# NREL/SSRS

Hardware: AMD Instinct MI355X
Metric: simulated tracks/sec (whole node) (higher is better)
Workload: dtype f64

## Files before the change

include/ssrs_hip.h:

```cpp
#ifndef SSRS_HIP_H_
#define SSRS_HIP_H_

#include <stddef.h>
#include <stdint.h>

#ifdef __cplusplus
extern "C" {
#endif

#define SSRS_VERSION 108

#define SSRS_OK 0
#define SSRS_ERR_INVALID (-1)
#define SSRS_ERR_HIP (-2)
#define SSRS_ERR_START (-3)

#define SSRS_F32 0
#define SSRS_F64 1

int ssrs_version(void);
int ssrs_build_flags(void);
const char *ssrs_last_error(void);
int ssrs_device_info(int device, char *name, size_t name_len, int *compute_units,
                     size_t *hbm_bytes);
// ... 174 lines not shown
                       int64_t ntracks, const int64_t *traj_offsets, int16_t *traj,
                       void *cursor_ws, size_t cursor_bytes, void *stream);

int ssrs_hist_reduce(uint32_t *hist, size_t n, int root, void *nccl_comm, void *stream);


int ssrs_presence_count(const int16_t *traj, int64_t npoints, uint32_t *hist,
                        int rows, int cols, void *scratch8, void *stream);

size_t ssrs_presence_workspace_bytes(int rows, int cols, int krad);

int ssrs_presence_smooth(const uint32_t *count, int krad, float *out, int rows,
                         int cols, void *workspace, size_t workspace_bytes,
                         void *stream);

int ssrs_presence_smooth_u64(const uint64_t *count, int krad, float *out, int rows,
                             int cols, void *workspace, size_t workspace_bytes,
                             void *stream);

int ssrs_presence_normalise_add(const void *src, int src_type, double *acc, size_t n,
                                void *scratch8, void *stream);
int ssrs_presence_normalise_f32(const double *src, float *out, size_t n,
                                void *scratch8, void *stream);


#define SSRS_TURBINE_BIN 32
#define SSRS_TURBINE_MAX 8192
int ssrs_turbine_encounters(const int16_t *traj, const int64_t *traj_offsets, int64_t ntracks,
                            const double *turbines, int nturb, double radius_cells,
                            const int32_t *bin_start, const int32_t *bin_items, int rows, int cols,
                            uint32_t *hits, int32_t *first_step, void *stream);

int ssrs_turbine_encounter_counts(const uint32_t *hits, int64_t ntracks, int nturb,
                                  int64_t *tracks_per_turbine, int32_t *turbines_per_track, void *stream);


#define SSRS_OCCUPANCY_MAX_PLANES 8
size_t ssrs_track_occupancy_workspace_bytes(int rows, int cols, int planes);
int ssrs_track_occupancy(const int16_t *traj, const int64_t *traj_offsets, int64_t ntracks,
                         int rows, int cols, int planes,
                         uint32_t *counts, uint32_t *cells_per_track,
                         void *workspace, size_t workspace_bytes, void *stream);


#define SSRS_RAY_ROW_NORTH 0
#define SSRS_RAY_ROW_EAST 1
#define SSRS_SHELTER_AUTO 0
#define SSRS_SHELTER_LDS 1
#define SSRS_SHELTER_GLOBAL 2
int ssrs_shelter_sx(const void *dem, int dem_type, double res, const double *ray_ur, const double *ray_uc,
                    const double *wdirn, double dmax, int ray_axes, int path, double *tan_sx, double *sx_deg,
                    int rows, int cols, int batch, void *stream);

typedef struct SsrsShelterParams {
    double dmax;
    int32_t ray_axes;
    int32_t path;
    double height;
    double coef[7];
} SsrsShelterParams;

int ssrs_updraft_sheltered(const void *dem, int dem_type, double res, const double *ray_ur, const double *ray_uc,
                           const double *wspeed0, const double *wdirn0, const double *wspeed, const double *wdirn,
                           const void *slope, const void *aspect, int sa_type, const SsrsShelterParams *params,
                           double min_updraft_val, double threshold, float *orograph, double *usable,
                           double *sx_deg, int rows, int cols, int batch, void *stream);

int ssrs_shelter_sx_sector(const void *dem, int dem_type, double res, const double *ray_ur, const double *ray_uc,
                           const double *wdirn, double dmax, int ray_axes, int path, double sector_half_width,
                           double sector_step, double *tan_sx, double *sx_deg, int rows, int cols, int batch,
                           void *stream);
int ssrs_updraft_sheltered_sector(const void *dem, int dem_type, double res, const double *ray_ur, const double *ray_uc,
                                  const double *wspeed0, const double *wdirn0, const double *wspeed,
                                  const double *wdirn, const void *slope, const void *aspect, int sa_type,
                                  const SsrsShelterParams *params, double sector_half_width, double sector_step,
                                  double min_updraft_val, double threshold, float *orograph, double *usable,
                                  double *sx_deg, int rows, int cols, int batch, void *stream);


#define SSRS_SMOOTH_AUTO 0
#define SSRS_SMOOTH_LDS 1
#define SSRS_SMOOTH_GLOBAL 2
size_t ssrs_smooth_workspace_bytes(int rows, int cols, int batch, double sigma);
int ssrs_smooth_reflect(const float *in, double sigma, int path, double min_updraft_val, double threshold,
                        double *smooth, float *orograph, double *usable, int rows, int cols, int batch,
                        void *workspace, size_t workspace_bytes, void *stream);


#define SSRS_ALLEN_MAX_UPDRAFTS (1 << 22)
#define SSRS_ALLEN_TABLE_COLS 6
#define SSRS_ALLEN_AUTO 0
#define SSRS_ALLEN_LDS 1
#define SSRS_ALLEN_GLOBAL 2
size_t ssrs_allen_workspace_bytes(int n_updrafts);
int ssrs_allen_thermal_field(const double *xt, const double *yt, const double *wgain, const double *rgain,
                             int n_updrafts, const int32_t *bin_start, const int32_t *bin_items, double bin_size_m,
                             int nbx, int nby, double rbar, double wtbar, double zzi, int z_below_zi, double we,
                             double res, int rows, int cols, int path, void *out, int out_type, int32_t *nearest,
                             double *table, void *workspace, size_t workspace_bytes, void *stream);


typedef struct SsrsProjection {
    double a;
    double e2;
    double lat_1;
    double lat_2;
    double lat_0;
    double lon_0;
    double x_0;
    double y_0;
    double n;
    double C;
    double rho0;
    double e;
} SsrsProjection;

int ssrs_projection_init_albers(SsrsProjection *proj);

int ssrs_warp_lonlat_raster(const void *src, int src_type, int src_rows, int src_cols, double lon0, double lat0,
                            double dlon, double dlat, double nodata, const SsrsProjection *proj, double west,
                            double south, double res, void *dst, int dst_type, double *lon, double *lat,
                            unsigned long long *uncovered, int rows, int cols, void *stream);


typedef struct SsrsSolveStats {
    int32_t iterations;
    int32_t converged;
    double residual;
    float kernel_ms;
    int32_t amg_levels;
    int32_t amg_coarsest;
    float setup_ms;
    uint64_t workspace_used;
} SsrsSolveStats;

#define SSRS_SOLVE_NO_AMG 1
#define SSRS_SOLVE_K_CYCLE 2
#define SSRS_SOLVE_ONE_SIDED 4

size_t ssrs_potential_workspace_bytes(int rows, int cols);

int ssrs_potential_solve(const double *conductivity, const uint8_t *fixed_mask,
                         const double *fixed_values, const double *initial_guess,
                         float *potential, int rows, int cols, double rel_tol,
                         int max_iterations, int flags, void *workspace,
                         size_t workspace_bytes,
                         void *stats ,
                         void *stream);

int ssrs_uniform_selftest(uint64_t seed, const uint64_t *track,
                          const uint64_t *step, double *out, size_t n,
                          void *stream);

#ifdef __cplusplus
}
#endif
#endif
```

ssrs_amd/_native.py:

```python
import ctypes as C
import os

_HERE = os.path.dirname(os.path.abspath(__file__))
LIB_PATH = os.environ.get('SSRS_HIP_LIB') or os.path.join(_HERE, 'libssrs_hip.so')

SSRS_F32, SSRS_F64 = 0, 1
SSRS_OK, SSRS_ERR_INVALID, SSRS_ERR_HIP, SSRS_ERR_START = 0, -1, -2, -3
SSRS_TRACKS_PROFILE = 1
SSRS_TRACKS_EXACT_ONLY = 2
SSRS_TRACKS_NO_SCHEDULE = 4
SSRS_TRACKS_NO_BINNING = 8
SSRS_TRACKS_RING_TABLE = 16
SSRS_TRACKS_SCATTERED = 32
SSRS_TRACKS_NO_SCATTERED = 64
SSRS_TRACKS_THR_TABLE = 128
SSRS_SOLVE_NO_AMG = 1
SSRS_TURBINE_BIN, SSRS_TURBINE_MAX = 32, 8192
SSRS_OCCUPANCY_MAX_PLANES = 8
SSRS_RAY_AXES = {'row_north': 0, 'row_east': 1}
SSRS_SHELTER_PATH = {'auto': 0, 'lds': 1, 'global': 2}
SSRS_SMOOTH_PATH = {'auto': 0, 'lds': 1, 'global': 2}
SSRS_ALLEN_PATH = {'auto': 0, 'lds': 1, 'global': 2}
SSRS_ALLEN_MAX_UPDRAFTS, SSRS_ALLEN_TABLE_COLS = 1 << 22, 6
SSRS_INTERP = {'nearest': 0, 'linear': 1, 'cubic': 2}

EXPORTS = (
    'ssrs_version', 'ssrs_build_flags', 'ssrs_last_error', 'ssrs_device_info', 'ssrs_slope_aspect',
    'ssrs_orographic_updraft', 'ssrs_threshold_updraft', 'ssrs_updraft_from_dem',
    'ssrs_lattice_workspace_bytes', 'ssrs_updraft_from_dem_lattice',
    'ssrs_wind_from_lattice', 'ssrs_wind_triangles_workspace_bytes', 'ssrs_wind_from_triangles',
    'ssrs_wind_nearest_workspace_bytes', 'ssrs_wind_nearest_index', 'ssrs_wind_from_nearest',
    'ssrs_wind_cubic_workspace_bytes', 'ssrs_wind_from_triangles_cubic', 'ssrs_thermal_seeds', 'ssrs_blur_workspace_bytes',
    'ssrs_gaussian_blur', 'ssrs_thermal_fields', 'ssrs_potential_temperature', 'ssrs_deardorff_velocity',
    'ssrs_thermal_updraft', 'ssrs_scalar_interp_workspace_bytes', 'ssrs_scalar_from_samples', 'ssrs_wtk_thermal_fields',
    'ssrs_track_params_init', 'ssrs_transition_table_build',
    'ssrs_transition_ring_bytes', 'ssrs_transition_ring_build',
    'ssrs_transition_thr_bytes', 'ssrs_transition_thr_build',
    'ssrs_tracks_workspace_bytes', 'ssrs_tracks_workspace_bytes_ex', 'ssrs_tracks_simulate', 'ssrs_uniform_selftest',
    'ssrs_traj_recorder_create', 'ssrs_traj_recorder_destroy', 'ssrs_traj_recorder_complete',
    'ssrs_traj_recorder_used', 'ssrs_tracks_simulate_rec', 'ssrs_tracks_gather', 'ssrs_tracks_simulate_h64',
    'ssrs_hist_reduce', 'ssrs_presence_count', 'ssrs_presence_workspace_bytes', 'ssrs_presence_smooth',
    'ssrs_presence_smooth_u64',
    'ssrs_presence_normalise_add', 'ssrs_presence_normalise_f32',
    'ssrs_potential_workspace_bytes', 'ssrs_potential_solve',
    'ssrs_turbine_encounters', 'ssrs_turbine_encounter_counts',
    'ssrs_shelter_sx', 'ssrs_updraft_sheltered', 'ssrs_shelter_sx_sector', 'ssrs_updraft_sheltered_sector',
    'ssrs_smooth_workspace_bytes', 'ssrs_smooth_reflect',
    'ssrs_projection_init_albers', 'ssrs_warp_lonlat_raster',
    'ssrs_allen_workspace_bytes', 'ssrs_allen_thermal_field',
    'ssrs_track_occupancy_workspace_bytes', 'ssrs_track_occupancy',
)


class SsrsTrackParams(C.Structure):
    _fields_ = [('rows', C.c_int32), ('cols', C.c_int32), ('burnin', C.c_int32),
                ('memory_parameter', C.c_int32), ('max_moves', C.c_int64),
                ('scaling_parameter', C.c_double), ('prior', C.c_double * 9),
                ('steps_per_launch', C.c_int32), ('flags', C.c_int32)]


class SsrsTrackStats(C.Structure):
    _fields_ = [('total_steps', C.c_int64), ('launches', C.c_int32),
                ('kernel_ms', C.c_float), ('wall_ms', C.c_float), ('hist_ms', C.c_float),
                ('window_launches', C.c_int32), ('tile_launches', C.c_int32),
                ('block_window_launches', C.c_int32), ('wander_sorts', C.c_int32),
                ('timed_launches', C.c_int32), ('first_move_ms', C.c_float),
                ('block_window_ms', C.c_float), ('block_window_timed', C.c_int32),
                ('block_window_steps', C.c_int64), ('roam_launches', C.c_int32), ('reserved0', C.c_int32),
                ('roam_wave_pairs', C.c_int64), ('roam_slow_wave_pairs', C.c_int64),
                ('roam_shuffles', C.c_int32), ('roam_wide_launches', C.c_int32)]


class SsrsSolveStats(C.Structure):
    _fields_ = [('iterations', C.c_int32), ('converged', C.c_int32),
                ('residual', C.c_double), ('kernel_ms', C.c_float),
                ('amg_levels', C.c_int32), ('amg_coarsest', C.c_int32),
                ('setup_ms', C.c_float), ('workspace_used', C.c_uint64)]


class SsrsShelterParams(C.Structure):
    _fields_ = [('dmax', C.c_double), ('ray_axes', C.c_int32), ('path', C.c_int32), ('height', C.c_double),
                ('coef', C.c_double * 7)]


class SsrsProjection(C.Structure):
    _fields_ = [(name, C.c_double) for name in ('a', 'e2', 'lat_1', 'lat_2', 'lat_0', 'lon_0', 'x_0', 'y_0',
                                                'n', 'C', 'rho0', 'e')]


OCCUPANCY_ARGTYPES = [C.c_void_p, C.c_void_p, C.c_int64, C.c_int, C.c_int, C.c_int, C.c_void_p, C.c_void_p, C.c_void_p,
                      C.c_size_t, C.c_void_p]

ALLEN_FIELD_ARGTYPES = [C.c_void_p] * 4 + [C.c_int, C.c_void_p, C.c_void_p, C.c_double, C.c_int, C.c_int] + \
    [C.c_double] * 3 + [C.c_int, C.c_double, C.c_double, C.c_int, C.c_int, C.c_int, C.c_void_p, C.c_int, C.c_void_p,
                        C.c_void_p, C.c_void_p, C.c_size_t, C.c_void_p]


class SsrsError(RuntimeError):
    def __init__(self, code, message):
        super().__init__(f'libssrs_hip error {code}: {message}')
        self.code = code


_lib = None


def lib():
    global _lib
    if _lib is None:
        if not os.path.exists(LIB_PATH):
            raise ImportError(
                f'{LIB_PATH} is missing: build it with `python ssrs_amd/csrc/build.py` '
                '(hipcc, gfx950). ssrs_amd has no CPU fallback.')
        L = C.CDLL(LIB_PATH)
        L.ssrs_version.restype = C.c_int
        if L.ssrs_build_flags() & 1 and not os.environ.get('SSRS_ALLOW_PROBE_LIB'):
            raise ImportError(f'{LIB_PATH} is a timing-probe build (results are wrong on purpose); '
                              'set SSRS_ALLOW_PROBE_LIB=1 for timing runs only')
        L.ssrs_last_error.restype = C.c_char_p
        L.ssrs_tracks_workspace_bytes.restype = C.c_size_t
        L.ssrs_tracks_workspace_bytes.argtypes = [C.c_int64]
        L.ssrs_lattice_workspace_bytes.restype = C.c_size_t
        L.ssrs_wind_triangles_workspace_bytes.restype = C.c_size_t
        L.ssrs_wind_triangles_workspace_bytes.argtypes = [C.c_int, C.c_int, C.c_int, C.c_int]
        L.ssrs_lattice_workspace_bytes.argtypes = [C.c_int, C.c_int, C.c_int]
        L.ssrs_wind_nearest_workspace_bytes.restype = C.c_size_t
        L.ssrs_wind_nearest_workspace_bytes.argtypes = [C.c_int, C.c_int, C.c_int]
        L.ssrs_wind_nearest_index.argtypes = [C.c_void_p, C.c_int, C.c_double, C.c_void_p, C.c_int, C.c_int,
                                              C.c_void_p, C.c_size_t, C.c_void_p]
        L.ssrs_wind_cubic_workspace_bytes.restype = C.c_size_t
        L.ssrs_wind_cubic_workspace_bytes.argtypes = [C.c_int, C.c_int, C.c_int, C.c_int, C.c_int]
        L.ssrs_wind_from_triangles_cubic.argtypes = [C.c_void_p] * 8 + [C.c_int, C.c_int, C.c_double, C.c_void_p, C.c_void_p,
                                                                        C.c_int, C.c_int, C.c_int, C.c_void_p, C.c_size_t,
                                                                        C.c_void_p]
        L.ssrs_tracks_workspace_bytes_ex.restype = C.c_size_t
        L.ssrs_tracks_workspace_bytes_ex.argtypes = [C.c_int64, C.c_int, C.c_int, C.c_int]
        L.ssrs_traj_recorder_create.restype = C.c_void_p
        L.ssrs_traj_recorder_create.argtypes = [C.c_void_p, C.c_size_t]
        L.ssrs_traj_recorder_destroy.restype = None
        L.ssrs_traj_recorder_destroy.argtypes = [C.c_void_p]
        L.ssrs_traj_recorder_complete.argtypes = [C.c_void_p]
        L.ssrs_traj_recorder_used.restype = C.c_size_t
        L.ssrs_traj_recorder_used.argtypes = [C.c_void_p]
        L.ssrs_transition_thr_bytes.restype = C.c_size_t
        L.ssrs_transition_thr_bytes.argtypes = [C.c_int, C.c_int]
        L.ssrs_transition_ring_bytes.restype = C.c_size_t
        L.ssrs_transition_ring_bytes.argtypes = [C.c_int, C.c_int]
        if hasattr(L, 'ssrs_presence_workspace_bytes'):
            L.ssrs_presence_workspace_bytes.restype = C.c_size_t
            L.ssrs_presence_workspace_bytes.argtypes = [C.c_int, C.c_int, C.c_int]
        if hasattr(L, 'ssrs_blur_workspace_bytes'):
            L.ssrs_blur_workspace_bytes.restype = C.c_size_t
            L.ssrs_blur_workspace_bytes.argtypes = [C.c_int, C.c_int, C.c_double]
        L.ssrs_thermal_fields.argtypes = [C.c_void_p, C.c_double, C.c_double, C.POINTER(C.c_uint64), C.c_int,
                                          C.c_void_p, C.c_int, C.c_int, C.c_int, C.c_void_p]
        L.ssrs_potential_temperature.argtypes = [C.c_void_p, C.c_void_p, C.c_void_p, C.c_size_t, C.c_void_p]
        L.ssrs_deardorff_velocity.argtypes = [C.c_void_p, C.c_void_p, C.c_void_p, C.c_double, C.c_void_p, C.c_size_t, C.c_void_p]
        L.ssrs_thermal_updraft.argtypes = [C.c_void_p, C.c_double, C.c_void_p, C.c_void_p, C.c_double, C.c_void_p, C.c_size_t,
                                           C.c_void_p]
        L.ssrs_scalar_interp_workspace_bytes.restype = C.c_size_t
        L.ssrs_scalar_interp_workspace_bytes.argtypes = [C.c_int] * 5
        L.ssrs_scalar_from_samples.argtypes = [C.c_int] + [C.c_void_p] * 7 + [C.c_int, C.c_int, C.c_double, C.c_void_p, C.c_int,
                                                                             C.c_int, C.c_int, C.c_void_p, C.c_size_t, C.c_void_p]
        L.ssrs_wtk_thermal_fields.argtypes = [C.c_int] + [C.c_void_p] * 7 + [C.c_int, C.c_int, C.c_double, C.c_void_p, C.c_double,
                                                                            C.c_double, C.c_void_p, C.c_int, C.c_int, C.c_int,
                                                                            C.c_int, C.c_void_p, C.c_size_t, C.c_void_p]
        if hasattr(L, 'ssrs_potential_workspace_bytes'):
            L.ssrs_potential_workspace_bytes.restype = C.c_size_t
            L.ssrs_potential_workspace_bytes.argtypes = [C.c_int, C.c_int]
        if hasattr(L, 'ssrs_turbine_encounters'):
            L.ssrs_turbine_encounters.argtypes = [C.c_void_p, C.c_void_p, C.c_int64, C.c_void_p, C.c_int, C.c_double,
                                                  C.c_void_p, C.c_void_p, C.c_int, C.c_int, C.c_void_p, C.c_void_p,
                                                  C.c_void_p]
            L.ssrs_turbine_encounter_counts.argtypes = [C.c_void_p, C.c_int64, C.c_int, C.c_void_p, C.c_void_p, C.c_void_p]
        L.ssrs_shelter_sx.argtypes = [C.c_void_p, C.c_int, C.c_double, C.c_void_p, C.c_void_p, C.c_void_p, C.c_double,
                                      C.c_int, C.c_int, C.c_void_p, C.c_void_p, C.c_int, C.c_int, C.c_int, C.c_void_p]
        L.ssrs_updraft_sheltered.argtypes = [C.c_void_p, C.c_int, C.c_double] + [C.c_void_p] * 8 + \
            [C.c_int, C.POINTER(SsrsShelterParams), C.c_double, C.c_double, C.c_void_p, C.c_void_p, C.c_void_p,
             C.c_int, C.c_int, C.c_int, C.c_void_p]
        L.ssrs_shelter_sx_sector.argtypes = [C.c_void_p, C.c_int, C.c_double, C.c_void_p, C.c_void_p, C.c_void_p, C.c_double,
                                             C.c_int, C.c_int, C.c_double, C.c_double, C.c_void_p, C.c_void_p, C.c_int,
                                             C.c_int, C.c_int, C.c_void_p]
        L.ssrs_updraft_sheltered_sector.argtypes = [C.c_void_p, C.c_int, C.c_double] + [C.c_void_p] * 8 + \
            [C.c_int, C.POINTER(SsrsShelterParams), C.c_double, C.c_double, C.c_double, C.c_double, C.c_void_p, C.c_void_p,
             C.c_void_p, C.c_int, C.c_int, C.c_int, C.c_void_p]
        L.ssrs_smooth_workspace_bytes.restype = C.c_size_t
        L.ssrs_smooth_workspace_bytes.argtypes = [C.c_int, C.c_int, C.c_int, C.c_double]
        L.ssrs_smooth_reflect.argtypes = [C.c_void_p, C.c_double, C.c_int, C.c_double, C.c_double, C.c_void_p, C.c_void_p,
                                          C.c_void_p, C.c_int, C.c_int, C.c_int, C.c_void_p, C.c_size_t, C.c_void_p]
        L.ssrs_projection_init_albers.argtypes = [C.POINTER(SsrsProjection)]
        L.ssrs_warp_lonlat_raster.argtypes = [C.c_void_p, C.c_int, C.c_int, C.c_int] + [C.c_double] * 5 + \
            [C.POINTER(SsrsProjection)] + [C.c_double] * 3 + [C.c_void_p, C.c_int, C.c_void_p, C.c_void_p, C.c_void_p,
                                                             C.c_int, C.c_int, C.c_void_p]
        L.ssrs_allen_workspace_bytes.restype = C.c_size_t
        L.ssrs_allen_workspace_bytes.argtypes = [C.c_int]
        L.ssrs_allen_thermal_field.argtypes = ALLEN_FIELD_ARGTYPES
        L.ssrs_track_occupancy_workspace_bytes.restype = C.c_size_t
        L.ssrs_track_occupancy_workspace_bytes.argtypes = [C.c_int, C.c_int, C.c_int]
        L.ssrs_track_occupancy.argtypes = OCCUPANCY_ARGTYPES
        _lib = L
    return _lib


def check(rc):
    if rc != SSRS_OK:
        msg = lib().ssrs_last_error().decode('utf-8', 'replace')
        if rc == SSRS_ERR_INVALID or rc == SSRS_ERR_START:
            raise ValueError(f'libssrs_hip: {msg}')
        raise SsrsError(rc, msg)


def ptr(t):
    return C.c_void_p(0 if t is None else t.data_ptr())
```

ssrs_amd/csrc/tracks.hip:

```cpp
#include <rocrand/rocrand_philox4x32_10.h>
#include <hipcub/hipcub.hpp>

#include <cmath>
#include <cstdlib>
#include <cstring>
#include <new>
#include <vector>

#include "common.h"
#include "track_plan.h"
#include "track_policy.h"

namespace ssrs {

__host__ __device__ constexpr int dr_of(int k) { return k / 3 - 1; }
__host__ __device__ constexpr int dc_of(int k) { return k % 3 - 1; }
#define SSRS_NINV_DIAG 0.70710677f

constexpr uint32_t restriction(int d)
{
    const int dr = dr_of(d), dc = dc_of(d);
    uint32_t m = 0;
    for (int k = 0; k < 9; ++k) {
        bool ok = false;
// ... 31 lines not shown
    int n = 0;
    for (int k = 0; k < 9 && n < 3; ++k)
        if ((restriction(d) >> k) & 1u) v |= static_cast<uint32_t>(k < 4 ? k : k - 1) << (3 * n++);
    return v;
}
constexpr uint64_t pack_candidates(int first, int count)
{
    uint64_t v = 0;
    for (int i = 0; i < count; ++i) v |= static_cast<uint64_t>(candidates(first + i)) << (9 * i);
    return v;
}
constexpr uint64_t kCandLo = pack_candidates(0, 7), kCandHi = pack_candidates(7, 2);
static_assert(candidates(7) == (5u | (6u << 3) | (7u << 6)), "(1,0) -> table slots 5,6,7");
static_assert(candidates(5) == (2u | (4u << 3) | (7u << 6)), "(0,1) -> k = 2,5,8 = slots 2,4,7");

__device__ __forceinline__ uint32_t candidates_of(uint32_t d)
{
    const uint64_t v = d < 7 ? (kCandLo >> (9 * d)) : (kCandHi >> (9 * (d - 7)));
    return static_cast<uint32_t>(v) & 0x1FFu;
}

constexpr int kRingK[8] = {7, 8, 5, 2, 1, 0, 3, 6};
constexpr int ring_of_k(int k)
{
    for (int c = 0; c < 8; ++c)
        if (kRingK[c] == k) return c;
    return 8;
}
constexpr bool ring_matches_restrictions()
{
    for (int c = 0; c < 8; ++c) {
        const uint32_t m = (1u << kRingK[(c + 7) % 8]) | (1u << kRingK[c]) | (1u << kRingK[(c + 1) % 8]);
        if (m != restriction(kRingK[c])) return false;
    }
    return true;
}
static_assert(ring_matches_restrictions(), "restriction(d) = ring neighbours of d");
constexpr uint32_t ring_order(int c)
{
    const int ks[3] = {kRingK[(c + 7) % 8], kRingK[c], kRingK[(c + 1) % 8]};
    uint32_t v = 0;
    int n = 0;
    for (int k = 0; k < 9; ++k)
        for (int j = 0; j < 3; ++j)
            if (ks[j] == k) v |= static_cast<uint32_t>(j) << (2 * n++);
    return v;
}
constexpr uint64_t pack_ring_orders()
{
    uint64_t v = 0;
    for (int c = 0; c < 8; ++c) v |= static_cast<uint64_t>(ring_order(c)) << (6 * c);
    return v;
}
constexpr uint64_t kRingOrder = pack_ring_orders();
constexpr uint32_t kOrdId = 0u | (1u << 2) | (2u << 4), kOrdRot = 2u | (0u << 2) | (1u << 4),
                   kOrdRev = 2u | (1u << 2) | (0u << 4), kOrdSwp = 1u | (0u << 2) | (2u << 4);
static_assert(ring_order(0) == kOrdId && ring_order(6) == kOrdId && ring_order(7) == kOrdId, "x0 x1 x2");
static_assert(ring_order(1) == kOrdRot, "after NE: x2 x0 x1");
static_assert(ring_order(2) == kOrdRev && ring_order(3) == kOrdRev && ring_order(4) == kOrdRev, "x2 x1 x0");
static_assert(ring_order(5) == kOrdSwp, "after SW: x1 x0 x2");
static_assert(ring_order(0) == (0u | (1u << 2) | (2u << 4)), "after N: NW, N, NE are k = 6, 7, 8");
static_assert(ring_order(2) == (2u | (1u << 2) | (0u << 4)), "after E: NE, E, SE are k = 8, 5, 2");
constexpr uint32_t pack_ring_deltas(bool rows)
{
    uint32_t v = 1u << 16;
    for (int c = 0; c < 8; ++c)
        v |= static_cast<uint32_t>((rows ? dr_of(kRingK[c]) : dc_of(kRingK[c])) + 1) << (2 * c);
    return v;
}
constexpr uint32_t kRingDr = pack_ring_deltas(true), kRingDc = pack_ring_deltas(false);
constexpr uint32_t pack_ring_next(int sel)
{
    uint32_t v = 0;
    for (int c = 0; c < 8; ++c) v |= static_cast<uint32_t>((c + 7 + ((ring_order(c) >> (2 * sel)) & 3u)) & 7u) << (4 * c);
    return v;
}
constexpr uint32_t kRingNext0 = pack_ring_next(0), kRingNext1 = pack_ring_next(1), kRingNext2 = pack_ring_next(2);
constexpr uint32_t pack_ring_deltas_signed(bool rows)
{
    uint32_t v = 0;
    for (int c = 0; c < 8; ++c)
        v |= (static_cast<uint32_t>(rows ? dr_of(kRingK[c]) : dc_of(kRingK[c])) & 3u) << (4 * c);
    return v;
}
constexpr uint32_t kRingDrS = pack_ring_deltas_signed(true), kRingDcS = pack_ring_deltas_signed(false);
constexpr uint64_t pack_ring_of_k()
{
    uint64_t v = 0;
    for (int k = 0; k < 9; ++k) v |= static_cast<uint64_t>(ring_of_k(k)) << (4 * k);
    return v;
}
constexpr uint64_t kRingOfK = pack_ring_of_k();
constexpr uint64_t pack_k_of_ring()
{
    uint64_t v = 4ull << 32;
    for (int c = 0; c < 8; ++c) v |= static_cast<uint64_t>(kRingK[c]) << (4 * c);
    return v;
}
constexpr uint64_t kKOfRing = pack_k_of_ring();
constexpr int kRingFloats = 10;
__host__ __device__ constexpr size_t ring_mask_offset(int rows, int cols)
{
    return static_cast<size_t>(rows) * static_cast<size_t>(cols) * kRingFloats * sizeof(float) + 8;
}

__device__ __forceinline__ uint4 philox_block(uint64_t seed, uint64_t track, uint64_t blk)
{
#ifdef SSRS_PROBE_NO_PHILOX
    const uint32_t h = static_cast<uint32_t>(blk) * 0x9E3779B9u ^ static_cast<uint32_t>(track) * 0x85EBCA6Bu ^
                       static_cast<uint32_t>(seed);
    return make_uint4(h * 0xC2B2AE35u, h ^ 0x27D4EB2Fu, (h >> 3) * 0x165667B1u, h + 0x9E3779B9u);
#endif
    rocrand_state_philox4x32_10 st;
    rocrand_init(seed, track, blk * 4ull, &st);
    return rocrand4(&st);
}

__device__ __forceinline__ uint4 philox_block_b3(uint64_t seed, uint64_t track, uint64_t blk)
{
    uint32_t c0 = static_cast<uint32_t>(blk), c1 = static_cast<uint32_t>(blk >> 32);
    uint32_t c2 = static_cast<uint32_t>(track), c3 = static_cast<uint32_t>(track >> 32);
    uint32_t k0 = static_cast<uint32_t>(seed), k1 = static_cast<uint32_t>(seed >> 32);
#pragma unroll
    for (int r = 0; r < 10; ++r) {
        const uint64_t p0 = static_cast<uint64_t>(0xD2511F53u) * c0, p1 = static_cast<uint64_t>(0xCD9E8D57u) * c2;
        const uint32_t n0 = __builtin_amdgcn_bitop3_b32(static_cast<uint32_t>(p1 >> 32), c1, k0, 0x96);
        const uint32_t n2 = __builtin_amdgcn_bitop3_b32(static_cast<uint32_t>(p0 >> 32), c3, k1, 0x96);
        c1 = static_cast<uint32_t>(p1);
        c3 = static_cast<uint32_t>(p0);
        c0 = n0;
        c2 = n2;
        k0 += 0x9E3779B9u;
        k1 += 0xBB67AE85u;
    }
    return make_uint4(c0, c1, c2, c3);
}

__device__ __forceinline__ double words_to_uniform(uint32_t a, uint32_t b)
{
    return (static_cast<double>(a >> 5) * 67108864.0 + static_cast<double>(b >> 6)) *
           (1.0 / 9007199254740992.0);
}

__global__ void k_uniform_selftest(uint64_t seed, const uint64_t *track, const uint64_t *step,
                                   double *out, size_t n)
{
    const size_t i = blockIdx.x * static_cast<size_t>(blockDim.x) + threadIdx.x;
    if (i >= n) return;
    const uint4 w = philox_block(seed, track[i], step[i] >> 1);
    const uint4 v = philox_block_b3(seed, track[i], step[i] >> 1);
    const bool same = w.x == v.x && w.y == v.y && w.z == v.z && w.w == v.w;
    const double u = (step[i] & 1) ? words_to_uniform(w.z, w.w) : words_to_uniform(w.x, w.y);
    out[i] = same ? u : __longlong_as_double(0x7FF8000000000000ll);
}

__host__ __device__ __forceinline__ double sum9(const double *x)
{
    return (((x[0] + x[1]) + (x[2] + x[3])) + ((x[4] + x[5]) + (x[6] + x[7]))) + x[8];
}

__device__ __forceinline__ int choose_move(const double *w, const double *prior, double nu,
                                           uint32_t mask, double u, bool fast)
{
    double q[9];
    bool has_nan = false;
#pragma unroll
    for (int k = 0; k < 9; ++k) has_nan |= (w[k] != w[k]);
#pragma unroll
    for (int k = 0; k < 9; ++k) {
        const double v = has_nan ? prior[k] : w[k];
        q[k] = v > 0.0 ? v : 0.0;
    }
    q[4] = 0.0;
    bool any = false;
#pragma unroll
    for (int k = 0; k < 9; ++k) {
        const double z = q[k] * 0.0;
        q[k] = ((mask >> k) & 1u) ? q[k] : z;
        any |= (q[k] != 0.0);
    }
    if (!any) {
#pragma unroll
        for (int k = 0; k < 9; ++k) {
            q[k] = ((mask >> k) & 1u) && k != 4 ? prior[k] : 0.0;
            any |= (q[k] != 0.0);
        }
        if (!any) {
#pragma unroll
            for (int k = 0; k < 9; ++k) q[k] = prior[k];
        }
    }
    if (fast) {
        double c[8];
        double acc = 0.0;
#pragma unroll
        for (int k = 0; k < 8; ++k) { acc = acc + q[k]; c[k] = acc; }
        const double ut = u * (acc + q[8]);
        const double band = ut * 0x1p-46;
        int idx = 0;
        bool near = false;
#pragma unroll
        for (int k = 0; k < 8; ++k) {
            const double d = c[k] - ut;
            idx += d <= 0.0 ? 1 : 0;
            near |= !(fabs(d) > band);
        }
        if (!near) return idx;
    }
    const double s1 = sum9(q);
#pragma unroll
    for (int k = 0; k < 9; ++k) q[k] = q[k] / s1;
    if (nu != 1.0) {
#pragma unroll
        for (int k = 0; k < 9; ++k) q[k] = pow(q[k], nu);
    }
    const double s2 = sum9(q);
    double acc = 0.0;
    double cdf[9];
#pragma unroll
    for (int k = 0; k < 9; ++k) {
        q[k] = q[k] / s2;
        acc = acc + q[k];
        cdf[k] = acc;
    }
    int idx = 0;
#pragma unroll
    for (int k = 0; k < 9; ++k) idx += (cdf[k] / cdf[8] <= u) ? 1 : 0;
    return idx;
}

__device__ __forceinline__ int choose_table_fast(const double *t, uint32_t mask, double u)
{
    double c[8];
    double acc = 0.0;
#pragma unroll
    for (int j = 0; j < 8; ++j) {
        const int k = j < 4 ? j : j + 1;
        acc = acc + (((mask >> k) & 1u) ? t[j] : 0.0);
        c[j] = acc;
    }
    const double ut = u * acc;
    const double band = ut * 0x1p-46;
    int idx = 0;
    double closest = __builtin_inf();
#pragma unroll
    for (int j = 0; j < 7; ++j) {
        const double d = c[j] - ut;
        const int le = d <= 0.0 ? 1 : 0;
        idx += (j == 3) ? 2 * le : le;
        closest = fmin(closest, fabs(d));
    }
    const bool near = !(acc > 0.0) || !(closest > band);
    return near ? -1 : idx;
}

__device__ __forceinline__ int choose_three_fast(double wa, double wb, double wc, double u)
{
    const double ca = wa + 0.0;
    const double cb = ca + wb;
    const double acc = cb + wc;
    const double ut = u * acc;
    const double band = ut * 0x1p-46;
    const double da = ca - ut, db = cb - ut;
    const int sel = da > 0.0 ? 0 : (db > 0.0 ? 1 : 2);
    const double closest = fmin(fmin(fabs(da), fabs(db)), fmin(ut, fabs(acc - ut)));
    const bool near = !(acc > 0.0) || !(closest > band);
    return near ? -1 : sel;
}

__device__ __forceinline__ int choose_three_ring(float fa, float fb, float fc, double u)
{
    const double ca = static_cast<double>(fa);
    const double cb = ca + static_cast<double>(fb);
    const double acc = cb + static_cast<double>(fc);
    const double ut = u * acc;
    const double band = acc * 0x1p-21;
    const double da = ca - ut, db = cb - ut;
    const int sel = da > 0.0 ? 0 : (db > 0.0 ? 1 : 2);
    const double closest = fmin(fabs(da), fabs(db));
    const bool near = !(acc > 0x1p-90) || !(closest > band);
    return near ? -1 : sel;
}

__device__ __forceinline__ int choose_three_ring_f32(float fa, float fb, float fc, float uf)
{
    const float cb = fa + fb;
    const float acc = cb + fc;
    const float ut = uf * acc;
    const float band = acc * 0x1p-19f;
    const float da = fa - ut, db = cb - ut;
    const int sel = da > 0.f ? 0 : (db > 0.f ? 1 : 2);
    const float closest = fminf(fabsf(da), fabsf(db));
    const bool near = !(acc > 0x1p-90f) || !(closest > band);
    return near ? -1 : sel;
}

template <bool HAS_POT>
__device__ __forceinline__ void window_weights(const double *__restrict__ updraft,
                                               const float *__restrict__ potential,
                                               int cols, int row, int col, double *w)
{
    const size_t centre = static_cast<size_t>(row) * cols + col;
    double win[9];
#pragma unroll
    for (int j = 0; j < 9; ++j) {
        const double v = updraft[centre + dr_of(j) * cols + dc_of(j)];
// ... 28 lines not shown
        v[j] = updraft[centre + dr_of(j) * cols + dc_of(j)];
        fine &= (v[j] <= 1e150) & (v[j] >= -1e150);
        if (HAS_POT) {
            p[j] = potential[centre + dr_of(j) * cols + dc_of(j)];
            fine &= fabsf(p[j]) <= 1e38f;
        }
    }
    if (!fine) return -1;
    const double ic = 1.0 / (v[4] > 1e-06 ? v[4] : 1e-06);
    double w3[3] = {0.0, 0.0, 0.0};
    int k3[3] = {0, 0, 0};
    int n = 0;
#pragma unroll
    for (int j = 0; j < 9; ++j) {
        if (j == 4) continue;
        const bool adm = (mask >> j) & 1u;
        if (adm) {
            double w = 2.0 / (ic + 1.0 / (v[j] > 1e-06 ? v[j] : 1e-06));
            if (HAS_POT) {
                const float d = p[4] - p[j];
                const float ninv = (j & 1) ? 1.f : SSRS_NINV_DIAG;
                const float e = d * ninv;
                w = w * static_cast<double>(e);
            }
            w = w > 0.0 ? w : 0.0;
            if (n == 0) { w3[0] = w; k3[0] = j; } else if (n == 1) { w3[1] = w; k3[1] = j; } else { w3[2] = w; k3[2] = j; }
            ++n;
        }
    }
    if (n != 3) return -1;
    if (w3[0] == 0.0 && w3[1] == 0.0 && w3[2] == 0.0) {
        const double *t = thr + 9u * last_k;
        int idx = 0;
#pragma unroll
        for (int k = 0; k < 9; ++k) idx += t[k] <= u ? 1 : 0;
        return (idx == 4 || idx > 8) ? -1 : idx;
    }
    const int sel = choose_three_fast(w3[0], w3[1], w3[2], u);
    return sel < 0 ? -1 : (sel == 0 ? k3[0] : (sel == 1 ? k3[1] : k3[2]));
}

constexpr int kTabW = 64, kTabH = 16;
__device__ __forceinline__ int xcd_band(int b, int n)
{
    const int q = n / 8, r = n % 8, x = b % 8, j = b / 8;
    return (x < r ? x * (q + 1) : r * (q + 1) + (x - r) * q) + j;
}

template <bool RING>
__global__ __launch_bounds__(kBlock) void k_transition_table(
    const double *__restrict__ updraft, const float *__restrict__ potential,
    void *__restrict__ table_out, int rows, int cols, int tiles_x, int ntiles)
{
    constexpr int LW = kTabW + 2, LH = kTabH + 2;
    __shared__ double s_inv[LW * LH];
    __shared__ float s_pot[LW * LH];
    const int t = xcd_band(blockIdx.x, ntiles);
    const int r0 = (t / tiles_x) * kTabH, c0 = (t % tiles_x) * kTabW;
    for (int i = threadIdx.x; i < LW * LH; i += kBlock) {
        const int lr = i / LW, lc = i - lr * LW;
        int gr = r0 - 1 + lr, gc = c0 - 1 + lc;
        gr = gr < 0 ? 0 : (gr >= rows ? rows - 1 : gr);
        gc = gc < 0 ? 0 : (gc >= cols ? cols - 1 : gc);
        const size_t g = static_cast<size_t>(gr) * cols + gc;
        const double v = updraft[g];
        const double w = v != v ? v : (v > 1e-06 ? v : 1e-06);
        s_inv[i] = 1.0 / w;
        s_pot[i] = potential ? potential[g] : 0.f;
    }
    __syncthreads();
    const int lc = static_cast<int>(threadIdx.x % kTabW) + 1;
    const int col = c0 + lc - 1;
    if (col >= cols) return;
    for (int lr = static_cast<int>(threadIdx.x / kTabW) + 1; lr <= kTabH; lr += kBlock / kTabW) {
        const int row = r0 + lr - 1;
        if (row >= rows) break;
        const size_t i = static_cast<size_t>(row) * cols + col;
        double w[9];
        const bool interior = row > 0 && col > 0 && row < rows - 1 && col < cols - 1;
        if (interior) {
            const double ic = s_inv[lr * LW + lc];
            const float pc = s_pot[lr * LW + lc];
#pragma unroll
            for (int j = 0; j < 9; ++j) {
                const int o = (lr + dr_of(j)) * LW + lc + dc_of(j);
                w[j] = 2.0 / (ic + s_inv[o]);
                if (potential) {
                    const float d = pc - s_pot[o];
                    const float ninv = (j == 4) ? 0.f : ((j & 1) ? 1.f : SSRS_NINV_DIAG);
                    const float e = d * ninv;
                    w[j] = w[j] * static_cast<double>(e);
                }
            }
        } else {
#pragma unroll
            for (int j = 0; j < 9; ++j) w[j] = 0.0;
        }
        bool has_nan = false;
#pragma unroll
        for (int j = 0; j < 9; ++j) has_nan |= (w[j] != w[j]);
        if (RING) {
            bool bad = has_nan;
#pragma unroll
            for (int j = 0; j < 9; ++j) bad |= (w[j] - w[j] != 0.0);
            float f[kRingFloats];
#pragma unroll
            for (int j = 0; j < kRingFloats; ++j) {
                const double v = w[kRingK[(j + 7) % 8]];
                f[j] = bad ? __builtin_nanf("") : (v > 0.0 ? static_cast<float>(v) : -0.0f);
            }
            float2 *dst = reinterpret_cast<float2 *>(static_cast<float *>(table_out) + i * kRingFloats);
#pragma unroll
            for (int k = 0; k < kRingFloats / 2; ++k) dst[k] = make_float2(f[2 * k], f[2 * k + 1]);
            uint32_t zm = 0;
#pragma unroll
            for (int c = 0; c < 8; ++c) zm |= (!bad && !(w[kRingK[c]] > 0.0)) ? (1u << c) : 0u;
            (static_cast<uint8_t *>(table_out) + ring_mask_offset(rows, cols))[i] = static_cast<uint8_t>(zm);
        } else {
            double2 *dst = reinterpret_cast<double2 *>(static_cast<double *>(table_out) + i * 8);
            double o[8];
#pragma unroll
            for (int j = 0, k = 0; j < 9; ++j) {
                if (j == 4) continue;
                o[k++] = has_nan ? __builtin_nan("") : (w[j] > 0.0 ? w[j] : 0.0);
            }
#pragma unroll
            for (int k = 0; k < 4; ++k) dst[k] = make_double2(o[2 * k], o[2 * k + 1]);
        }
    }
}

struct alignas(16) TrackState {
    int32_t pos;
    int32_t k;
    uint32_t dirs;
    uint32_t aux;
};

static_assert(kPlanBlock == kBlock, "track_plan.h counts in stepper blocks");
struct alignas(16) TrackCtl {
    uint32_t count[4][kXcd];
    uint32_t error;
    uint32_t par_min;
    unsigned long long steps;
    unsigned long long strays;
    uint32_t bin_done;
    uint32_t pad;
    double prior[9];
    unsigned long long roam_slow;
    unsigned long long roam_pairs;
    unsigned long long dbg_tsum, dbg_tmax, dbg_waves, dbg_slowmax;
    uint32_t roam_stop;
    uint32_t deal_live;
};

static_assert(sizeof(TrackCtl) <= 128 * sizeof(uint32_t), "final read-back slot of pinned_counts()");

constexpr uint32_t kWanderMix = 256;
constexpr int kBinRows = 36, kBinCols = kWinCols / 4;
constexpr int kWinBinRows = kWinRows / kBinRows;
constexpr int kWanderBins = 16384;
struct WanderWindows {
    int32_t n;
    int32_t r0[kWanderWindows], c0[kWanderWindows];
};



struct PlanGeom {
    double cos_t, sin_t;
    int offset;
};
__device__ __forceinline__ void plan_coords(const PlanGeom &g, int row, int col, int &par, int &perp)
{
    par = static_cast<int>(lrint(row * g.cos_t + col * g.sin_t)) + g.offset;
    perp = static_cast<int>(lrint(col * g.cos_t - row * g.sin_t)) + g.offset;
}

template <typename KeyT>
__global__ __launch_bounds__(kBlock) void k_plan_keys(const int32_t *__restrict__ start_rc,
                                                     long long ntracks, PlanGeom g,
                                                     KeyT *__restrict__ keys,
                                                     int32_t *__restrict__ vals, TrackCtl *ctl, int par_bits)
{
    const long long t = blockIdx.x * static_cast<long long>(kBlock) + threadIdx.x;
    int par = 0x7fffffff;
    if (t < ntracks) {
        int perp;
        plan_coords(g, start_rc[2 * t], start_rc[2 * t + 1], par, perp);
        par = par < 0 ? 0 : par;
        perp = perp < 0 ? 0 : perp;
        const int top = (1 << par_bits) - 1;
        keys[t] = (static_cast<KeyT>(perp > top ? top : perp) << par_bits) | static_cast<KeyT>(par > top ? top : par);
        vals[t] = static_cast<int32_t>(t);
    }
    __shared__ int s_min;
    if (threadIdx.x == 0) s_min = 0x7fffffff;
    __syncthreads();
#pragma unroll
    for (int off = 32; off > 0; off >>= 1) {
        const int o = __shfl_down(par, off);
        par = o < par ? o : par;
    }
    if ((threadIdx.x & 63) == 0 && par != 0x7fffffff) atomicMin(&s_min, par);
    __syncthreads();
    if (threadIdx.x == 0 && s_min != 0x7fffffff) atomicMin(&ctl->par_min, static_cast<uint32_t>(s_min));
}

__device__ __forceinline__ int wander_window_of(const WanderWindows *__restrict__ w, int n, int row, int col)
{
    int id = n;
    for (int q = n - 1; q >= 0; --q)
        if (static_cast<uint32_t>(row - w->r0[q]) < static_cast<uint32_t>(kWinRows) &&
            static_cast<uint32_t>(col - w->c0[q]) < static_cast<uint32_t>(kWinCols)) id = q;
    return id;
}

enum { MODE_PRIOR = 0, MODE_UPDRAFT = 1, MODE_FLUIDFLOW = 2, MODE_TABLE = 3 };

struct RoamEntry;

struct StepArgs {
    int rows, cols, burnin, memory;
    long long max_k;
    double nu;
    const double *prior;
    const double *updraft;
    const float *potential;
    const double *table;
    unsigned long long seed, track_base;
    uint32_t *hist;
    int16_t *end_rc;
    int32_t *lengths;
    int16_t *traj;
    const long long *traj_off;
    TrackState *state;
    const int32_t *list_in;
    int32_t *list_out;
    TrackCtl *ctl;
    int launch;
    int fast;
    int steps;
    int coherent;
    uint32_t *visits;
    long long visit_stride;
    uint32_t cap;
    long long it_base;
    int plane_shift;
    uint32_t guard;
    int v16_offset;
    int pf_dir, pf_rc;
    uint32_t vcap;
    const double *thr;
    const uint8_t *zmask;
    uint32_t *hist_copies;
    int ncopies;
    const WanderWindows *wander;
    const RoamEntry *roam;
    const void *fine;
    int roam_stop;
    int cheap_exact;
    unsigned long long *dbg_buf;
    int debug_roam;
    uint32_t vis_r, vis_c;
};

__global__ __launch_bounds__(kBlock) void k_tracks_init(
    const int32_t *__restrict__ start_rc, long long ntracks, int rows, int cols,
    uint32_t *hist, int16_t *traj, const long long *traj_off, int32_t *lengths,
    int16_t *end_rc, TrackState *state, TrackCtl *ctl, PlanGeom g, int coherent, uint32_t cap)
{
    const long long t = blockIdx.x * static_cast<long long>(kBlock) + threadIdx.x;
    if (t < kXcd) {
        const long long left = ntracks - t * static_cast<long long>(cap);
        ctl->count[0][t] = static_cast<uint32_t>(left < 0 ? 0 : (left > cap ? cap : left));
        ctl->count[1][t] = ctl->count[2][t] = ctl->count[3][t] = 0;
        if (t == 0) ctl->steps = 0;
    }
    if (t >= ntracks) return;
    const int row = start_rc[2 * t], col = start_rc[2 * t + 1];
    TrackState s;
    s.dirs = 0x44444444u;
    uint32_t delay = 0;
    if (coherent) {
        int par, perp;
        plan_coords(g, row, col, par, perp);
        par = par < 0 ? 0 : par;
        const uint32_t pmin = ctl->par_min;
        delay = static_cast<uint32_t>(par) > pmin ? static_cast<uint32_t>(par) - pmin : 0u;
        if (delay > 0x7FFFFFu) delay = 0x7FFFFFu;
        delay &= ~1u;
    }
    s.aux = kAllButCentre | (delay << 9);
    if (row < 0 || col < 0 || row >= rows || col >= cols) {
        atomicOr(&ctl->error, 1u);
        s.pos = 0;
        s.k = -1;
        if (lengths) lengths[t] = 0;
        if (end_rc) { end_rc[2 * t] = -1; end_rc[2 * t + 1] = -1; }
    } else {
        s.pos = row | (col << 16);
        s.k = 0;
        if (hist) atomicAdd(&hist[static_cast<size_t>(row) * cols + col], 1u);
        if (traj)
            reinterpret_cast<uint32_t *>(traj)[traj_off[t]] =
                static_cast<uint32_t>(row & 0xFFFF) | (static_cast<uint32_t>(col) << 16);
    }
    state[t] = s;
}

template <int MODE>
__global__ __launch_bounds__(kBlock) void k_step_tracks(const StepArgs a)
{
    TrackCtl *ctl = a.ctl;
    const int in_slot = a.launch & 3, out_slot = (a.launch + 1) & 3;
    const uint32_t xcd = blockIdx.x % kXcd;
    const uint32_t nlive = ctl->count[in_slot][xcd];
    const uint32_t il = (blockIdx.x / kXcd) * kBlock + threadIdx.x;
    const uint32_t i = xcd * a.cap + il;
    const uint32_t iv = xcd * a.vcap + il;
    if (blockIdx.x == 0 && threadIdx.x < kXcd)
        ctl->count[(a.launch + 2) & 3][threadIdx.x] = 0;
    if ((il & ~63u) >= nlive) return;

    bool active = il < nlive;
    const int32_t t = active ? (a.list_in ? a.list_in[i] : static_cast<int32_t>(i)) : 0;
    TrackState s = {0, -1, 0, 0};
    if (active) s = a.state[t];
    active = active && s.k >= 0;
    int row = s.pos & 0xFFFF, col = (s.pos >> 16) & 0xFFFF;
    int k = s.k;
    const int max_k = static_cast<int>(a.max_k);
    uint32_t dirs = s.dirs, run = s.aux & 0x1FFu;
    const long long rel64 = (a.coherent ? static_cast<long long>(s.aux >> 9) : 0) -
                            static_cast<long long>(a.launch) * a.steps;
    const int release = rel64 > 0x7fffffffLL ? 0x7fffffff : (rel64 < 0 ? 0 : static_cast<int>(rel64));
    const unsigned long long track = a.track_base + static_cast<unsigned long long>(t);
    const long long toff = (a.traj && active) ? a.traj_off[t] : 0;
    const long long troom = (a.traj && active) ? a.traj_off[t + 1] - toff : 0;
    uint32_t pend_a = 0, pend_b = 0;
    bool have_pending = false;
    uint32_t moved = 0;
    int last_it = -1;

    const int lane_id = threadIdx.x & 63;

    bool done = false;
    int er = row, ec = col;
    auto loop_head = [&]() {
        done = !(k < max_k);
        er = row;
        ec = col;
        if (!done) {
            if (k > a.burnin) {
                done = !(0 < row && row < a.rows - 1 && 0 < col && col < a.cols - 1);
            } else {
                if (er <= 1) er += 2; else if (er >= a.rows - 2) er -= 2;
                if (ec <= 0) ec += 2; else if (ec >= a.cols - 2) ec -= 2;
            }
        }
    };
    double2 t0 = {0.0, 0.0}, t1 = t0, t2 = t0, t3 = t0;
    auto fetch_entry = [&]() {
        if (MODE == MODE_TABLE) {
            const double2 *src = reinterpret_cast<const double2 *>(
                a.table + (static_cast<size_t>(er) * a.cols + ec) * 8);
            t0 = src[0]; t1 = src[1]; t2 = src[2]; t3 = src[3];
        }
    };
    if (active) loop_head();
    fetch_entry();

    for (int it = 0; it < a.steps; ++it) {
        if (!__any(active)) break;
        bool stepped = false;
        if (active && it >= release) {
            if (done) {
                if (a.lengths) a.lengths[t] = static_cast<int32_t>(k + 1);
                if (a.end_rc)
                    reinterpret_cast<uint32_t *>(a.end_rc)[t] =
                        static_cast<uint32_t>(row & 0xFFFF) | (static_cast<uint32_t>(col) << 16);
                active = false;
            } else {
                uint32_t wa, wb;
                if ((k & 1) && have_pending) {
                    wa = pend_a; wb = pend_b;
                } else {
                    const uint4 w4 = philox_block(a.seed, track, static_cast<unsigned long long>(k) >> 1);
                    if (k & 1) { wa = w4.z; wb = w4.w; }
                    else { wa = w4.x; wb = w4.y; pend_a = w4.z; pend_b = w4.w; }
                }
                have_pending = !(k & 1);
                const double u = words_to_uniform(wa, wb);
                uint32_t mask = kAllButCentre;
                if (a.memory == 1) {
                    mask = restriction_of(dirs & 0xFu);
                } else if (a.memory == 0) {
                    mask = run;
                } else {
                    uint32_t d = dirs;
                    for (int j = 0; j < a.memory; ++j) {
                        mask &= restriction_of(d & 0xFu);
                        d >>= 4;
                    }
                }
                int idx = -1;
                if (MODE == MODE_TABLE) {
                    const double tt[8] = {t0.x, t0.y, t1.x, t1.y, t2.x, t2.y, t3.x, t3.y};
                    if (a.fast) idx = choose_table_fast(tt, mask, u);
                    if (__builtin_expect(idx < 0, 0)) {
                        double o[8];
#pragma unroll
                        for (int j = 0; j < 8; ++j) { o[j] = tt[j]; asm volatile("" : "+v"(o[j])); }
                        asm volatile("" : "+v"(mask));
                        const double w[9] = {o[0], o[1], o[2], o[3], 0.0, o[4], o[5], o[6], o[7]};
                        double pr[9];
#pragma unroll
                        for (int j = 0; j < 9; ++j) pr[j] = a.prior[j];
                        idx = choose_move(w, pr, a.nu, mask, u, false);
                    }
                } else {
                    double w[9];
                    if (MODE == MODE_FLUIDFLOW) {
                        window_weights<true>(a.updraft, a.potential, a.cols, er, ec, w);
                    } else if (MODE == MODE_UPDRAFT) {
                        window_weights<false>(a.updraft, a.potential, a.cols, er, ec, w);
                    } else {
#pragma unroll
                        for (int j = 0; j < 9; ++j) w[j] = a.prior[j];
                    }
                    double pr[9];
#pragma unroll
                    for (int j = 0; j < 9; ++j) pr[j] = a.prior[j];
                    idx = choose_move(w, pr, a.nu, mask, u, a.fast != 0);
                }
                row = er + idx / 3 - 1;
                col = ec + idx % 3 - 1;
                dirs = (dirs << 4) | static_cast<uint32_t>(idx);
                if (a.memory == 0) run &= restriction_of(static_cast<uint32_t>(idx));
                ++k;
                ++moved;
                stepped = true;
                loop_head();
                if (a.traj && k < troom)
                    reinterpret_cast<uint32_t *>(a.traj)[toff + k] =
                        static_cast<uint32_t>(row & 0xFFFF) | (static_cast<uint32_t>(col) << 16);
            }
        }
        fetch_entry();
        if (a.visits) {
            a.visits[static_cast<long long>(it) * a.visit_stride + iv] =
                stepped ? __umul24(static_cast<uint32_t>(row), a.vis_r) + __umul24(static_cast<uint32_t>(col), a.vis_c)
                        : 0xFFFFFFFFu;
        } else if (a.hist) {
            uint32_t *h = a.hist;
            if (a.hist_copies)
                h = a.hist_copies + static_cast<size_t>((i >> 6) % static_cast<uint32_t>(a.ncopies)) *
                                        (static_cast<size_t>(a.rows) * a.cols);
            atomicAdd(&h[static_cast<size_t>(row) * a.cols + col], stepped ? 1u : 0u);
        }
        last_it = it;
    }
    if (a.visits)
        for (int it = last_it + 1; it < a.steps; ++it)
            a.visits[static_cast<long long>(it) * a.visit_stride + iv] = 0xFFFFFFFFu;

    const unsigned long long live = __ballot(active);
    const int lane = lane_id;
    const int nsurv = __popcll(live);
    uint32_t base = 0;
    if (lane == 0 && nsurv) base = atomicAdd(&ctl->count[out_slot][xcd], static_cast<uint32_t>(nsurv));
    base = __shfl(base, 0);
    if (active) {
        const int rank = __popcll(live & ((1ull << lane) - 1ull));
        a.list_out[xcd * a.cap + base + rank] = t;
        TrackState o;
        o.pos = row | (col << 16);
        o.k = k;
        o.dirs = dirs;
        o.aux = run | (s.aux & ~0x1FFu);
        a.state[t] = o;
    }
    unsigned long long m = moved;
#pragma unroll
    for (int off = 32; off > 0; off >>= 1) m += __shfl_down(m, off);
    if (lane == 0 && m) atomicAdd(&ctl->steps, m);
}

struct PriorArg { double v[9]; };

constexpr unsigned long long kThrMagic = 0x3152485453525353ull;
struct ThrHeader {
    unsigned long long magic;
    int32_t rows, cols;
    double prior[9];
};
static_assert(sizeof(ThrHeader) <= 256, "the header lives in the leading guard band (>= 256 bytes)");

__global__ void k_ctl_init(TrackCtl *ctl, const PriorArg pr, double *__restrict__ thr, WanderWindows *wander,
                           const ThrHeader *__restrict__ header, int rows, int cols)
{
    const int d = threadIdx.x;
    if (d == 33) wander->n = 0;
    if (d < 32) reinterpret_cast<uint32_t *>(ctl->count)[d] = 0;
    if (d == 32) {
        uint32_t bad = 0;
        if (header) {
            bad = (header->magic != kThrMagic || header->rows != rows || header->cols != cols) ? 2u : 0u;
            for (int k = 0; k < 9; ++k) bad |= (header->prior[k] != pr.v[k]) ? 2u : 0u;
        }
        ctl->error = bad; ctl->par_min = 0xFFFFFFFFu; ctl->steps = 0; ctl->strays = 0; ctl->bin_done = 0; ctl->pad = 0; ctl->roam_slow = 0; ctl->roam_pairs = 0;
        ctl->dbg_tsum = ctl->dbg_tmax = ctl->dbg_waves = ctl->dbg_slowmax = 0;
        ctl->roam_stop = ctl->deal_live = 0;
    }
    if (d < 9) ctl->prior[d] = pr.v[d];
    if (d >= 9) return;
    const double *prior = pr.v;
    const uint32_t mask = restriction_of(static_cast<uint32_t>(d));
    double q[9];
    bool any = false;
#pragma unroll
    for (int k = 0; k < 9; ++k) {
        q[k] = ((mask >> k) & 1u) && k != 4 ? prior[k] : 0.0;
        any |= (q[k] != 0.0);
    }
    if (!any) {
#pragma unroll
        for (int k = 0; k < 9; ++k) q[k] = prior[k];
    }
    const double s1 = sum9(q);
#pragma unroll
    for (int k = 0; k < 9; ++k) q[k] = q[k] / s1;
    const double s2 = sum9(q);
    double acc = 0.0, cdf[9];
#pragma unroll
    for (int k = 0; k < 9; ++k) {
        q[k] = q[k] / s2;
        acc = acc + q[k];
        cdf[k] = acc;
    }
#pragma unroll
    for (int k = 0; k < 9; ++k) thr[d * 9 + k] = cdf[k] / cdf[8];
}

constexpr uint32_t pack_slot_deltas(bool rows)
{
    uint32_t v = 0;
    for (int j = 0; j < 8; ++j) {
        const int k = j < 4 ? j : j + 1;
        v |= static_cast<uint32_t>((rows ? dr_of(k) : dc_of(k)) + 1) << (2 * j);
    }
    return v;
}
constexpr uint32_t kSlotDr = pack_slot_deltas(true), kSlotDc = pack_slot_deltas(false);

struct __attribute__((packed, aligned(4))) RingTriple { float x0, x1, x2; };

template <bool RING, bool ZMASK = false, bool VT = false>
__global__ __launch_bounds__(kBlock) void k_step_lean(const StepArgs a)
{
    TrackCtl *ctl = a.ctl;
    const int in_slot = a.launch & 3, out_slot = (a.launch + 1) & 3;
    const uint32_t xcd = blockIdx.x % kXcd;
    const uint32_t nlive = ctl->count[in_slot][xcd];
    const uint32_t il = (blockIdx.x / kXcd) * kBlock + threadIdx.x;
    const uint32_t i = xcd * a.cap + il;
    const uint32_t iv = xcd * a.vcap + il;
    if (blockIdx.x == 0 && threadIdx.x < kXcd) ctl->count[(a.launch + 2) & 3][threadIdx.x] = 0;
    if ((il & ~63u) >= nlive) return;

    bool active = il < nlive;
    const int32_t t = active ? (a.list_in ? a.list_in[i] : static_cast<int32_t>(i)) : 0;
    TrackState s = {0, -1, 0, 0};
    if (active) s = a.state[t];
    active = active && s.k >= 0;
    const bool was_active = active;
    int row = s.pos & 0xFFFF, col = (s.pos >> 16) & 0xFFFF;
    int k = s.k;
    const int max_k = static_cast<int>(a.max_k);
    uint32_t dirs = s.dirs;
    uint32_t rc = static_cast<uint32_t>(kRingOfK >> (4 * (dirs & 0xFu))) & 0xFu;
    (void)rc;
    const long long rel64 = (a.coherent ? static_cast<long long>(s.aux >> 9) : 0) -
                            static_cast<long long>(a.launch) * a.steps;
    const int release = rel64 > 0x7fffffffLL ? 0x7fffffff : (rel64 < 0 ? 0 : static_cast<int>(rel64));
    const unsigned long long track = a.track_base + static_cast<unsigned long long>(t);
    uint32_t pend_a = 0, pend_b = 0, moved = 0;
    const uint32_t ucols = static_cast<uint32_t>(a.cols);
    const uint32_t in_rows = static_cast<uint32_t>(a.rows - 2), in_cols = static_cast<uint32_t>(a.cols - 2);

    bool done;
    int er, ec;
    auto loop_head = [&]() {
        const bool interior = static_cast<uint32_t>(row - 1) < in_rows && static_cast<uint32_t>(col - 1) < in_cols;
        done = !(k < max_k) || (k > a.burnin && !interior);
        er = row;
        ec = col;
        if (__any(k <= a.burnin)) {
            if (k <= a.burnin) {
                if (er <= 1) er += 2; else if (er >= a.rows - 2) er -= 2;
                if (ec <= 0) ec += 2; else if (ec >= a.cols - 2) ec -= 2;
            }
        }
    };
    double ta = 0.0, tb = 0.0, tc = 0.0;
    uint32_t cand = 0;
    RingTriple x = {0.f, 0.f, 0.f};
    (void)ta; (void)tb; (void)tc; (void)cand; (void)x;
    auto fetch_entry = [&]() {
        const uint32_t cell = __umul24(static_cast<uint32_t>(er), ucols) + static_cast<uint32_t>(ec);
        if (RING) {
            const float *src = reinterpret_cast<const float *>(a.table) +
                               static_cast<size_t>(cell) * kRingFloats + (rc & 7u);
            if (ZMASK) {
                const uint32_t m = a.zmask[cell];
                const uint32_t tri = (((m << 8) | m) >> ((rc + 7u) & 7u)) & 7u;
                if (tri == 7u && rc != 8u) x = RingTriple{-0.0f, -0.0f, -0.0f};
                else x = *reinterpret_cast<const RingTriple *>(src);
            } else {
#ifdef SSRS_PROBE_NO_GATHER
                (void)src;
                x = RingTriple{1.0f, 2.0f + static_cast<float>(er & 1), 1.5f};
#else
                x = *reinterpret_cast<const RingTriple *>(src);
#endif
            }
        } else {
            cand = candidates_of(dirs & 0xFu);
            const double *src = a.table + static_cast<size_t>(cell) * 8;
            ta = src[cand & 7u];
            tb = src[(cand >> 3) & 7u];
            tc = src[cand >> 6];
        }
    };
    loop_head();
    fetch_entry();

    int last_it = -1;
    auto one_step = [&](const int it, const bool even) {
        const bool go = active && it >= release;
        const bool st = go && !done;
        active = active && !(go && done);
        uint32_t w0, w1;
        if (even) {
            const uint4 w4 = philox_block(a.seed, track, static_cast<unsigned long long>(static_cast<uint32_t>(k) >> 1));
            w0 = w4.x; w1 = w4.y; pend_a = w4.z; pend_b = w4.w;
        } else {
            w0 = pend_a; w1 = pend_b;
        }
        int nrow, ncol;
        if (RING) {
            const float uf = static_cast<float>(w0 >> 8) * 0x1p-24f;
            const uint32_t ord = static_cast<uint32_t>(kRingOrder >> (6 * (rc & 7u))) & 63u;
            const uint32_t b0 = __float_as_uint(x.x0), b1 = __float_as_uint(x.x1), b2 = __float_as_uint(x.x2);
            const bool rot = ord == ring_order(1), rev = ord == ring_order(2), swp = ord == ring_order(5);
            const uint32_t ba = (rot || rev) ? b2 : (swp ? b1 : b0);
            const uint32_t bb = (rot || swp) ? b0 : b1;
            const uint32_t bc = rev ? b0 : (rot ? b1 : b2);
            int sel = choose_three_ring_f32(__uint_as_float(ba), __uint_as_float(bb), __uint_as_float(bc), uf);
            bool slow = st && (sel < 0 || rc == 8u);
            double u = 0.0;
            uint32_t prior_nc = 8u;
            if (__builtin_expect(__any(slow), 0)) {
                u = words_to_uniform(w0, w1);
                if (slow && rc != 8u) {
                    if ((ba & bb & bc) == 0x80000000u && (ba | bb | bc) == 0x80000000u) {
// ... 680 lines not shown
            s_surv[kBlock / 64] = tot ? atomicAdd(&ctl->count[out_slot][xcd], static_cast<uint32_t>(kBlock)) : 0xFFFFFFFFu;
        }
        __syncthreads();
        basei = s_surv[kBlock / 64];
        if (basei != 0xFFFFFFFFu) {
            a.list_out[xcd * a.cap + basei + threadIdx.x] = active ? t : -1;
            if (active) {
                TrackState o;
                o.pos = static_cast<int32_t>(row | (col << 16));
                o.k = k;
                o.dirs = static_cast<uint32_t>(kKOfRing >> (4 * rc)) & 0xFu;
                o.aux = s.aux;
                a.state[t] = o;
            }
        }
    } else {
        if (lane == 0 && nsurv) basei = atomicAdd(&ctl->count[out_slot][xcd], static_cast<uint32_t>(nsurv));
        basei = __shfl(basei, 0);
    }
    if (HM != 6 && active) {
        const int rank = __popcll(live & ((1ull << lane) - 1ull));
        a.list_out[xcd * a.cap + basei + rank] = t;
        TrackState o;
        o.pos = static_cast<int32_t>(row | (col << 16));
        o.k = k;
        o.dirs = static_cast<uint32_t>(kKOfRing >> (4 * rc)) & 0xFu;
        o.aux = s.aux;
        a.state[t] = o;
    }
    unsigned long long mv = live0 ? static_cast<unsigned long long>(k - s.k) : 0ull;
#pragma unroll
    for (int off = 32; off > 0; off >>= 1) mv += __shfl_down(mv, off);
    if (lane == 0 && mv) atomicAdd(&ctl->steps, mv);
}

struct alignas(16) RoamEntry {
    uint32_t e0, ea, eb, ec;
};
static_assert(sizeof(RoamEntry) == 16, "one dwordx4 per state");
constexpr size_t kPairMaxCells = 1ull << 25;

template <bool REV>
__global__ __launch_bounds__(kBlock) void k_roam_build(const char *__restrict__ tab, uint32_t guard, int plane_shift,
                                                      int rows, int cols, RoamEntry *__restrict__ out, const ThrPrior pr)
{
    const uint32_t nstate = static_cast<uint32_t>(rows) * static_cast<uint32_t>(cols) * 8u;
    for (uint32_t s = blockIdx.x * kBlock + threadIdx.x; s < nstate; s += gridDim.x * kBlock) {
        const uint32_t rc = s & 7u, cell = s >> 3;
        auto entry = [&](uint32_t c, uint32_t q) {
            return *reinterpret_cast<const uint32_t *>(tab + (guard + (q << plane_shift)) + (c << 2));
        };
        uint4 en = make_uint4(entry(cell, rc), kThrPoison, kThrPoison, kThrPoison);
        const bool rev = REV && en.x == kThrReversal;
        const uint32_t eu = rev ? pr.rev_e : en.x, rcd = rev ? pr.rev_rc : rc;
        if ((eu & 0xFFFFu) <= (eu >> 16)) {
            const uint32_t ord = static_cast<uint32_t>(kRingOrder >> (6u * rcd)) & 63u;
            uint32_t es[3];
#pragma unroll
            for (int j = 0; j < 3; ++j) {
                const uint32_t ncj = (rcd + 7u + ((ord >> (2 * j)) & 3u)) & 7u;
                const uint32_t cj = cell + ((kRingDr >> (2u * ncj)) & 3u) * static_cast<uint32_t>(cols) + ((kRingDc >> (2u * ncj)) & 3u) -
                                    static_cast<uint32_t>(cols) - 1u;
                es[j] = entry(cj, ncj);
            }
            en.y = es[0]; en.z = es[1]; en.w = es[2];
        }
        reinterpret_cast<uint4 *>(out)[s] = en;
    }
}

struct FineEntry { uint32_t t1, t2; };
struct FinePrior { uint32_t zero_t1[8], zero_t2[8], reversal; };

__host__ __device__ __forceinline__ uint32_t fine_fixed(double x)
{
    const double v = x * 4294967296.0 + 0.5;
    return v >= 4294967295.0 ? 0xFFFFFFFFu : static_cast<uint32_t>(static_cast<unsigned long long>(v));
}

template <bool HAS_POT>
__global__ __launch_bounds__(kBlock) void k_fine_build(const double *__restrict__ updraft, const float *__restrict__ potential,
                                                      FineEntry *__restrict__ out, int rows, int cols, int tiles_x, int ntiles,
                                                      const FinePrior fp)
{
    constexpr int LW = kTabW + 2, LH = kTabH + 2;
    __shared__ double s_inv[LW * LH];
    __shared__ float s_pot[LW * LH];
    const int t = xcd_band(blockIdx.x, ntiles);
    const int r0 = (t / tiles_x) * kTabH, c0 = (t % tiles_x) * kTabW;
    for (int i = threadIdx.x; i < LW * LH; i += kBlock) {
        const int lr = i / LW, lc = i - lr * LW;
        int gr = r0 - 1 + lr, gc = c0 - 1 + lc;
        gr = gr < 0 ? 0 : (gr >= rows ? rows - 1 : gr);
        gc = gc < 0 ? 0 : (gc >= cols ? cols - 1 : gc);
        const size_t g = static_cast<size_t>(gr) * cols + gc;
        const double v = updraft[g];
        const double w = v != v ? v : (v > 1e-06 ? v : 1e-06);
        s_inv[i] = 1.0 / w;
        s_pot[i] = HAS_POT ? potential[g] : 0.f;
    }
    __syncthreads();
    const int lc = static_cast<int>(threadIdx.x % kTabW) + 1;
    const int col = c0 + lc - 1;
    if (col >= cols) return;
    for (int lr = static_cast<int>(threadIdx.x / kTabW) + 1; lr <= kTabH; lr += kBlock / kTabW) {
        const int row = r0 + lr - 1;
        if (row >= rows) break;
        const size_t cell = static_cast<size_t>(row) * cols + col;
        const bool interior = row > 0 && col > 0 && row < rows - 1 && col < cols - 1;
        double w[9];
        bool bad = !interior;
        if (interior) {
            const double ic = s_inv[lr * LW + lc];
            const float pc = s_pot[lr * LW + lc];
#pragma unroll
            for (int j = 0; j < 9; ++j) {
                const int o = (lr + dr_of(j)) * LW + lc + dc_of(j);
                w[j] = 2.0 / (ic + s_inv[o]);
                if (HAS_POT) {
                    const float d = pc - s_pot[o];
                    const float ninv = (j == 4) ? 0.f : ((j & 1) ? 1.f : SSRS_NINV_DIAG);
                    const float e = d * ninv;
                    w[j] = w[j] * static_cast<double>(e);
                }
                bad |= !(w[j] - w[j] == 0.0);
                w[j] = w[j] > 0.0 ? w[j] : 0.0;
            }
        }
        FineEntry en[8];
#pragma unroll
        for (int rc = 0; rc < 8; ++rc) {
            const uint32_t ord = ring_order(rc);
            const int ring3[3] = {(rc + 7) % 8, rc, (rc + 1) % 8};
            const int ka = kRingK[ring3[ord & 3u]], kb = kRingK[ring3[(ord >> 2) & 3u]], kc = kRingK[ring3[(ord >> 4) & 3u]];
            FineEntry e = {0xFFFFFFFFu, 0u};
            if (!bad) {
                const double ab = w[ka] + w[kb], tot = ab + w[kc];
                if (tot == 0.0) {
                    if (!((fp.reversal >> rc) & 1u)) { e.t1 = fp.zero_t1[rc]; e.t2 = fp.zero_t2[rc]; }
                } else if (tot - tot == 0.0) {
                    e.t1 = fine_fixed(w[ka] / tot);
                    e.t2 = fine_fixed(ab / tot);
                    if (e.t1 > e.t2) e.t1 = e.t2;
                }
            }
            en[rc] = e;
        }
        uint4 *dst = reinterpret_cast<uint4 *>(out + cell * 8);
#pragma unroll
        for (int q = 0; q < 4; ++q) dst[q] = make_uint4(en[2 * q].t1, en[2 * q].t2, en[2 * q + 1].t1, en[2 * q + 1].t2);
    }
}

template <bool REV, int BT = kBlock>
__global__ __launch_bounds__(BT) void k_step_roam(const StepArgs a, const ThrPrior pr)
{
    __shared__ uint32_t s_win[kWinRows * kWinCols];
    __shared__ int s_box[4];
    __shared__ int s_wid[BT / 64];
    for (int q = threadIdx.x; q < kWinRows * kWinCols; q += BT) s_win[q] = 0u;
    if (threadIdx.x == 0) { s_box[0] = s_box[1] = 0x7fffffff; s_box[2] = s_box[3] = -1; }
    __syncthreads();
    TrackCtl *ctl = a.ctl;
    const int in_slot = a.launch & 3, out_slot = (a.launch + 1) & 3;
    const uint32_t xcd = blockIdx.x % kXcd;
    const uint32_t nlive = ctl->count[in_slot][xcd];
    const uint32_t il = (blockIdx.x / kXcd) * BT + threadIdx.x;
    const uint32_t i = xcd * a.cap + il;
    if (blockIdx.x == 0 && threadIdx.x < kXcd) ctl->count[(a.launch + 2) & 3][threadIdx.x] = 0;

    bool live0 = il < nlive;
    int32_t t = live0 ? (a.list_in ? a.list_in[i] : static_cast<int32_t>(i)) : 0;
    if (t < 0) { live0 = false; t = 0; }
    TrackState s = {0, -1, 0, 0};
    if (live0) s = a.state[t];
    uint32_t rc = static_cast<uint32_t>(kRingOfK >> (4 * (s.dirs & 0xFu))) & 0xFu;
    live0 = live0 && s.k >= 0 && rc < 8u;
    rc &= 7u;
    int row = s.pos & 0xFFFF, col = (s.pos >> 16) & 0xFFFF;
    int win_r0 = 0, win_c0 = 0;
    {
        int r_lo = live0 ? row : 0x7fffffff, r_hi = live0 ? row : -1, c_lo = live0 ? col : 0x7fffffff, c_hi = live0 ? col : -1;
#pragma unroll
        for (int off = 32; off > 0; off >>= 1) {
            int o = __shfl_xor(r_lo, off); r_lo = o < r_lo ? o : r_lo;
            o = __shfl_xor(r_hi, off); r_hi = o > r_hi ? o : r_hi;
            o = __shfl_xor(c_lo, off); c_lo = o < c_lo ? o : c_lo;
            o = __shfl_xor(c_hi, off); c_hi = o > c_hi ? o : c_hi;
        }
        if ((threadIdx.x & 63) == 0 && r_hi >= 0) {
            atomicMin(&s_box[0], r_lo); atomicMin(&s_box[1], c_lo);
            atomicMax(&s_box[2], r_hi); atomicMax(&s_box[3], c_hi);
        }
        __syncthreads();
        const bool fits = s_box[2] - s_box[0] < kWinRows && s_box[3] - s_box[1] < kWinCols;
        const int nwin = a.wander->n;
        int wid = live0 && nwin > 0 ? wander_window_of(a.wander, nwin, row, col) : 0x7fffffff;
        wid = wid >= nwin ? 0x7fffffff : wid;
        {
            const unsigned long long lm = __ballot(wid != 0x7fffffff);
            wid = lm ? __shfl(wid, __ffsll(static_cast<long long>(lm)) - 1) : 0x7fffffff;
        }
        if ((threadIdx.x & 63) == 0) s_wid[threadIdx.x >> 6] = wid;
        __syncthreads();
        wid = 0x7fffffff;
        for (int q = BT / 64 - 1; q >= 0; --q) wid = s_wid[q] != 0x7fffffff ? s_wid[q] : wid;
        if (wid != 0x7fffffff && threadIdx.x == 0) {
            s_box[0] = a.wander->r0[wid]; s_box[2] = s_box[0] + kWinRows - 1;
            s_box[1] = a.wander->c0[wid]; s_box[3] = s_box[1] + kWinCols - 1;
        }
        const bool placed = wid != 0x7fffffff;
        __syncthreads();
        if (!placed && !fits && threadIdx.x == 0) { s_box[0] = r_lo; s_box[1] = c_lo; s_box[2] = r_hi; s_box[3] = c_hi; }
        __syncthreads();
        if (s_box[2] >= 0) {
            win_r0 = (s_box[0] + s_box[2] + 1 - kWinRows) / 2;
            win_c0 = (s_box[1] + s_box[3] + 1 - kWinCols) / 2;
        }
    }
    const char *pair = reinterpret_cast<const char *>(a.roam);
    const uint32_t ucols = static_cast<uint32_t>(a.cols);
    const uint32_t last_cell = static_cast<uint32_t>(a.rows) * ucols - 1u;
    int k = s.k;
    const long long rel64 = (a.coherent ? static_cast<long long>(s.aux >> 9) : 0) + 1 - a.it_base;
    const int rel = rel64 > 0x3fffffffLL ? 0x3fffffff : (rel64 < 0 ? 0 : static_cast<int>(rel64));
    const long long left = a.max_k - k;
    uint32_t span = !live0 ? 0u : (left > 0x3fffffffLL ? 0x3fffffffu : (left < 0 ? 0u : static_cast<uint32_t>(left)));
    const int blk0 = (k - rel) >> 1;
    const unsigned long long track = a.track_base + static_cast<unsigned long long>(t);
    const char *tab = reinterpret_cast<const char *>(a.table);
    const uint32_t psh = static_cast<uint32_t>(a.plane_shift);
    const uint32_t rev_e = pr.rev_e;
    uint32_t win_stray = 0, n_fine = 0;
    const void *fine = a.fine;

    int wr = 0, wc = 0, lcell = 0;
    bool fast = false;
    uint4 E = make_uint4(kThrPoison, kThrPoison, kThrPoison, kThrPoison);
    auto enter = [&](bool released) __attribute__((always_inline)) {
        wr = row - win_r0;
        wc = col - win_c0;
        lcell = row * a.cols + col;
        fast = live0 && released && span != 0u && k > a.burnin;
        const uint32_t sidx = fast ? ((static_cast<uint32_t>(lcell) << 3) | rc) : 0u;
        E = *reinterpret_cast<const uint4 *>(pair + (sidx << 4));
    };
    enter(rel == 0);
    const uint32_t rev_rc4 = 4u * pr.rev_rc;

    auto slow_step = [&](const uint32_t w0, const uint32_t w1) __attribute__((always_inline)) {
        const uint32_t ufi = w0 >> 16;
        const uint32_t cell = static_cast<uint32_t>(row) * ucols + static_cast<uint32_t>(col);
        const uint32_t e = *reinterpret_cast<const uint32_t *>(tab + (a.guard + (rc << psh)) + (cell << 2));
        const int32_t d1 = static_cast<int32_t>(ufi) - static_cast<int32_t>(e & 0xFFFFu);
        const int32_t d2 = static_cast<int32_t>(ufi) - static_cast<int32_t>(e >> 16);
        const bool burn = k <= a.burnin;
        bool special = (static_cast<uint32_t>(d1 + 1) < 2u) | (static_cast<uint32_t>(d2 + 1) < 2u) | (d1 < d2);
        if (burn) special |= (row <= 1) | (row >= a.rows - 2) | (col >= a.cols - 2);
        uint32_t nc;
        int br = row, bc = col;
        if (!special) {
            const uint32_t ord = static_cast<uint32_t>(kRingOrder >> (6u * rc)) & 63u;
            const uint32_t neg = (static_cast<uint32_t>(d1) >> 31) + (static_cast<uint32_t>(d2) >> 31);
            nc = (rc + 7u + ((ord >> (4u - 2u * neg)) & 3u)) & 7u;
        } else {
            if (e == kThrBoundary && !burn) { span = 0u; return; }
            bool exact = true;
            nc = 0;
            if (fine && !(d1 < d2) && !(burn && ((row <= 1) | (row >= a.rows - 2) | (col >= a.cols - 2)))) {
                const uint2 f = reinterpret_cast<const uint2 *>(fine)[(cell << 3) | rc];
                const uint32_t u32 = (w0 & ~31u) | (w1 >> 27);
                const long long f1 = static_cast<long long>(u32) - static_cast<long long>(f.x);
                const long long f2 = static_cast<long long>(u32) - static_cast<long long>(f.y);
                const bool unsure = (f.x > f.y) | (static_cast<unsigned long long>(f1 + 1) < 2ull) | (static_cast<unsigned long long>(f2 + 1) < 2ull);
                if (!unsure) {
                    const uint32_t ord = static_cast<uint32_t>(kRingOrder >> (6u * rc)) & 63u;
                    const uint32_t neg = (f1 < 0 ? 1u : 0u) + (f2 < 0 ? 1u : 0u);
                    nc = (rc + 7u + ((ord >> (4u - 2u * neg)) & 3u)) & 7u;
                    exact = false;
                    ++n_fine;
                }
            }
            if (e == kThrReversal && !burn) {
                int idx = 0;
                bool near = false;
#pragma unroll
                for (int q = 0; q < 9; ++q) {
                    const int32_t d = static_cast<int32_t>(ufi) - static_cast<int32_t>(pr.thr9[q]);
                    idx += d >= 0 ? 1 : 0;
                    near |= static_cast<uint32_t>(d + 1) < 2u;
                }
                const uint32_t pnc = static_cast<uint32_t>(kRingOfK >> (4 * (idx > 8 ? 4 : idx))) & 0xFu;
                if (!near && pnc < 8u) { nc = pnc; exact = false; }
            }
            if (exact) {
                int er = row, ec = col;
                if (burn) {
                    if (er <= 1) er += 2; else if (er >= a.rows - 2) er -= 2;
                    if (ec <= 0) ec += 2; else if (ec >= a.cols - 2) ec -= 2;
                }
                double w[9];
                if (a.potential) window_weights<true>(a.updraft, a.potential, a.cols, er, ec, w);
                else window_weights<false>(a.updraft, a.potential, a.cols, er, ec, w);
                double prr[9];
#pragma unroll
                for (int j = 0; j < 9; ++j) prr[j] = a.prior[j];
                const uint32_t last = static_cast<uint32_t>(kKOfRing >> (4 * rc)) & 0xFu;
                const int idx = choose_move(w, prr, 1.0, restriction_of(last), words_to_uniform(w0, w1), true);
                nc = static_cast<uint32_t>(kRingOfK >> (4 * idx)) & 0xFu;
                br = er; bc = ec;
            }
        }
        row = br + static_cast<int>((kRingDr >> (2u * nc)) & 3u) - 1;
        col = bc + static_cast<int>((kRingDc >> (2u * nc)) & 3u) - 1;
        rc = nc;
        ++k;
        const uint32_t hr = static_cast<uint32_t>(row - win_r0), hc = static_cast<uint32_t>(col - win_c0);
        if (hr < static_cast<uint32_t>(kWinRows) && hc < static_cast<uint32_t>(kWinCols)) {
            atomicAdd(&s_win[hr * kWinCols + hc], 1u);
        } else {
            atomicAdd(&a.hist[static_cast<uint32_t>(row) * ucols + static_cast<uint32_t>(col)], 1u);
            ++win_stray;
        }
    };

    int it = 0;
    uint32_t n_pairs = 0, n_slow = 0;
    const unsigned long long t_begin = a.debug_roam ? __builtin_amdgcn_s_memtime() : 0ull;
    auto one_pair = [&]() __attribute__((always_inline)) {
        const uint4 w4 = philox_block_b3(a.seed, track, static_cast<unsigned long long>(static_cast<uint32_t>(blk0 + (it >> 1))));
        const uint32_t ufa = w4.x >> 16, ufb = w4.z >> 16;
        const bool st_a = static_cast<uint32_t>(it - rel) < span, st_b = static_cast<uint32_t>(it + 1 - rel) < span;
        const uint32_t q0 = E.x, qa = E.y, qb = E.z, qc = E.w;
        const uint32_t rc0 = rc;
        const uint32_t rc04 = 4u * rc0;
        const bool rva = REV && q0 == kThrReversal;
        const uint32_t eua = rva ? rev_e : q0;
        const uint32_t t4a = rva ? rev_rc4 : rc04;
        const bool ga1 = ufa >= (eua & 0xFFFFu), ga2 = ufa >= (eua >> 16);
        const uint32_t nxa = ga2 ? kRingNext2 : (ga1 ? kRingNext1 : kRingNext0);
        const uint32_t nca = (nxa >> t4a) & 7u, nca4 = 4u * nca;
        const uint32_t q1 = ga2 ? qc : (ga1 ? qb : qa);
        const int dra = __builtin_amdgcn_sbfe(static_cast<int>(kRingDrS), nca4, 2u), dca = __builtin_amdgcn_sbfe(static_cast<int>(kRingDcS), nca4, 2u);
        const int cell_a = lcell + __mul24(dra, a.cols) + dca;
        const bool rvb = REV && q1 == kThrReversal;
        const uint32_t eub = rvb ? rev_e : q1;
        const uint32_t t4b = rvb ? rev_rc4 : nca4;
        const bool gb1 = ufb >= (eub & 0xFFFFu), gb2 = ufb >= (eub >> 16);
        const uint32_t nxb = gb2 ? kRingNext2 : (gb1 ? kRingNext1 : kRingNext0);
        const uint32_t ncb = (nxb >> t4b) & 7u, ncb4 = 4u * ncb;
        const int drb = __builtin_amdgcn_sbfe(static_cast<int>(kRingDrS), ncb4, 2u), dcb = __builtin_amdgcn_sbfe(static_cast<int>(kRingDcS), ncb4, 2u);
        const int cell_b = cell_a + __mul24(drb, a.cols) + dcb;
        {
            const uint32_t cb = static_cast<uint32_t>(cell_b) < last_cell ? static_cast<uint32_t>(cell_b) : last_cell;
            E = *reinterpret_cast<const uint4 *>(pair + ((cb << 7) | (ncb4 << 2)));
        }
        const int wra = wr + dra, wca = wc + dca, wrb = wra + drb, wcb = wca + dcb;
        const int32_t a1 = static_cast<int32_t>(ufa) - static_cast<int32_t>(eua & 0xFFFFu);
        const int32_t a2 = static_cast<int32_t>(ufa) - static_cast<int32_t>(eua >> 16);
        const int32_t b1 = static_cast<int32_t>(ufb) - static_cast<int32_t>(eub & 0xFFFFu);
        const int32_t b2 = static_cast<int32_t>(ufb) - static_cast<int32_t>(eub >> 16);
        const bool special = (static_cast<uint32_t>(a1 + 1) < 2u) | (static_cast<uint32_t>(a2 + 1) < 2u) | (a1 < a2) |
                             (static_cast<uint32_t>(b1 + 1) < 2u) | (static_cast<uint32_t>(b2 + 1) < 2u) | (b1 < b2);
        const bool go = fast & st_a & st_b & !special;
        const bool in_a = go & (static_cast<uint32_t>(wra) < static_cast<uint32_t>(kWinRows)) & (static_cast<uint32_t>(wca) < static_cast<uint32_t>(kWinCols));
        const bool in_b = go & (static_cast<uint32_t>(wrb) < static_cast<uint32_t>(kWinRows)) & (static_cast<uint32_t>(wcb) < static_cast<uint32_t>(kWinCols));
        const bool out = go & !(in_a & in_b);
        const bool slow = (st_a | st_b) & !go;
        const unsigned long long rare = __ballot(out | slow);
        atomicAdd(&s_win[in_a ? (wra << 8) + wca : 0], in_a ? 1u : 0u);
        atomicAdd(&s_win[in_b ? (wrb << 8) + wcb : 0], in_b ? 1u : 0u);
        k += go ? 2 : 0;
        wr = go ? wrb : wr;
        wc = go ? wcb : wc;
        lcell = go ? cell_b : lcell;
        rc = go ? ncb : rc0;
        ++n_pairs;
        if (__builtin_expect(rare != 0ull, 0)) {
            if (__any(out)) {
#ifdef SSRS_PROBE_NO_STRAY_ATOMICS
                if (go && !in_a) ++win_stray;
                if (go && !in_b) ++win_stray;
#else
                if (go && !in_a) { atomicAdd(&a.hist[cell_a], 1u); ++win_stray; }
                if (go && !in_b) { atomicAdd(&a.hist[cell_b], 1u); ++win_stray; }
#endif
            }
            if (__any(slow)) {
                ++n_slow;
                if (slow) {
                    if (fast) { row = win_r0 + wr; col = win_c0 + wc; }
#pragma unroll 1
                    for (int h = 0; h < 2; ++h)
                        if (static_cast<uint32_t>(it + h - rel) < span) slow_step(h ? w4.z : w4.x, h ? w4.w : w4.y);
                    enter(true);
                }
            }
        }
        it += 2;
    };
    const uint32_t stop_stamp = static_cast<uint32_t>(a.launch) + 1u;
    uint32_t stop_seen = 0u;
    bool stopped = false;
    for (; it + 8 <= a.steps; ) {
        const unsigned long long stepping = __ballot(static_cast<uint32_t>(it - rel) < span), waiting = __ballot(it < rel && span != 0u);
        const bool stop_now = a.roam_stop && waiting == 0ull &&
                              static_cast<uint32_t>(__builtin_amdgcn_readfirstlane(static_cast<int>(stop_seen))) == stop_stamp;
        if (((stepping | waiting) == 0ull) | stop_now) { stopped = stop_now; break; }
        if (a.roam_stop) stop_seen = __hip_atomic_load(&ctl->roam_stop, __ATOMIC_RELAXED, __HIP_MEMORY_SCOPE_AGENT);
#pragma unroll
        for (int u = 0; u < 4; ++u) one_pair();
    }
    for (; it < a.steps && !stopped; ) {
        if (!__any(static_cast<uint32_t>(it - rel) < span || (it < rel && span != 0u))) break;
        one_pair();
    }
    if (a.roam_stop && !stopped && it >= a.steps && (threadIdx.x & 63) == 0) atomicMax(&ctl->roam_stop, stop_stamp);
    if (fast) { row = win_r0 + wr; col = win_c0 + wc; }
    {
        uint32_t nf = n_fine;
#pragma unroll
        for (int off = 32; off > 0; off >>= 1) nf += __shfl_down(nf, off);
        if ((threadIdx.x & 63) == 0 && nf) atomicAdd(&ctl->pad, nf);
    }
    if ((threadIdx.x & 63) == 0 && n_pairs) {
        atomicAdd(&ctl->roam_pairs, static_cast<unsigned long long>(n_pairs));
        if (n_slow) atomicAdd(&ctl->roam_slow, static_cast<unsigned long long>(n_slow));
        if (a.debug_roam) {
            const unsigned long long dt = __builtin_amdgcn_s_memtime() - t_begin;
            atomicAdd(&ctl->dbg_tsum, dt);
            atomicMax(&ctl->dbg_tmax, dt);
            atomicAdd(&ctl->dbg_waves, 1ull);
            atomicMax(&ctl->dbg_slowmax, (static_cast<unsigned long long>(n_slow) << 32) | n_pairs);
        }
    }
#ifdef SSRS_DEBUG_WAVE_DUMP
    if (a.debug_roam && a.launch == SSRS_DEBUG_WAVE_DUMP && a.dbg_buf) {
        const unsigned long long dt = __builtin_amdgcn_s_memtime() - t_begin;
        const int lanes = __popcll(__ballot(live0));
        uint32_t wst = win_stray;
        for (int off = 32; off > 0; off >>= 1) wst += __shfl_down(wst, off);
        if ((threadIdx.x & 63) == 0) {
            unsigned long long *r = a.dbg_buf + 8ull * (blockIdx.x * (BT / 64) + (threadIdx.x >> 6));
            r[0] = dt; r[1] = static_cast<unsigned long long>(lanes); r[2] = n_pairs; r[3] = n_slow; r[4] = wst;
            r[5] = static_cast<unsigned long long>(win_r0); r[6] = static_cast<unsigned long long>(win_c0);
            r[7] = static_cast<uint32_t>(__popcll(__ballot(fast)));
        }
    }
#endif
    __syncthreads();
    for (int q = threadIdx.x; q < kWinRows * kWinCols; q += BT) {
        const uint32_t n = s_win[q];
        if (n) atomicAdd(&a.hist[static_cast<uint32_t>(win_r0 + q / kWinCols) * ucols + static_cast<uint32_t>(win_c0 + q % kWinCols)], n);
    }
    {
        unsigned long long ws = win_stray;
#pragma unroll
        for (int off = 32; off > 0; off >>= 1) ws += __shfl_down(ws, off);
        if ((threadIdx.x & 63) == 0 && ws) atomicAdd(&ctl->strays, ws);
    }
    const bool active = live0 && span != 0u && k < static_cast<int>(a.max_k);
    if (live0 && !active) {
        if (a.lengths) a.lengths[t] = static_cast<int32_t>(k + 1);
        if (a.end_rc) reinterpret_cast<uint32_t *>(a.end_rc)[t] = (static_cast<uint32_t>(row) & 0xFFFFu) | (static_cast<uint32_t>(col) << 16);
    }
    __shared__ uint32_t s_surv[BT / 64 + 1];
    const int lane = threadIdx.x & 63, wv = threadIdx.x >> 6;
    const int nsurv = __popcll(__ballot(active));
    if (lane == 0) s_surv[wv] = static_cast<uint32_t>(nsurv);
    __syncthreads();
    if (threadIdx.x == 0) {
        uint32_t tot = 0;
        for (int q = 0; q < BT / 64; ++q) tot += s_surv[q];
        s_surv[BT / 64] = tot ? atomicAdd(&ctl->count[out_slot][xcd], static_cast<uint32_t>(BT)) : 0xFFFFFFFFu;
    }
    __syncthreads();
    const uint32_t basei = s_surv[BT / 64];
    if (basei != 0xFFFFFFFFu) {
        a.list_out[xcd * a.cap + basei + threadIdx.x] = active ? t : -1;
        if (active) {
            TrackState o;
            o.pos = static_cast<int32_t>((static_cast<uint32_t>(row) & 0xFFFFu) | (static_cast<uint32_t>(col) << 16));
            o.k = k;
            o.dirs = static_cast<uint32_t>(kKOfRing >> (4 * rc)) & 0xFu;
            o.aux = s.aux;
            a.state[t] = o;
        }
    }
    unsigned long long mv = live0 ? static_cast<unsigned long long>(k - s.k) : 0ull;
#pragma unroll
    for (int off = 32; off > 0; off >>= 1) mv += __shfl_down(mv, off);
    if (lane == 0 && mv) atomicAdd(&ctl->steps, mv);
}

constexpr int kBinThreads = 1024;
constexpr int kBinCells = 30720;
__global__ __launch_bounds__(kBinThreads) void k_bin_visits(const uint32_t *__restrict__ visits,
                                                           long long stride,
                                                           TrackCtl *__restrict__ ctl, int slot,
                                                           uint32_t *__restrict__ hist, int rows,
                                                           int cols, uint32_t cap)
{
    __shared__ uint32_t bins[kBinCells];
    __shared__ uint32_t s_first;
    uint32_t nslots[kXcd];
#pragma unroll
    for (int x = 0; x < kXcd; ++x) nslots[x] = (ctl->count[slot][x] + 63u) & ~63u;
    const uint32_t *v = visits + static_cast<long long>(blockIdx.x) * stride;
    const uint32_t ncell = static_cast<uint32_t>(rows) * cols;
    const int wrows = kBinCells / cols < 1 ? 0 : (kBinCells / cols > rows ? rows : kBinCells / cols);
    if (threadIdx.x == 0) s_first = 0xFFFFFFFFu;
    for (int k = threadIdx.x; k < wrows * cols; k += kBinThreads) bins[k] = 0;
    __syncthreads();
    uint32_t mn = 0xFFFFFFFFu;
    {
        const uint32_t x = threadIdx.x % kXcd;
        uint32_t nx = 0;
#pragma unroll
        for (int y = 0; y < kXcd; ++y) nx = (static_cast<uint32_t>(y) == x) ? nslots[y] : nx;
        for (uint32_t q = 0, j = threadIdx.x / kXcd; q < 4 && j < nx; ++q, j += kBinThreads / kXcd) {
            const uint32_t c = v[x * cap + j];
            mn = c < mn ? c : mn;
        }
    }
#pragma unroll
    for (int off = 32; off > 0; off >>= 1) {
        const uint32_t o = __shfl_down(mn, off);
        mn = o < mn ? o : mn;
    }
    if ((threadIdx.x & 63) == 0 && mn != 0xFFFFFFFFu) atomicMin(&s_first, mn);
    __syncthreads();
    if (s_first == 0xFFFFFFFFu) {
        __syncthreads();
        mn = 0xFFFFFFFFu;
#pragma unroll
        for (int x = 0; x < kXcd; ++x)
            for (uint32_t j = threadIdx.x; j < nslots[x]; j += kBinThreads) {
                const uint32_t c = v[x * cap + j];
                mn = c < mn ? c : mn;
            }
#pragma unroll
        for (int off = 32; off > 0; off >>= 1) {
            const uint32_t o = __shfl_down(mn, off);
            mn = o < mn ? o : mn;
        }
        if ((threadIdx.x & 63) == 0 && mn != 0xFFFFFFFFu) atomicMin(&s_first, mn);
        __syncthreads();
    }
    const uint32_t first = s_first;
    if (first == 0xFFFFFFFFu) return;
    uint32_t brow = first / cols;
    if (wrows >= 3 && brow > 0) --brow;
    const uint32_t base = brow * cols;
    const uint32_t wcells = static_cast<uint32_t>(wrows) * cols;
    uint32_t stray = 0;
    constexpr int kU = 16;
#pragma unroll
    for (int x = 0; x < kXcd; ++x)
        for (uint32_t j = threadIdx.x; j < nslots[x]; j += kBinThreads * kU) {
            uint32_t c[kU];
#pragma unroll
            for (int q = 0; q < kU; ++q) {
                const uint32_t jj = j + q * kBinThreads;
                c[q] = jj < nslots[x] ? v[x * cap + jj] : 0xFFFFFFFFu;
            }
#pragma unroll
            for (int q = 0; q < kU; ++q) {
                if (c[q] >= ncell) continue;
                const uint32_t off = c[q] - base;
                if (off < wcells) atomicAdd(&bins[off], 1u);
                else { atomicAdd(&hist[c[q]], 1u); ++stray; }
            }
        }
#pragma unroll
    for (int off = 32; off > 0; off >>= 1) stray += __shfl_down(stray, off);
    if ((threadIdx.x & 63) == 0 && stray) atomicAdd(&ctl->strays, static_cast<unsigned long long>(stray));
    __syncthreads();
    for (uint32_t k = threadIdx.x; k < wcells; k += kBinThreads * 4) {
        uint32_t n[4];
#pragma unroll
        for (int q = 0; q < 4; ++q) {
            const uint32_t kk = k + q * kBinThreads;
            n[q] = (kk < wcells && base + kk < ncell) ? bins[kk] : 0u;
        }
#pragma unroll
        for (int q = 0; q < 4; ++q)
            if (n[q]) atomicAdd(&hist[base + k + q * kBinThreads], n[q]);
    }
}


__global__ __launch_bounds__(kBinThreads) void k_bin_visits16(const uint16_t *__restrict__ visits, long long stride, int steps,
                                                             TrackCtl *__restrict__ ctl, int slot,
                                                             uint32_t *__restrict__ hist, int rows, int cols, uint32_t cap,
                                                             int v16_offset, long long it_base, uint32_t *host_out, int host_words)
{
    __shared__ uint32_t bins[kBinCells];
    uint32_t nslots[kXcd];
#pragma unroll
    for (int x = 0; x < kXcd; ++x) nslots[x] = (ctl->count[slot][x] + 63u) & ~63u;
    const int it0 = 2 * static_cast<int>(blockIdx.x);
    const long long base = (static_cast<long long>(ctl->par_min) - v16_offset + it_base + it0 - 1) * cols;
    const long long ncell = static_cast<long long>(rows) * cols;
    for (int k = threadIdx.x; k < kBinCells; k += kBinThreads) bins[k] = 0;
    __syncthreads();
    uint32_t stray = 0;
    constexpr int kU = 8;
    for (int sub = 0; sub < 2 && it0 + sub < steps; ++sub) {
        const uint16_t *v = visits + static_cast<long long>(it0 + sub) * stride;
        const uint32_t shift = sub ? static_cast<uint32_t>(cols) : 0u;
#pragma unroll
        for (int x = 0; x < kXcd; ++x) {
            const uint32_t *v2 = reinterpret_cast<const uint32_t *>(v + static_cast<size_t>(x) * cap);
            const uint32_t npair = nslots[x] / 2;
            for (uint32_t j = threadIdx.x; j < npair; j += kBinThreads * kU) {
                uint32_t c[kU];
#pragma unroll
                for (int q = 0; q < kU; ++q) {
                    const uint32_t jj = j + q * kBinThreads;
#ifdef SSRS_PROBE_K3_NOREAD
                    c[q] = jj < npair ? (jj * 2654435761u) % 24000u * 65537u : 0xFFFFFFFFu;
#else
                    c[q] = jj < npair ? v2[jj] : 0xFFFFFFFFu;
#endif
                }
#pragma unroll
                for (int q = 0; q < kU; ++q) {
#pragma unroll
                    for (int h = 0; h < 2; ++h) {
                        uint32_t key = h ? c[q] >> 16 : c[q] & 0xFFFFu;
                        if (key == 0xFFFFu) continue;
                        key += shift;
// ... 642 lines not shown
        if (support == 0 || (support & ~restriction(kRingK[rh])) != 0) continue;
        const uint32_t ord = ring_order(rh);
        const int ring3[3] = {(rh + 7) % 8, rh, (rh + 1) % 8};
        const int ka = kRingK[ring3[ord & 3u]], kb = kRingK[ring3[(ord >> 2) & 3u]];
        out->rev_ok = 1;
        out->rev_rc = static_cast<uint32_t>(rh);
        out->rev_e = thr_pack(thr[ka], thr[kb]);
    }
}

extern "C" int ssrs_build_flags(void)
{
#if defined(SSRS_PROBE_NO_PHILOX) || defined(SSRS_PROBE_NO_GATHER) || defined(SSRS_PROBE_K2A_NOLOAD) || \
    defined(SSRS_PROBE_K2A_NOSTORE) || defined(SSRS_PROBE_K2A_PAD) || defined(SSRS_K2A_NT) || \
    defined(SSRS_PROBE_K3_NOREAD) || defined(SSRS_PROBE_K3_NOFLUSH) || defined(SSRS_PROBE_NO_STRAY_ATOMICS)
    return 1;
#else
    return 0;
#endif
}

static void fine_prior_tables(const double *prior, FinePrior *out)
{
    *out = FinePrior{};
    for (int rc = 0; rc < 8; ++rc) {
        const uint32_t mask = restriction(kRingK[rc]);
        double q[9], qq[9], cdf[9];
        bool any = false;
        for (int k = 0; k < 9; ++k) {
            q[k] = ((mask >> k) & 1u) && k != 4 ? prior[k] : 0.0;
            any |= q[k] != 0.0;
        }
        if (!any) { out->reversal |= 1u << rc; continue; }
        const double s1 = sum9(q);
        for (int k = 0; k < 9; ++k) qq[k] = q[k] / s1;
        const double s2 = sum9(qq);
        double acc = 0.0;
        for (int k = 0; k < 9; ++k) { qq[k] = qq[k] / s2; acc = acc + qq[k]; cdf[k] = acc; }
        const uint32_t ord = ring_order(rc);
        const int ring3[3] = {(rc + 7) % 8, rc, (rc + 1) % 8};
        const int ka = kRingK[ring3[ord & 3u]], kb = kRingK[ring3[(ord >> 2) & 3u]];
        out->zero_t1[rc] = fine_fixed(cdf[ka] / cdf[8]);
        out->zero_t2[rc] = fine_fixed(cdf[kb] / cdf[8]);
        if (out->zero_t1[rc] > out->zero_t2[rc]) out->zero_t1[rc] = out->zero_t2[rc];
    }
}

extern "C" int ssrs_track_params_init(SsrsTrackParams *p, int rows, int cols,
                                      int memory_parameter, double scaling_parameter)
{
    SSRS_REQUIRE(p != nullptr, "ssrs_track_params_init: params is NULL");
    SSRS_REQUIRE(rows >= 5 && cols >= 5, "ssrs_track_params_init: need rows, cols >= 5");
    *p = SsrsTrackParams{};
    p->rows = rows;
    p->cols = cols;
    p->burnin = static_cast<int32_t>((rows < cols ? rows : cols) / 10.0);
    const double mm = rows / 2.0 * cols / 2.0;
    p->max_moves = static_cast<int64_t>(ceil(mm));
    p->memory_parameter = memory_parameter;
    p->scaling_parameter = scaling_parameter;
    return SSRS_OK;
}

extern "C" size_t ssrs_tracks_workspace_bytes(int64_t ntracks)
{
    if (ntracks < 0) ntracks = 0;
    return workspace_layout(ntracks, nullptr, nullptr);
}

static size_t pair_table_bytes(int64_t ntracks, int rows, int cols)
{
    if (ntracks < kWanderMinTracks || rows <= 0 || cols <= 0) return 0;
    const size_t cells = static_cast<size_t>(rows) * static_cast<size_t>(cols);
    return cells < kPairMaxCells ? align_up(cells * 8 * sizeof(RoamEntry), 256) + align_up(cells * 8 * sizeof(FineEntry), 256) : 0;
}

extern "C" size_t ssrs_tracks_workspace_bytes_ex(int64_t ntracks, int rows, int cols, int hist_copies)
{
    const size_t base = align_up(ssrs_tracks_workspace_bytes(ntracks), 256) + pair_table_bytes(ntracks, rows, cols);
    if (rows <= 0 || cols <= 0 || hist_copies < 2) return base;
    if (hist_copies > 64) hist_copies = 64;
    return base + static_cast<size_t>(hist_copies) * static_cast<size_t>(rows) * static_cast<size_t>(cols) * sizeof(uint32_t);
}

extern "C" int ssrs_transition_table_build(const double *updraft, const float *potential,
                                           double *table, int rows, int cols, void *stream)
{
    SSRS_REQUIRE(updraft && table, "ssrs_transition_table_build: updraft/table is NULL");
    SSRS_REQUIRE(rows >= 3 && cols >= 3, "ssrs_transition_table_build: need rows, cols >= 3");
    SSRS_REQUIRE((reinterpret_cast<uintptr_t>(table) & 63u) == 0,
                 "ssrs_transition_table_build: table must be 64-byte aligned");
    const int tx = (cols + kTabW - 1) / kTabW, ty = (rows + kTabH - 1) / kTabH, nt = tx * ty;
    hipLaunchKernelGGL(k_transition_table<false>, dim3(static_cast<unsigned>(nt)), dim3(kBlock), 0,
                       as_stream(stream), updraft, potential, static_cast<void *>(table), rows, cols, tx, nt);
    SSRS_HIP_CHECK(hipGetLastError());
    return SSRS_OK;
}

extern "C" size_t ssrs_transition_ring_bytes(int rows, int cols)
{
    if (rows <= 0 || cols <= 0) return 0;
    const size_t cells = static_cast<size_t>(rows) * static_cast<size_t>(cols);
    return ring_mask_offset(rows, cols) + (cells + 3) / 4 * 4;
}

extern "C" int ssrs_transition_ring_build(const double *updraft, const float *potential,
                                          float *ring, int rows, int cols, void *stream)
{
    SSRS_REQUIRE(updraft && ring, "ssrs_transition_ring_build: updraft/ring is NULL");
    SSRS_REQUIRE(rows >= 3 && cols >= 3, "ssrs_transition_ring_build: need rows, cols >= 3");
    SSRS_REQUIRE((reinterpret_cast<uintptr_t>(ring) & 7u) == 0,
                 "ssrs_transition_ring_build: ring must be 8-byte aligned");
    const int tx = (cols + kTabW - 1) / kTabW, ty = (rows + kTabH - 1) / kTabH, nt = tx * ty;
    hipLaunchKernelGGL(k_transition_table<true>, dim3(static_cast<unsigned>(nt)), dim3(kBlock), 0,
                       as_stream(stream), updraft, potential, static_cast<void *>(ring), rows, cols, tx, nt);
    SSRS_HIP_CHECK(hipGetLastError());
    return SSRS_OK;
}

static size_t thr_guard_bytes(int cols) { return align_up((static_cast<size_t>(cols) + 2) * 4, 256); }

extern "C" size_t ssrs_transition_thr_bytes(int rows, int cols)
{
    if (rows <= 0 || cols <= 0) return 0;
    return (static_cast<size_t>(8) << thr_plane_shift(rows, cols)) + 2 * thr_guard_bytes(cols);
}

extern "C" int ssrs_transition_thr_build(const double *updraft, const float *potential,
                                         const double *prior, float *thr, int rows, int cols, void *stream)
{
    SSRS_REQUIRE(updraft && thr && prior, "ssrs_transition_thr_build: updraft/prior/thr is NULL");
    SSRS_REQUIRE(rows >= 3 && cols >= 3, "ssrs_transition_thr_build: need rows, cols >= 3");
    SSRS_REQUIRE(static_cast<size_t>(rows) * static_cast<size_t>(cols) <= (1ull << 26),
                 "ssrs_transition_thr_build: the table and its guard bands are addressed with 32-bit offsets (rows * cols <= 2^26)");
    SSRS_REQUIRE((reinterpret_cast<uintptr_t>(thr) & 63u) == 0,
                 "ssrs_transition_thr_build: table must be 64-byte aligned");
    ThrPrior pr;
    prior_tables(prior, &pr);
    const int tx = (cols + kTabW - 1) / kTabW, ty = (rows + kTabH - 1) / kTabH, nt = tx * ty;
    uint32_t *planes = reinterpret_cast<uint32_t *>(reinterpret_cast<char *>(thr) + thr_guard_bytes(cols));
    ThrHeader *header = reinterpret_cast<ThrHeader *>(thr);
    PriorArg heading;
    for (int k = 0; k < 9; ++k) heading.v[k] = prior[k];
    if (potential)
        hipLaunchKernelGGL(k_transition_thr<true>, dim3(static_cast<unsigned>(nt)), dim3(kBlock), 0, as_stream(stream),
                           updraft, potential, planes, rows, cols, tx, nt, pr, thr_plane_shift(rows, cols), header, heading);
    else
        hipLaunchKernelGGL(k_transition_thr<false>, dim3(static_cast<unsigned>(nt)), dim3(kBlock), 0, as_stream(stream),
                           updraft, potential, planes, rows, cols, tx, nt, pr, thr_plane_shift(rows, cols), header, heading);
    SSRS_HIP_CHECK(hipGetLastError());
    return SSRS_OK;
}

extern "C" int ssrs_uniform_selftest(uint64_t seed, const uint64_t *track, const uint64_t *step,
                                     double *out, size_t n, void *stream)
{
    SSRS_REQUIRE(track && step && out, "ssrs_uniform_selftest: NULL pointer");
    if (n == 0) return SSRS_OK;
    hipLaunchKernelGGL(k_uniform_selftest, dim3(static_cast<unsigned>((n + 255) / 256)), dim3(256),
                       0, as_stream(stream), seed, track, step, out, n);
    SSRS_HIP_CHECK(hipGetLastError());
    return SSRS_OK;
}


struct TrackCall {
    const SsrsTrackParams *p;
    const double *updraft; const float *potential; const double *table;
    const int32_t *start_rc; int64_t ntracks; uint64_t seed, track_id_base;
    uint32_t *hist; int16_t *end_rc; int32_t *lengths; int16_t *traj; const int64_t *traj_offsets;
    void *workspace; size_t workspace_bytes; void *stream;
    SsrsTrajRecorder *rec;
    unsigned long long *hist64;
};

struct TrackSwitches {
    bool debug, debug_roam;
    bool roam_stop, cheap_exact, block_window, fine_table, roam_table, rev, deal_contiguous, rebalance, grow_steps;
    long long roam_wide_from;
    int roam_width;
    int roam_shuffle;
};

static TrackSwitches read_track_switches()
{
    auto set = [](const char *name) { return std::getenv(name) != nullptr; };
    TrackSwitches sw;
    sw.debug = set("SSRS_TRACKS_DEBUG");
    sw.debug_roam = set("SSRS_TRACKS_DEBUG_ROAM");
    sw.roam_stop = !set("SSRS_TRACKS_NO_ROAM_STOP");
    sw.cheap_exact = !set("SSRS_TRACKS_NO_CHEAP_EXACT");
    sw.block_window = !set("SSRS_TRACKS_NO_BLOCK_WINDOW");
    sw.fine_table = !set("SSRS_TRACKS_NO_FINE_TABLE");
    sw.roam_table = !set("SSRS_TRACKS_NO_ROAM_TABLE");
    sw.rev = !set("SSRS_TRACKS_NO_REV");
    sw.deal_contiguous = !set("SSRS_TRACKS_DEAL_ROUND_ROBIN");
    sw.rebalance = !set("SSRS_TRACKS_NO_REBALANCE");
    sw.grow_steps = !set("SSRS_TRACKS_FIXED_STEPS");
    sw.roam_wide_from = static_cast<long long>(kDealBlocks + kWanderWindows - 2) * kBlock + 1;
    if (const char *e = std::getenv("SSRS_TRACKS_ROAM_WIDE")) sw.roam_wide_from = std::atoll(e);
    sw.roam_width = 0;
    if (const char *e = std::getenv("SSRS_TRACKS_ROAM_WIDTH")) { const int w = std::atoi(e); if (w == 1 || w == 2 || w == 4) sw.roam_width = w; }
    sw.roam_shuffle = 16;
    if (const char *e = std::getenv("SSRS_TRACKS_ROAM_SHUFFLE")) sw.roam_shuffle = std::atoi(e);
    return sw;
}

static_assert(offsetof(TrackCtl, steps) == kSlotSteps * sizeof(uint32_t) &&
              offsetof(TrackCtl, strays) == kSlotSteps * sizeof(uint32_t) + sizeof(unsigned long long), "read-back slot");

struct TrackEvents {
    hipEvent_t first = nullptr, last = nullptr;
    hipEvent_t batch[kRing] = {};
    bool own_batch = false;
    std::vector<hipEvent_t> marks;
    std::vector<int> kind;
    TrackEvents() = default;
    TrackEvents(const TrackEvents &) = delete;
    TrackEvents &operator=(const TrackEvents &) = delete;
    ~TrackEvents()
    {
        for (hipEvent_t e : marks) (void)hipEventDestroy(e);
        if (own_batch)
            for (hipEvent_t e : batch)
                if (e) (void)hipEventDestroy(e);
        if (first) (void)hipEventDestroy(first);
        if (last) (void)hipEventDestroy(last);
    }
};

static int check_track_args(const TrackCall &c)
{
    const SsrsTrackParams *p = c.p;
    SSRS_REQUIRE(p != nullptr, "ssrs_tracks_simulate: params is NULL");
    SSRS_REQUIRE(c.hist64 == nullptr || c.hist != nullptr, "ssrs_tracks_simulate_h64: the 32-bit raster the kernels count into is NULL");
    SSRS_REQUIRE(p->rows >= 5 && p->cols >= 5, "ssrs_tracks_simulate: need rows, cols >= 5 (got %d x %d)",
                 p->rows, p->cols);
    SSRS_REQUIRE(p->rows <= 32767 && p->cols <= 32767,
                 "ssrs_tracks_simulate: rows, cols must fit int16 trajectories (<= 32767)");
    SSRS_REQUIRE(p->memory_parameter >= 0 && p->memory_parameter <= 8,
                 "ssrs_tracks_simulate: memory_parameter must be in 0..8 (got %d)",
                 p->memory_parameter);
    SSRS_REQUIRE(p->max_moves >= 0 && p->max_moves < (1ll << 31) - 1,
                 "ssrs_tracks_simulate: max_moves out of range");
    SSRS_REQUIRE(p->burnin >= 0, "ssrs_tracks_simulate: burnin must be >= 0");
    SSRS_REQUIRE(c.ntracks >= 0 && c.ntracks < (1ll << 31) - 64, "ssrs_tracks_simulate: bad ntracks");
    SSRS_REQUIRE(!(c.potential && !c.updraft && !c.table),
                 "ssrs_tracks_simulate: potential_field needs updraft_field (reference raises)");
    SSRS_REQUIRE(!(c.traj && !c.traj_offsets), "ssrs_tracks_simulate: traj needs traj_offsets");
    SSRS_REQUIRE(!(c.table && (reinterpret_cast<uintptr_t>(c.table) & 63u)),
                 "ssrs_tracks_simulate: table must be 64-byte aligned");
    return SSRS_OK;
}

struct TrackRun {
    const TrackCall c;
    const SsrsTrackParams *p;
    const TrackSwitches sw;
    hipStream_t st;
    Workspace ws = {};
    uint32_t *host_counts = nullptr;
    int S = 0, mode = 0, mode0 = 0;
    bool profile = false, coherent = false, lean = false, ring = false, thr = false;
    PlanGeom geom = {};
    ThrPrior thr_prior = {};
    StepArgs a = {};
    uint32_t ntc = 0, ntiles = 0;
    size_t ncell = 0;
    bool roam_ok = false, rev = false, wander_sort_ok = false, v16_ok = false;
    uint32_t *hist_t = nullptr;
    uint32_t *copies_ptr = nullptr;
    int ncopies = 0;
    bool copies_live = false;
    unsigned long long private_visits = 0;
    bool roam_ready = false;
    int roam_width = 1;
    TrackPolicy pol;
    int launch = 0, batches = 0, last_Sl = 0;
    long long it_done = 0;
    int window_launches = 0, tile_launches = 0, block_window_launches = 0, roam_launches = 0, roam_wide_launches = 0;
    int slot_row[kRing] = {};
    bool slot_block_window[kRing] = {};
    TrackEvents ev;
    bool marks_adjacent = false;

    explicit TrackRun(const TrackCall &call)
        : c(call), p(call.p), sw(read_track_switches()), st(as_stream(call.stream)) {}

    void mark(int kind)
    {
        hipEvent_t e;
        if (hipEventCreate(&e) != hipSuccess) return;
        (void)hipEventRecord(e, st);
        ev.marks.push_back(e);
        ev.kind.push_back(kind);
        marks_adjacent = true;
    }

    int check_thr_header();
    int plan_and_init();
    int choose_front_path();
    int launch_steps(bool first_move, unsigned blocks, uint32_t *vcap, long long *vstride) const;
    int record_launch(unsigned blocks, int Sl, bool bin_window, const uint32_t **rec_counts);
    void launch_stepper(bool first_move, bool v16, unsigned blocks, int Sl, bool *block_window);
    void bin_launch(unsigned blocks, int Sl, bool bin_window, bool bin_tiles, bool v16, const uint32_t *rec_counts,
                    uint32_t *read_back, bool *read_back_done);
    int wander_sort();
    void build_roam_tables();
    void rebalance();
    void fold_private(bool zero);
    int queue_batch();
    int examine_batches();
    int finish(int rc, SsrsTrackStats *stats);
};

int TrackRun::check_thr_header()
{
    SSRS_REQUIRE(c.table != nullptr, "ssrs_tracks_simulate: SSRS_TRACKS_THR_TABLE needs `table`");
    ThrHeader *hh = reinterpret_cast<ThrHeader *>(host_counts + kHeaderSlot);
    SSRS_HIP_CHECK(hipMemcpyAsync(hh, c.table, sizeof(ThrHeader), hipMemcpyDeviceToHost, st));
    SSRS_HIP_CHECK(hipStreamSynchronize(st));
    bool bad = hh->magic != kThrMagic || hh->rows != p->rows || hh->cols != p->cols;
    for (int k = 0; k < 9; ++k) bad |= hh->prior[k] != p->prior[k];
    if (bad)
        return set_error(SSRS_ERR_INVALID, "ssrs_tracks_simulate: `table` is not a threshold table built by "
                         "ssrs_transition_thr_build for this %d x %d raster and params->prior (nothing was launched)",
                         p->rows, p->cols);
    return SSRS_OK;
}

int TrackRun::plan_and_init()
{
    const int64_t ntracks = c.ntracks;
    SSRS_HIP_CHECK(hipEventCreate(&ev.first));
    SSRS_HIP_CHECK(hipEventCreate(&ev.last));
    SSRS_HIP_CHECK(hipEventRecord(ev.first, st));
    {
        PriorArg pa;
        for (int k = 0; k < 9; ++k) pa.v[k] = p->prior[k];
        const ThrHeader *header = (p->flags & SSRS_TRACKS_THR_TABLE) ? reinterpret_cast<const ThrHeader *>(c.table) : nullptr;
        hipLaunchKernelGGL(k_ctl_init, dim3(1), dim3(64), 0, st, ws.ctl, pa, ws.thr, ws.wander, header, p->rows, p->cols);
        SSRS_HIP_CHECK(hipGetLastError());
    }
    coherent = (p->flags & SSRS_TRACKS_NO_SCHEDULE) == 0;
    const unsigned blocks = static_cast<unsigned>((ntracks + kBlock - 1) / kBlock);
    if (coherent) {
        double vr = 0.0, vc = 0.0;
        for (int k = 0; k < 9; ++k) { vr += p->prior[k] * dr_of(k); vc += p->prior[k] * dc_of(k); }
        const double nrm = std::sqrt(vr * vr + vc * vc);
        geom.cos_t = nrm > 0.0 ? vr / nrm : 1.0;
        geom.sin_t = nrm > 0.0 ? vc / nrm : 0.0;
        geom.offset = p->rows + p->cols;
        int par_bits = 1;
        while ((1ll << par_bits) <= 2ll * geom.offset) ++par_bits;
        size_t temp_bytes = ws.sort_temp_bytes;
        if (2 * par_bits <= 32) {
            uint32_t *k0 = reinterpret_cast<uint32_t *>(ws.keys[0]), *k1 = reinterpret_cast<uint32_t *>(ws.keys[1]);
            hipLaunchKernelGGL(k_plan_keys<uint32_t>, dim3(blocks), dim3(kBlock), 0, st, c.start_rc,
                               static_cast<long long>(ntracks), geom, k0, ws.list[1], ws.ctl, par_bits);
            SSRS_HIP_CHECK(hipGetLastError());
            SSRS_HIP_CHECK(hipcub::DeviceRadixSort::SortPairs(
                ws.sort_temp, temp_bytes, k0, k1, ws.list[1], ws.list[0], static_cast<int>(ntracks), 0, 2 * par_bits, st));
        } else {
            hipLaunchKernelGGL(k_plan_keys<unsigned long long>, dim3(blocks), dim3(kBlock), 0, st, c.start_rc,
                               static_cast<long long>(ntracks), geom, ws.keys[0], ws.list[1], ws.ctl, par_bits);
            SSRS_HIP_CHECK(hipGetLastError());
            SSRS_HIP_CHECK(hipcub::DeviceRadixSort::SortPairs(
                ws.sort_temp, temp_bytes, ws.keys[0], ws.keys[1], ws.list[1], ws.list[0],
                static_cast<int>(ntracks), 0, 2 * par_bits, st));
        }
    }
    hipLaunchKernelGGL(k_tracks_init, dim3(blocks), dim3(kBlock), 0, st, c.start_rc,
                       static_cast<long long>(ntracks), p->rows, p->cols, c.hist, c.traj,
                       reinterpret_cast<const long long *>(c.traj_offsets), c.lengths, c.end_rc,
                       ws.state, ws.ctl, geom, coherent ? 1 : 0, ws.cap);
    SSRS_HIP_CHECK(hipGetLastError());

    S = p->steps_per_launch > 0 ? p->steps_per_launch : 512;
    profile = (p->flags & SSRS_TRACKS_PROFILE) != 0;
    mode = c.table ? MODE_TABLE : (c.updraft ? (c.potential ? MODE_FLUIDFLOW : MODE_UPDRAFT) : MODE_PRIOR);
    mode0 = c.updraft ? (c.potential ? MODE_FLUIDFLOW : MODE_UPDRAFT) : MODE_PRIOR;
    a.rows = p->rows; a.cols = p->cols; a.burnin = p->burnin; a.memory = p->memory_parameter;
    a.max_k = p->max_moves; a.nu = p->scaling_parameter;
    a.prior = ws.ctl->prior;
    a.updraft = c.updraft; a.potential = c.potential; a.table = c.table;
    a.seed = c.seed; a.track_base = c.track_id_base;
    a.hist = c.hist; a.end_rc = c.end_rc; a.lengths = c.lengths; a.traj = c.traj;
    a.traj_off = reinterpret_cast<const long long *>(c.traj_offsets);
    a.state = ws.state; a.ctl = ws.ctl; a.steps = S;
    a.fast = ((p->flags & SSRS_TRACKS_EXACT_ONLY) == 0 && p->scaling_parameter == 1.0) ? 1 : 0;
    a.coherent = coherent ? 1 : 0;
    a.cap = ws.cap;
    a.thr = ws.thr;
    a.wander = ws.wander;
    a.debug_roam = sw.debug_roam ? 1 : 0;
    a.roam_stop = sw.roam_stop ? 1 : 0;
    a.dbg_buf = nullptr;
#ifdef SSRS_DEBUG_WAVE_DUMP
    {
        static unsigned long long *dump_buf = nullptr;
        if (!dump_buf && a.debug_roam && hipMalloc(&dump_buf, 8ull * 8 * 4096 * (kBlock / 64)) != hipSuccess) dump_buf = nullptr;
        if (dump_buf) (void)hipMemsetAsync(dump_buf, 0, 8ull * 8 * 4096 * (kBlock / 64), st);
        a.dbg_buf = dump_buf;
    }
#endif
    a.cheap_exact = sw.cheap_exact ? 1 : 0;
    a.vcap = ws.cap;
    lean = p->memory_parameter == 1 && c.traj == nullptr;
    ring = (p->flags & SSRS_TRACKS_RING_TABLE) != 0;
    thr = (p->flags & SSRS_TRACKS_THR_TABLE) != 0;
    if (thr) {
        SSRS_REQUIRE(!ring && c.table && c.updraft && lean && a.fast && (S & 1) == 0,
                     "ssrs_tracks_simulate: SSRS_TRACKS_THR_TABLE needs table + updraft, memory_parameter 1, "
                     "scaling_parameter 1, no direct trajectory output, no EXACT_ONLY and an even steps_per_launch");
        SSRS_REQUIRE(static_cast<size_t>(p->rows) * static_cast<size_t>(p->cols) <= (1ull << 26),
                     "ssrs_tracks_simulate: the threshold table needs rows * cols <= 2^26");
        prior_tables(p->prior, &thr_prior);
        a.plane_shift = thr_plane_shift(p->rows, p->cols);
        a.guard = static_cast<uint32_t>(thr_guard_bytes(p->cols));
        a.pf_dir = coherent ? (geom.cos_t > 0.98 ? 1 : (geom.cos_t < -0.98 ? -1 : 0)) : 0;
        a.pf_rc = a.pf_dir < 0 ? 4 : 0;
    }
    if (ring)
        SSRS_REQUIRE(c.table && c.updraft && lean && a.fast && (S & 1) == 0,
                     "ssrs_tracks_simulate: SSRS_TRACKS_RING_TABLE needs table + updraft, memory_parameter 1, "
                     "scaling_parameter 1, no trajectory output, no EXACT_ONLY and an even steps_per_launch");
    return SSRS_OK;
}

int TrackRun::choose_front_path()
{
    const int64_t ntracks = c.ntracks;
    uint32_t *const hist = c.hist;
    const double off_axis = std::fabs(geom.sin_t) < std::fabs(geom.cos_t) ? std::fabs(geom.sin_t) : std::fabs(geom.cos_t);
    ntc = static_cast<uint32_t>((p->cols + kTileCols - 1) / kTileCols);
    ntiles = ntc * static_cast<uint32_t>((p->rows + kTileRows - 1) / kTileRows);
    const bool tiles_ok = hist != nullptr && coherent && S <= kVisitSteps && ntracks >= 8192 && ntiles <= kTilesMax &&
                          static_cast<unsigned long long>(ws.cap) * kXcd * static_cast<unsigned long long>(S) < (1ull << 32) &&
                          (p->flags & SSRS_TRACKS_NO_BINNING) == 0;
    bool tiles_on = tiles_ok && off_axis > 0.17;
    const bool want_transposed = coherent && !tiles_on && std::fabs(geom.sin_t) > std::fabs(geom.cos_t);
    const bool binning = hist != nullptr && coherent && S <= kVisitSteps &&
                         (p->flags & SSRS_TRACKS_NO_BINNING) == 0 &&
                         (want_transposed ? p->rows : p->cols) <= kBinCells;
    a.visits = nullptr;
    a.visit_stride = ws.visit_stride;
    bool binning_on = binning && ntracks >= 8192 && !tiles_on;
    const bool never_scattered = (p->flags & SSRS_TRACKS_NO_SCATTERED) != 0;
    const bool scattered = (p->flags & SSRS_TRACKS_SCATTERED) != 0;
    if (scattered) binning_on = tiles_on = false;
    const bool cache_ok = thr && hist != nullptr && !(c.rec && c.rec->complete) && sw.block_window;
    size_t ws_base = align_up(ssrs_tracks_workspace_bytes(ntracks), 256);
    {
        const size_t pb = thr ? pair_table_bytes(ntracks, p->rows, p->cols) : 0;
        if (pb && c.workspace_bytes >= ws_base + pb) {
            ws.roam = reinterpret_cast<RoamEntry *>(static_cast<char *>(c.workspace) + ws_base);
            if (sw.fine_table)
                a.fine = static_cast<char *>(c.workspace) + ws_base +
                         align_up(static_cast<size_t>(p->rows) * static_cast<size_t>(p->cols) * 8 * sizeof(RoamEntry), 256);
            ws_base += pb;
        }
        a.roam = ws.roam;
    }
    roam_ok = cache_ok && ws.roam != nullptr && sw.roam_table;
    rev = thr_prior.rev_ok != 0 && sw.rev;
    wander_sort_ok = ntracks >= kWanderMinTracks &&
                     static_cast<long long>((p->rows + kBinRows - 1) / kBinRows) * ((p->cols + kBinCols - 1) / kBinCols) <= kWanderBins;
    ncell = static_cast<size_t>(p->rows) * static_cast<size_t>(p->cols);
    if (hist && c.workspace_bytes > ws_base) ncopies = static_cast<int>((c.workspace_bytes - ws_base) / (ncell * sizeof(uint32_t)));
    uint32_t *extra = reinterpret_cast<uint32_t *>(static_cast<char *>(c.workspace) + ws_base);
    if (want_transposed && binning_on) {
        if (ncopies >= 1) { hist_t = extra; extra += ncell; --ncopies; }
        else binning_on = false;
    }
    if (hist_t) SSRS_HIP_CHECK(hipMemsetAsync(hist_t, 0, sizeof(uint32_t) * ncell, st));
    ncopies = ncopies > 64 ? 64 : ncopies;
    copies_ptr = ncopies >= 2 ? extra : nullptr;
    a.hist_copies = nullptr;
    a.ncopies = 1;
    a.zmask = ring ? reinterpret_cast<const uint8_t *>(c.table) + ring_mask_offset(p->rows, p->cols) : nullptr;
    v16_ok = 5ll * p->cols <= kBinCells;
    a.v16_offset = geom.offset;

    pol.thr = thr; pol.tiles_ok = tiles_ok; pol.cache_ok = cache_ok; pol.never_scattered = never_scattered;
    pol.front = a.pf_dir != 0; pol.may_rebalance = sw.rebalance; pol.debug = sw.debug; pol.roam_shuffle = sw.roam_shuffle;
    pol.ntracks = ntracks; pol.crossing = p->rows + p->cols;
    pol.binning_on = binning_on; pol.tiles_on = tiles_on; pol.scattered = scattered;
    pol.cached = cache_ok && scattered;
    pol.want_wander_sort = pol.cached;
    pol.upper = static_cast<uint32_t>(ntracks < static_cast<int64_t>(ws.cap) ? ntracks : ws.cap);
    ev.own_batch = !profile;
    if (!profile)
        for (int i = 0; i < kRing; ++i) SSRS_HIP_CHECK(hipEventCreate(&ev.batch[i]));
    return SSRS_OK;
}

int TrackRun::launch_steps(bool first_move, unsigned blocks, uint32_t *vcap, long long *vstride) const
{
    *vcap = ws.cap;
    *vstride = ws.visit_stride;
    if (first_move) return 1;
    const bool recording = c.rec && c.rec->complete;
    if (thr && pol.cached && !recording && sw.grow_steps) {
        return (roam_ok && roam_ready && pol.stable_roam >= 2) ? 128 * S : 8 * S;
    }
    if (thr && (pol.binning_on || pol.tiles_on) && !recording && sw.grow_steps) {
        const uint32_t vc = (blocks / kXcd) * kBlock;
        const long long room = (ws.visit_stride * kVisitSteps) / (static_cast<long long>(kXcd) * vc);
        long long grown = room < 8ll * S ? room : 8ll * S;
        grown &= ~1ll;
        if (grown >= S + S / 4) {
            *vcap = vc;
            *vstride = static_cast<long long>(kXcd) * vc;
            return static_cast<int>(grown);
        }
    }
    return S;
}

int TrackRun::record_launch(unsigned blocks, int Sl, bool bin_window, const uint32_t **rec_counts)
{
    SsrsTrajRecorder *rec = c.rec;
    const uint32_t vcap = (blocks / kXcd) * kBlock;
    const bool identity = a.list_in == nullptr;
    const size_t list_bytes = identity ? 0 : align_up(sizeof(int32_t) * kXcd * static_cast<size_t>(vcap), 256);
    const size_t vis_bytes = align_up(sizeof(uint32_t) * kXcd * static_cast<size_t>(vcap) * static_cast<size_t>(Sl), 256);
    const size_t need = 256 + list_bytes + vis_bytes;
    if (rec->bytes - rec->used < need) {
        rec->complete = 0;
        return SSRS_OK;
    }
    char *base = rec->pool + rec->used;
    rec->used += need;
    TrajChunk ch = {};
    ch.counts = reinterpret_cast<const uint32_t *>(base);
    ch.list = identity ? nullptr : reinterpret_cast<const int32_t *>(base + 256);
    ch.visits = reinterpret_cast<const uint32_t *>(base + 256 + list_bytes);
    ch.vcap = vcap;
    ch.cap = ws.cap;
    ch.steps = Sl;
    ch.transposed = (hist_t && bin_window) ? 1 : 0;
    hipError_t e1 = hipMemcpyAsync(base, ws.ctl->count[launch & 3], kXcd * sizeof(uint32_t),
                                   hipMemcpyDeviceToDevice, st);
    hipError_t e2 = identity ? hipSuccess
                             : hipMemcpy2DAsync(base + 256, sizeof(int32_t) * vcap, a.list_in,
                                                sizeof(int32_t) * ws.cap, sizeof(int32_t) * vcap, kXcd,
                                                hipMemcpyDeviceToDevice, st);
    if (e1 != hipSuccess || e2 != hipSuccess) return set_error(SSRS_ERR_HIP, "trajectory record copy failed");
    rec->chunks.push_back(ch);
    marks_adjacent = false;
    a.visits = const_cast<uint32_t *>(ch.visits);
    a.visit_stride = static_cast<long long>(kXcd) * vcap;
    a.vcap = vcap;
    *rec_counts = ch.counts;
    return SSRS_OK;
}

void TrackRun::launch_stepper(bool first_move, bool v16, unsigned blocks, int Sl, bool *block_window)
{
    const bool binning_on = pol.binning_on, tiles_on = pol.tiles_on, scattered = pol.scattered;
    switch (first_move ? mode0 : mode) {
    case MODE_TABLE:
        if (thr) {
            const bool pf = a.pf_dir != 0 && a.coherent && !scattered && !tiles_on;
            if (v16) {
                hipLaunchKernelGGL((k_step_thr<4, true>), dim3(blocks), dim3(kBlock + 64), 0, st, a, thr_prior);
                return;
            }
            if (pol.cached && !a.visits) {
                ++block_window_launches;
                *block_window = true;
                if (roam_ok && roam_ready) {
                    ++roam_launches;
                    if (roam_width > 1) {
                        const unsigned bt = static_cast<unsigned>(roam_width) * kBlock;
                        const unsigned wblocks = kXcd * ((pol.upper + bt - 1) / bt);
                        ++roam_wide_launches;
                        if (roam_width == 2) {
                            if (rev) hipLaunchKernelGGL((k_step_roam<true, 2 * kBlock>), dim3(wblocks), dim3(bt), 0, st, a, thr_prior);
                            else hipLaunchKernelGGL((k_step_roam<false, 2 * kBlock>), dim3(wblocks), dim3(bt), 0, st, a, thr_prior);
                        } else {
                            if (rev) hipLaunchKernelGGL((k_step_roam<true, 4 * kBlock>), dim3(wblocks), dim3(bt), 0, st, a, thr_prior);
                            else hipLaunchKernelGGL((k_step_roam<false, 4 * kBlock>), dim3(wblocks), dim3(bt), 0, st, a, thr_prior);
                        }
                    } else if (rev) hipLaunchKernelGGL(k_step_roam<true>, dim3(blocks), dim3(kBlock), 0, st, a, thr_prior);
                    else hipLaunchKernelGGL(k_step_roam<false>, dim3(blocks), dim3(kBlock), 0, st, a, thr_prior);
#ifdef SSRS_DEBUG_WAVE_DUMP
                    if (a.debug_roam && launch == SSRS_DEBUG_WAVE_DUMP && a.dbg_buf) {
                        std::vector<unsigned long long> rec(8ull * blocks * (kBlock / 64));
                        (void)hipStreamSynchronize(st);
                        (void)hipMemcpy(rec.data(), a.dbg_buf, rec.size() * 8, hipMemcpyDeviceToHost);
                        for (uint32_t w = 0; w < blocks * (kBlock / 64); ++w) {
                            const unsigned long long *r = &rec[8ull * w];
                            fprintf(stderr, "W %u %u %llu %llu %llu %llu %llu %lld %lld %llu\n", w / (kBlock / 64), w % (kBlock / 64), r[1], r[0], r[2], r[3], r[4],
                                    static_cast<long long>(r[5]), static_cast<long long>(r[6]), r[7]);
                        }
                    }
#endif
                    if (a.debug_roam) {
                        TrackCtl cb;
                        (void)hipMemcpyAsync(&host_counts[kFinalSlot], ws.ctl, sizeof(TrackCtl), hipMemcpyDeviceToHost, st);
                        (void)hipStreamSynchronize(st);
                        memcpy(&cb, &host_counts[kFinalSlot], sizeof(TrackCtl));
                        if (cb.dbg_waves)
                            fprintf(stderr, "[roam] launch %d blocks %u Sl %d: %llu waves, mean %.0f clk, max %.0f clk (x%.2f); slowest-by-slow-pairs wave: %llu of %llu pairs slow\n",
                                    launch, blocks, Sl, cb.dbg_waves, static_cast<double>(cb.dbg_tsum) / cb.dbg_waves, static_cast<double>(cb.dbg_tmax),
                                    static_cast<double>(cb.dbg_tmax) * cb.dbg_waves / static_cast<double>(cb.dbg_tsum), cb.dbg_slowmax >> 32, cb.dbg_slowmax & 0xFFFFFFFFull);
                        (void)hipMemsetAsync(&ws.ctl->dbg_tsum, 0, 4 * sizeof(unsigned long long), st);
                    }
                    return;
                }
                if (rev) hipLaunchKernelGGL((k_step_thr<6, false, true>), dim3(blocks), dim3(kBlock), 0, st, a, thr_prior);
                else hipLaunchKernelGGL((k_step_thr<6>), dim3(blocks), dim3(kBlock), 0, st, a, thr_prior);
                return;
            }
            if (a.visits && hist_t && binning_on) hipLaunchKernelGGL((k_step_thr<2>), dim3(blocks), dim3(kBlock), 0, st, a, thr_prior);
            else if (a.visits && pf) hipLaunchKernelGGL((k_step_thr<1, true>), dim3(blocks), dim3(kBlock + 64), 0, st, a, thr_prior);
            else if (a.visits && rev) hipLaunchKernelGGL((k_step_thr<1, false, true>), dim3(blocks), dim3(kBlock), 0, st, a, thr_prior);
            else if (a.visits) hipLaunchKernelGGL((k_step_thr<1>), dim3(blocks), dim3(kBlock), 0, st, a, thr_prior);
            else if (a.hist && pf) hipLaunchKernelGGL((k_step_thr<3, true>), dim3(blocks), dim3(kBlock + 64), 0, st, a, thr_prior);
            else if (a.hist && rev) hipLaunchKernelGGL((k_step_thr<3, false, true>), dim3(blocks), dim3(kBlock), 0, st, a, thr_prior);
            else if (a.hist) hipLaunchKernelGGL((k_step_thr<3>), dim3(blocks), dim3(kBlock), 0, st, a, thr_prior);
            else if (pf) hipLaunchKernelGGL((k_step_thr<0, true>), dim3(blocks), dim3(kBlock + 64), 0, st, a, thr_prior);
            else if (rev) hipLaunchKernelGGL((k_step_thr<0, false, true>), dim3(blocks), dim3(kBlock), 0, st, a, thr_prior);
            else hipLaunchKernelGGL((k_step_thr<0>), dim3(blocks), dim3(kBlock), 0, st, a, thr_prior);
            return;
        }
        if (ring && scattered && !binning_on && !tiles_on) hipLaunchKernelGGL((k_step_lean<true, true>), dim3(blocks), dim3(kBlock), 0, st, a);
        else if (ring && hist_t && binning_on) hipLaunchKernelGGL((k_step_lean<true, false, true>), dim3(blocks), dim3(kBlock), 0, st, a);
        else if (ring) hipLaunchKernelGGL((k_step_lean<true, false>), dim3(blocks), dim3(kBlock), 0, st, a);
        else if (lean && a.fast && (S & 1) == 0 && hist_t && binning_on) hipLaunchKernelGGL((k_step_lean<false, false, true>), dim3(blocks), dim3(kBlock), 0, st, a);
        else if (lean && a.fast && (S & 1) == 0) hipLaunchKernelGGL((k_step_lean<false, false>), dim3(blocks), dim3(kBlock), 0, st, a);
        else hipLaunchKernelGGL(k_step_tracks<MODE_TABLE>, dim3(blocks), dim3(kBlock), 0, st, a);
        return;
    case MODE_FLUIDFLOW: hipLaunchKernelGGL(k_step_tracks<MODE_FLUIDFLOW>, dim3(blocks), dim3(kBlock), 0, st, a); return;
    case MODE_UPDRAFT: hipLaunchKernelGGL(k_step_tracks<MODE_UPDRAFT>, dim3(blocks), dim3(kBlock), 0, st, a); return;
    default: hipLaunchKernelGGL(k_step_tracks<MODE_PRIOR>, dim3(blocks), dim3(kBlock), 0, st, a); return;
    }
}

void TrackRun::bin_launch(unsigned blocks, int Sl, bool bin_window, bool bin_tiles, bool v16, const uint32_t *rec_counts,
                          uint32_t *read_back, bool *read_back_done)
{
    uint32_t *const hist = c.hist;
    if (bin_window) {
        ++window_launches;
        if (v16) {
            hipLaunchKernelGGL(k_bin_visits16, dim3((Sl + 1) / 2), dim3(kBinThreads), 0, st, reinterpret_cast<const uint16_t *>(a.visits),
                               a.visit_stride, Sl, ws.ctl, launch & 3, hist, p->rows, p->cols, a.vcap, a.v16_offset, a.it_base,
                               read_back, kSlotWords);
            *read_back_done = read_back != nullptr;
        }
        else if (hist_t)
            hipLaunchKernelGGL(k_bin_visits, dim3(Sl), dim3(kBinThreads), 0, st, a.visits, a.visit_stride,
                               ws.ctl, launch & 3, hist_t, p->cols, p->rows, a.vcap);
        else
            hipLaunchKernelGGL(k_bin_visits, dim3(Sl), dim3(kBinThreads), 0, st, a.visits, a.visit_stride,
                               ws.ctl, launch & 3, hist, p->rows, p->cols, a.vcap);
        if (profile && !*read_back_done) mark(2);
    }
    if (bin_tiles) {
        ++tile_launches;
        const double inv_cols = 1.0 / static_cast<double>(p->cols);
        const uint32_t ucols = static_cast<uint32_t>(p->cols), ucell = static_cast<uint32_t>(ncell);
        (void)hipMemsetAsync(ws.tile_count, 0, sizeof(uint32_t) * ntiles, st);
        hipLaunchKernelGGL((k_tile_sort<false>), dim3(blocks, kStepSplit), dim3(kBlock), 0, st, a.visits, a.visit_stride, Sl,
                           ws.ctl, launch & 3, ucols, inv_cols, ucell, a.vcap, ntc, ntiles, ws.tile_count,
                           ws.tile_cursor, ws.bucket);
        hipLaunchKernelGGL(k_tile_scan, dim3(1), dim3(kTileThreads), 0, st, ws.tile_count, ntiles, ws.tile_start,
                           ws.tile_cursor, ws.item_start);
        hipLaunchKernelGGL((k_tile_sort<true>), dim3(blocks, kStepSplit), dim3(kBlock), 0, st, a.visits, a.visit_stride, Sl,
                           ws.ctl, launch & 3, ucols, inv_cols, ucell, a.vcap, ntc, ntiles, ws.tile_count,
                           ws.tile_cursor, ws.bucket);
        const unsigned long long max_visits = static_cast<unsigned long long>(blocks) * kBlock * Sl;
        const unsigned items = static_cast<unsigned>(max_visits / kItemVisits) + ntiles;
        hipLaunchKernelGGL(k_bin_bucket, dim3(items), dim3(kTileThreads), 0, st, ws.bucket, ws.tile_start,
                           ws.tile_count, ws.ctl, hist, static_cast<uint32_t>(p->rows), ucols, inv_cols, ntc,
                           ntiles, ws.item_start);
        if (profile) mark(2);
    }
    if (rec_counts && hist && !bin_window && !bin_tiles) {
        hipLaunchKernelGGL(k_count_visits, dim3(blocks), dim3(kBlock), 0, st, a.visits, a.vcap, Sl, rec_counts, hist,
                           static_cast<uint32_t>(ncell));
        marks_adjacent = false;
    }
}

int TrackRun::wander_sort()
{
    const uint32_t slots = ws.cap * kXcd;
    uint32_t *k0 = reinterpret_cast<uint32_t *>(ws.keys[0]), *k1 = reinterpret_cast<uint32_t *>(ws.keys[1]);
    int32_t *sorted = reinterpret_cast<int32_t *>(ws.bucket);
    hipLaunchKernelGGL(k_wander_windows, dim3(1), dim3(1024), 0, st, ws.list[launch & 1], ws.state, ws.ctl, launch & 3, ws.cap,
                       p->rows, p->cols, ws.wander);
    hipLaunchKernelGGL(k_wander_keys, dim3((slots + kBlock - 1) / kBlock), dim3(kBlock), 0, st, ws.list[launch & 1], ws.state,
                       ws.ctl, launch & 3, ws.cap, ws.wander, k0, pol.sort_is_periodic ? static_cast<uint32_t>(launch) : 0u);
    size_t temp_bytes = ws.sort_temp_bytes;
    if (hipcub::DeviceRadixSort::SortPairs(ws.sort_temp, temp_bytes, k0, k1, ws.list[launch & 1], sorted,
                                           static_cast<int>(slots), 0, 13, st) != hipSuccess)
        return set_error(SSRS_ERR_HIP, "wander sort failed");
    roam_width = 1;
    if (roam_ok && sw.deal_contiguous) {
        if (sw.roam_wide_from == 1) {
            roam_width = 2;
        } else if (sw.roam_wide_from > 1 && static_cast<long long>(pol.prev_total) >= sw.roam_wide_from) {
            uint32_t *word = &host_counts[kFinalSlot];
            if (hipMemcpyAsync(word, &ws.ctl->deal_live, sizeof(uint32_t), hipMemcpyDeviceToHost, st) != hipSuccess ||
                hipStreamSynchronize(st) != hipSuccess)
                return set_error(SSRS_ERR_HIP, "live-count read-back at the deal failed");
            if (static_cast<long long>(*word) >= sw.roam_wide_from) roam_width = 2;
        }
        if (sw.roam_width) roam_width = sw.roam_width;
    }
    hipLaunchKernelGGL(k_deal_sorted, dim3(64), dim3(1024), 0, st, k1, sorted, ws.list[(launch + 1) & 1], ws.ctl,
                       (launch + 1) & 3, (launch + 2) & 3, ws.cap, sw.deal_contiguous ? 1 : 0, roam_width);
    ++launch;
    marks_adjacent = false;
    pol.dealt(batches, ws.cap, sw.deal_contiguous, roam_width);
    return SSRS_OK;
}

void TrackRun::build_roam_tables()
{
    const char *tabc = reinterpret_cast<const char *>(c.table);
    const unsigned grid = 256 * 16;
    if (rev) hipLaunchKernelGGL(k_roam_build<true>, dim3(grid), dim3(kBlock), 0, st, tabc, a.guard, a.plane_shift, p->rows, p->cols,
                                ws.roam, thr_prior);
    else hipLaunchKernelGGL(k_roam_build<false>, dim3(grid), dim3(kBlock), 0, st, tabc, a.guard, a.plane_shift, p->rows, p->cols,
                            ws.roam, thr_prior);
    if (a.fine) {
        FinePrior fp;
        fine_prior_tables(p->prior, &fp);
        const int tx = (p->cols + kTabW - 1) / kTabW, ty = (p->rows + kTabH - 1) / kTabH, nt = tx * ty;
        FineEntry *fine_out = reinterpret_cast<FineEntry *>(const_cast<void *>(a.fine));
        if (c.potential) hipLaunchKernelGGL(k_fine_build<true>, dim3(static_cast<unsigned>(nt)), dim3(kBlock), 0, st, c.updraft, c.potential,
                                            fine_out, p->rows, p->cols, tx, nt, fp);
        else hipLaunchKernelGGL(k_fine_build<false>, dim3(static_cast<unsigned>(nt)), dim3(kBlock), 0, st, c.updraft, c.potential,
                                fine_out, p->rows, p->cols, tx, nt, fp);
    }
    roam_ready = true;
    marks_adjacent = false;
}

void TrackRun::rebalance()
{
    hipLaunchKernelGGL(k_rebalance_lists, dim3(1), dim3(1024), 0, st, ws.list[launch & 1], ws.list[(launch + 1) & 1],
                       ws.ctl, launch & 3, (launch + 1) & 3, (launch + 2) & 3, ws.cap);
    marks_adjacent = false;
    ++launch;
    pol.rebalanced();
}

int TrackRun::queue_batch()
{
    const int depth = (thr && last_Sl >= 512 && launch < 24) ? 1 : kBatch;
    const int slot = batches % kRing;
    bool read_back_done = false;
    bool batch_block_window = false;
    for (int j = 0; j < depth; ++j, ++launch) {
        a.launch = launch;
        a.list_in = (launch == 0 && !coherent) ? nullptr : ws.list[launch & 1];
        a.list_out = ws.list[(launch + 1) & 1];
        const bool first_move = thr && launch == 0;
        const unsigned blocks = kXcd * ((pol.upper + kBlock - 1) / kBlock);
        uint32_t vcap_l;
        long long vstride_l;
        const int Sl = launch_steps(first_move, blocks, &vcap_l, &vstride_l);
        if (sw.debug && (launch < 40 || launch % 500 == 0))
            fprintf(stderr, "[tracks] launch %d upper %u blocks %u Sl %d binning %d tiles %d scattered %d cached %d cap %u\n", launch, pol.upper, blocks, Sl,
                    pol.binning_on ? 1 : 0, pol.tiles_on ? 1 : 0, pol.scattered ? 1 : 0, pol.cached ? 1 : 0, ws.cap);
        a.steps = Sl;
        a.coherent = (coherent && !first_move) ? 1 : 0;
        a.it_base = thr && launch > 0 ? it_done : 0;
        a.visits = nullptr;
        if (!pol.binning_on && pol.scattered && copies_ptr && !copies_live && !pol.cached) {
            if (hipMemsetAsync(copies_ptr, 0, sizeof(uint32_t) * ncell * ncopies, st) != hipSuccess)
                return set_error(SSRS_ERR_HIP, "histogram copies memset failed");
            copies_live = true;
            marks_adjacent = false;
            a.hist_copies = copies_ptr;
            a.ncopies = ncopies;
        }
        if (c.hist64 && (copies_live || hist_t)) {
            const unsigned long long bound = static_cast<unsigned long long>(c.ntracks) * static_cast<unsigned long long>(Sl + 1);
            if (private_visits && private_visits + bound > 0xFFFFFFFFull) fold_private(true);
            private_visits += bound;
        }
        const bool bin_window = pol.binning_on && !first_move, bin_tiles = pol.tiles_on && !first_move;
        const bool transposed = hist_t && bin_window;
        a.vis_r = transposed ? 1u : static_cast<uint32_t>(p->cols);
        a.vis_c = transposed ? static_cast<uint32_t>(p->rows) : 1u;
        if (bin_window || bin_tiles) a.visits = ws.visits;
        a.visit_stride = vstride_l;
        a.vcap = vcap_l;
        const uint32_t *rec_counts = nullptr;
        if (c.rec && c.rec->complete) {
            const int rc = record_launch(blocks, Sl, bin_window, &rec_counts);
            if (rc != SSRS_OK) return rc;
        }
        if (profile && !marks_adjacent) mark(0);
        const bool v16 = thr && bin_window && a.visits == ws.visits && a.pf_dir == 1 && !hist_t && v16_ok &&
                         (it_done + Sl + 2ll * geom.offset) * p->cols < (1ll << 31);
        bool is_block_window = false;
        launch_stepper(first_move, v16, blocks, Sl, &is_block_window);
        batch_block_window |= is_block_window;
        if (profile) mark(is_block_window ? 3 : 1);
        uint32_t *read_back = j == depth - 1 ? &host_counts[kSlotWords * slot] : nullptr;
        bin_launch(blocks, Sl, bin_window, bin_tiles, v16, rec_counts, read_back, &read_back_done);
        if (thr && !first_move) it_done += Sl;
        last_Sl = Sl;
        if (hipGetLastError() != hipSuccess) return set_error(SSRS_ERR_HIP, "stepper launch failed");
    }
    if (c.hist64 && (batches & 1)) {
        hipLaunchKernelGGL(k_drain64, dim3(4096), dim3(kBlock), 0, st, c.hist, c.hist64, ncell);
        marks_adjacent = false;
    }
    bool queued = read_back_done || hipMemcpyAsync(&host_counts[kSlotWords * slot], ws.ctl, kSlotWords * sizeof(uint32_t),
                                                   hipMemcpyDeviceToHost, st) == hipSuccess;
    if (queued && profile) {
        const size_t before = ev.marks.size();
        mark(read_back_done ? 2 : 0);
        queued = ev.marks.size() > before;
        if (queued) ev.batch[slot] = ev.marks.back();
    } else if (queued) {
        queued = hipEventRecord(ev.batch[slot], st) == hipSuccess;
        marks_adjacent = false;
    }
    if (!queued) return set_error(SSRS_ERR_HIP, "live-count read-back failed");
    slot_row[slot] = launch & 3;
    slot_block_window[slot] = batch_block_window;
    ++batches;
    return SSRS_OK;
}

int TrackRun::examine_batches()
{
    while (pol.checked < batches - 1 && !pol.finished) {
        const int cs = pol.checked % kRing;
        if (hipEventSynchronize(ev.batch[cs]) != hipSuccess) return set_error(SSRS_ERR_HIP, "event sync failed");
        pol.examine(&host_counts[kSlotWords * cs], slot_row[cs], slot_block_window[cs], batches, it_done,
                    static_cast<long long>(launch) * S, roam_ready);
    }
    return SSRS_OK;
}

void TrackRun::fold_private(bool zero)
{
    if (copies_live) {
        if (zero) hipLaunchKernelGGL((k_fold_copies<unsigned long long, true>), dim3(4096), dim3(kBlock), 0, st, copies_ptr, ncopies, ncell, c.hist64);
        else hipLaunchKernelGGL((k_fold_copies<unsigned long long, false>), dim3(4096), dim3(kBlock), 0, st, copies_ptr, ncopies, ncell, c.hist64);
    }
    if (hist_t) {
        hipLaunchKernelGGL(k_transpose_add<unsigned long long>, dim3(static_cast<unsigned>(((p->rows + 31) / 32) * ((p->cols + 31) / 32))),
                           dim3(kBlock), 0, st, hist_t, p->rows, p->cols, c.hist64);
        if (zero) (void)hipMemsetAsync(hist_t, 0, sizeof(uint32_t) * ncell, st);
    }
    private_visits = 0;
    marks_adjacent = false;
}

int TrackRun::finish(int rc, SsrsTrackStats *stats)
{
    uint32_t *const hist = c.hist;
    if (rc != SSRS_OK) {
        (void)hipStreamSynchronize(st);
        return rc;
    }
    if (c.hist64) {
        fold_private(false);
        hipLaunchKernelGGL(k_drain64, dim3(4096), dim3(kBlock), 0, st, hist, c.hist64, ncell);
    } else {
        if (copies_live)
            hipLaunchKernelGGL((k_fold_copies<uint32_t, false>), dim3(4096), dim3(kBlock), 0, st, copies_ptr, ncopies, ncell, hist);
        if (hist_t)
            hipLaunchKernelGGL(k_transpose_add<uint32_t>, dim3(static_cast<unsigned>(((p->rows + 31) / 32) * ((p->cols + 31) / 32))),
                               dim3(kBlock), 0, st, hist_t, p->rows, p->cols, hist);
    }
    (void)hipEventRecord(ev.last, st);
    TrackCtl host_ctl = {};
    if (hipMemcpyAsync(&host_counts[kFinalSlot], ws.ctl, sizeof(TrackCtl), hipMemcpyDeviceToHost, st) != hipSuccess ||
        hipStreamSynchronize(st) != hipSuccess)
        return set_error(SSRS_ERR_HIP, "final read-back failed");
    memcpy(&host_ctl, &host_counts[kFinalSlot], sizeof(TrackCtl));
    if (stats) {
        stats->total_steps = static_cast<int64_t>(host_ctl.steps);
        stats->launches = launch;
        stats->window_launches = window_launches;
        stats->tile_launches = tile_launches;
        stats->block_window_launches = block_window_launches;
        stats->wander_sorts = pol.wander_sorts;
        stats->roam_launches = roam_launches;
        stats->roam_shuffles = pol.roam_shuffles;
        stats->roam_wide_launches = roam_wide_launches;
        stats->roam_wave_pairs = static_cast<int64_t>(host_ctl.roam_pairs);
        stats->roam_slow_wave_pairs = static_cast<int64_t>(host_ctl.roam_slow);
        stats->reserved0 = static_cast<int32_t>(host_ctl.pad);
        stats->block_window_steps = pol.block_window_steps;
        float ms = 0.f;
        if (hipEventElapsedTime(&ms, ev.first, ev.last) == hipSuccess) stats->wall_ms = ms;
        if (profile) {
            float sum = 0.f, hsum = 0.f;
            int timed = 0;
            for (size_t i = 1; i < ev.marks.size(); ++i) {
                if (ev.kind[i] == 0 || hipEventElapsedTime(&ms, ev.marks[i - 1], ev.marks[i]) != hipSuccess) continue;
                if (ev.kind[i] == 1 || ev.kind[i] == 3) {
                    sum += ms;
                    if (timed == 0 && thr) stats->first_move_ms = ms;
                    ++timed;
                    if (ev.kind[i] == 3) { stats->block_window_ms += ms; ++stats->block_window_timed; }
                } else {
                    hsum += ms;
                }
            }
            stats->timed_launches = timed;
            stats->kernel_ms = sum;
            stats->hist_ms = hsum;
        }
    }
    if (host_ctl.error & 2u)
        return set_error(SSRS_ERR_INVALID, "ssrs_tracks_simulate: `table` is not a threshold table built by "
                         "ssrs_transition_thr_build for this %d x %d raster and params->prior (results discarded)",
                         p->rows, p->cols);
    if (host_ctl.error)
        return set_error(SSRS_ERR_START, "ssrs_tracks_simulate: a start cell lies outside the %d x %d raster",
                         p->rows, p->cols);
    return SSRS_OK;
}

static int tracks_simulate_impl(const TrackCall &c, SsrsTrackStats *stats)
{
    int rc = check_track_args(c);
    if (rc != SSRS_OK) return rc;
    if (stats) *stats = SsrsTrackStats{};
    if (SsrsTrajRecorder *rec = c.rec) {
        rec->used = 0;
        rec->chunks.clear();
        rec->complete = 1;
        rec->rows = c.p->rows;
        rec->cols = c.p->cols;
        rec->ntracks = c.ntracks;
    }
    if (c.ntracks == 0) return SSRS_OK;
    SSRS_REQUIRE(c.start_rc != nullptr, "ssrs_tracks_simulate: start_rc is NULL");
    SSRS_REQUIRE(c.workspace && c.workspace_bytes >= ssrs_tracks_workspace_bytes(c.ntracks),
                 "ssrs_tracks_simulate: workspace too small (need %zu bytes)",
                 ssrs_tracks_workspace_bytes(c.ntracks));
    SSRS_REQUIRE((reinterpret_cast<uintptr_t>(c.workspace) & 255u) == 0,
                 "ssrs_tracks_simulate: workspace must be 256-byte aligned");

    TrackRun run(c);
    workspace_layout(c.ntracks, static_cast<char *>(c.workspace), &run.ws);
    run.host_counts = pinned_counts();
    SSRS_REQUIRE(run.host_counts != nullptr, "ssrs_tracks_simulate: hipHostMalloc failed");
    if (c.p->flags & SSRS_TRACKS_THR_TABLE) {
        if ((rc = run.check_thr_header()) != SSRS_OK) return rc;
    }
    if ((rc = run.plan_and_init()) != SSRS_OK) return rc;
    if ((rc = run.choose_front_path()) != SSRS_OK) return rc;
    TrackPolicy &pol = run.pol;
    while (!pol.finished && rc == SSRS_OK) {
        if (pol.want_wander_sort && pol.cached && run.wander_sort_ok && run.launch > 0) {
            if ((rc = run.wander_sort()) != SSRS_OK) break;
        }
        if (pol.cached) pol.want_rebalance = false;
        if (pol.cached && run.roam_ok && !run.roam_ready) run.build_roam_tables();
        if (pol.want_rebalance && run.launch > 0) run.rebalance();
        rc = run.queue_batch();
        if (rc == SSRS_OK) rc = run.examine_batches();
    }
    return run.finish(rc, stats);
}

extern "C" int ssrs_tracks_simulate(const SsrsTrackParams *p, const double *updraft,
                                    const float *potential, const double *table,
                                    const int32_t *start_rc, int64_t ntracks, uint64_t seed,
                                    uint64_t track_id_base, uint32_t *hist, int16_t *end_rc,
                                    int32_t *lengths, int16_t *traj, const int64_t *traj_offsets,
                                    void *workspace, size_t workspace_bytes,
                                    SsrsTrackStats *stats, void *stream)
{
    return tracks_simulate_impl({p, updraft, potential, table, start_rc, ntracks, seed, track_id_base, hist, end_rc,
                                 lengths, traj, traj_offsets, workspace, workspace_bytes, stream, nullptr, nullptr}, stats);
}

extern "C" int ssrs_tracks_simulate_h64(const SsrsTrackParams *p, const double *updraft,
                                        const float *potential, const double *table,
                                        const int32_t *start_rc, int64_t ntracks, uint64_t seed,
                                        uint64_t track_id_base, uint32_t *hist_scratch, uint64_t *hist64, int16_t *end_rc,
                                        int32_t *lengths, void *workspace, size_t workspace_bytes,
                                        SsrsTrackStats *stats, void *stream)
{
    SSRS_REQUIRE(hist_scratch != nullptr && hist64 != nullptr, "ssrs_tracks_simulate_h64: NULL histogram");
    static_assert(sizeof(unsigned long long) == sizeof(uint64_t), "64-bit counts");
    return tracks_simulate_impl({p, updraft, potential, table, start_rc, ntracks, seed, track_id_base, hist_scratch, end_rc,
                                 lengths, nullptr, nullptr, workspace, workspace_bytes, stream, nullptr,
                                 reinterpret_cast<unsigned long long *>(hist64)}, stats);
}

extern "C" SsrsTrajRecorder *ssrs_traj_recorder_create(void *pool, size_t pool_bytes)
{
    if (!pool || (reinterpret_cast<uintptr_t>(pool) & 255u)) {
        set_error(SSRS_ERR_INVALID, "ssrs_traj_recorder_create: pool must be non-NULL and 256-byte aligned");
        return nullptr;
    }
    SsrsTrajRecorder *rec = new (std::nothrow) SsrsTrajRecorder();
    if (!rec) { set_error(SSRS_ERR_INVALID, "ssrs_traj_recorder_create: out of host memory"); return nullptr; }
    rec->pool = static_cast<char *>(pool);
    rec->bytes = pool_bytes;
    rec->used = 0;
    rec->complete = 0;
    rec->rows = rec->cols = 0;
    rec->ntracks = -1;
    return rec;
}

extern "C" void ssrs_traj_recorder_destroy(SsrsTrajRecorder *rec) { delete rec; }

extern "C" int ssrs_traj_recorder_complete(const SsrsTrajRecorder *rec) { return rec ? rec->complete : 0; }

extern "C" size_t ssrs_traj_recorder_used(const SsrsTrajRecorder *rec) { return rec ? rec->used : 0; }

extern "C" int ssrs_tracks_simulate_rec(const SsrsTrackParams *p, const double *updraft,
                                        const float *potential, const double *table,
                                        const int32_t *start_rc, int64_t ntracks, uint64_t seed,
                                        uint64_t track_id_base, uint32_t *hist, int16_t *end_rc,
                                        int32_t *lengths, SsrsTrajRecorder *recorder,
                                        void *workspace, size_t workspace_bytes,
                                        SsrsTrackStats *stats, void *stream)
{
    SSRS_REQUIRE(recorder != nullptr, "ssrs_tracks_simulate_rec: recorder is NULL");
    return tracks_simulate_impl({p, updraft, potential, table, start_rc, ntracks, seed, track_id_base, hist, end_rc,
                                 lengths, nullptr, nullptr, workspace, workspace_bytes, stream, recorder, nullptr}, stats);
}

extern "C" int ssrs_tracks_gather(const SsrsTrajRecorder *rec, const int32_t *start_rc, int64_t ntracks,
                                  const int64_t *traj_offsets, int16_t *traj, void *cursor_ws,
                                  size_t cursor_bytes, void *stream)
{
    SSRS_REQUIRE(rec != nullptr, "ssrs_tracks_gather: recorder is NULL");
    SSRS_REQUIRE(rec->complete, "ssrs_tracks_gather: the record is incomplete (pool exhausted or no simulation yet)");
    SSRS_REQUIRE(ntracks == rec->ntracks, "ssrs_tracks_gather: ntracks differs from the recorded simulation");
    if (ntracks == 0) return SSRS_OK;
    SSRS_REQUIRE(start_rc && traj_offsets && traj && cursor_ws, "ssrs_tracks_gather: NULL pointer");
    SSRS_REQUIRE(cursor_bytes >= sizeof(uint32_t) * static_cast<size_t>(ntracks),
                 "ssrs_tracks_gather: cursor scratch too small (4 bytes per track)");
    hipStream_t st = as_stream(stream);
    uint32_t *cursor = static_cast<uint32_t *>(cursor_ws);
    const long long *off = reinterpret_cast<const long long *>(traj_offsets);
    hipLaunchKernelGGL(k_gather_init, dim3(static_cast<unsigned>((ntracks + kBlock - 1) / kBlock)), dim3(kBlock), 0, st,
                       start_rc, static_cast<long long>(ntracks), off, traj, cursor);
    for (const TrajChunk &ch : rec->chunks)
        hipLaunchKernelGGL(k_gather_chunk, dim3(kXcd * (ch.vcap / kBlock)), dim3(kBlock), 0, st, ch,
                           static_cast<uint32_t>(rec->rows), static_cast<uint32_t>(rec->cols), off, traj, cursor);
    SSRS_HIP_CHECK(hipGetLastError());
    return SSRS_OK;
}
```

ssrs_amd/movmodel.py:

```python
import ctypes as C
import os
import threading
from math import floor, ceil

import numpy as np
import torch

from . import _native as nat
from ._device import device, stream_ptr, to_dev, is_tensor

neighbour_deltas = [np.array([k // 3 - 1, k % 3 - 1]) for k in range(9)]
neighbour_delta_norms_inv = np.array(
    [[1 / np.sqrt(2.), 1., 1 / np.sqrt(2.)], [1., 0., 1.],
     [1 / np.sqrt(2.), 1., 1 / np.sqrt(2.)]], dtype=np.float32)


def get_starting_indices(ntracks, sbounds, stype, twidth, tres):
    if (sbounds[1] < sbounds[0] or sbounds[3] < sbounds[2] or sbounds[0] < 0.
            or sbounds[2] < 0. or sbounds[1] > twidth[0] or sbounds[3] > twidth[1]):
        raise ValueError('track_start_region incompatible with terrain_width!')
    res_km = tres / 1000.
    x_max = ceil(twidth[0] / res_km)
    y_max = ceil(twidth[1] / res_km)
    x_lo = min(max(floor(sbounds[0] / res_km) - 1, 1), x_max - 2)
# ... 189 lines not shown
                    scaling_parameter=1., updraft_field=None, potential_field=None, *,
                    seed=0, track_id_base=0, table=None, use_table=None, hist=None,
                    want_hist=True, want_tracks=False, steps_per_launch=0, profile=False,
                    exact_only=False, schedule=True, binning=True, ring=None, scattered=None,
                    max_moves=None, record=True, record_pool_bytes=None, thr=None, traj_budget_bytes=None, hist64=False):
    rows, cols = int(grid_shape[0]), int(grid_shape[1])
    dev = device()
    st = to_dev(np.asarray(starts) if not is_tensor(starts) else starts, torch.int32)
    st = st.reshape(-1, 2).contiguous()
    n = int(st.shape[0])
    upd = to_dev(updraft_field, torch.float64)
    pot = to_dev(potential_field, torch.float32)
    for name, f in (('updraft_field', upd), ('potential_field', pot)):
        if f is not None and tuple(f.shape) != (rows, cols):
            raise ValueError(f'{name} shape {tuple(f.shape)} != grid_shape {(rows, cols)}')
    if pot is not None and upd is None:
        raise ValueError('potential_field needs updraft_field')
    two_pass = bool(want_tracks) and not record
    if table is None and upd is not None:
        if use_table is None:
            use_table = n * max(rows, cols) >= rows * cols // 64 or n >= 4096
        if use_table:
            f32_ok = ring_table_applies(memory_parameter, scaling_parameter, two_pass,
                                        exact_only, steps_per_launch)
            if thr is None:
                thr = f32_ok and ring is None and rows * cols < THR_MAX_CELLS
            if ring is None:
                ring = f32_ok and not thr
            table = build_transition_table(upd, pot, ring=bool(ring) and not thr, thr=bool(thr),
                                           move_dirn=move_dirn)
    kind = table_kind(table, rows, cols)
    is_thr = kind == 'thr'
    is_ring = kind in ('ring', 'thr')
    if is_ring and not ring_table_applies(memory_parameter, scaling_parameter, two_pass,
                                          exact_only, steps_per_launch):
        raise ValueError('the ring table needs memory_parameter 1, scaling_parameter 1, no '
                         'two-pass trajectory output, exact_only=False and an even steps_per_launch')
    p = make_track_params((rows, cols), move_dirn, memory_parameter, scaling_parameter,
                          steps_per_launch, profile, exact_only, schedule, binning,
                          ring=is_ring and not is_thr, scattered=scattered, thr=is_thr)
    if max_moves is not None:
        p.max_moves = int(max_moves)
    hist_scratch = None
    if hist64:
        if want_tracks:
            raise ValueError('hist64 goes with want_tracks=False')
        if hist is None:
            hist = torch.zeros((rows, cols), dtype=torch.int64, device=dev)
        elif hist.dtype != torch.int64:
            raise ValueError('hist64=True: `hist` must be an int64 tensor')
        hist_scratch = torch.zeros((rows, cols), dtype=torch.int32, device=dev)
    if hist is None and want_hist:
        hist = torch.zeros((rows, cols), dtype=torch.int32, device=dev)
    lengths = torch.empty(n, dtype=torch.int32, device=dev)
    ends = torch.empty((n, 2), dtype=torch.int16, device=dev)
    copies = 0
    if hist is not None:
        copies = int(min(64, (4 << 30) // (rows * cols * 4)))
        copies = copies if copies >= 2 else 0
    ws_bytes = nat.lib().ssrs_tracks_workspace_bytes_ex(n, rows, cols, copies)
    ws = _workspace(ws_bytes, dev)
    stats = nat.SsrsTrackStats()

    def run(hist_t, traj_t, off_t):
        nat.check(nat.lib().ssrs_tracks_simulate(
            C.byref(p), nat.ptr(upd), nat.ptr(pot), nat.ptr(table), nat.ptr(st),
            C.c_int64(n), C.c_uint64(int(seed) & 0xFFFFFFFFFFFFFFFF),
            C.c_uint64(int(track_id_base)), nat.ptr(hist_t), nat.ptr(ends),
            nat.ptr(lengths), nat.ptr(traj_t), nat.ptr(off_t), nat.ptr(ws),
            C.c_size_t(ws_bytes), C.byref(stats), stream_ptr()))

    traj = offsets = None
    recorded = simulated = False
    if traj_budget_bytes is None:
        traj_budget_bytes = min(16 << 30, torch.cuda.mem_get_info()[0] // 3)
    if want_tracks and record and n > 0:
        pool_bytes = int(record_pool_bytes) if record_pool_bytes is not None else \
            default_record_pool_bytes(n, rows, cols)
        pool = torch.empty(max(256, pool_bytes // 256 * 256), dtype=torch.uint8, device=dev)
        rec = nat.lib().ssrs_traj_recorder_create(nat.ptr(pool), C.c_size_t(pool.numel()))
        if not rec:
            nat.check(nat.SSRS_ERR_INVALID)
        try:
            nat.check(nat.lib().ssrs_tracks_simulate_rec(
                C.byref(p), nat.ptr(upd), nat.ptr(pot), nat.ptr(table), nat.ptr(st),
                C.c_int64(n), C.c_uint64(int(seed) & 0xFFFFFFFFFFFFFFFF),
                C.c_uint64(int(track_id_base)), nat.ptr(hist), nat.ptr(ends),
                nat.ptr(lengths), C.c_void_p(rec), nat.ptr(ws), C.c_size_t(ws_bytes),
                C.byref(stats), stream_ptr()))
            if nat.lib().ssrs_traj_recorder_complete(C.c_void_p(rec)) and \
                    int(lengths.sum(dtype=torch.int64).item()) * 4 <= int(traj_budget_bytes):
                offsets = torch.zeros(n + 1, dtype=torch.int64, device=dev)
                torch.cumsum(lengths, 0, out=offsets[1:])
                total = int(offsets[-1].item())
                traj = torch.empty((total, 2), dtype=torch.int16, device=dev)
                cursor = torch.empty(n, dtype=torch.int32, device=dev)
                nat.check(nat.lib().ssrs_tracks_gather(
                    C.c_void_p(rec), nat.ptr(st), C.c_int64(n), nat.ptr(offsets), nat.ptr(traj),
                    nat.ptr(cursor), C.c_size_t(4 * n), stream_ptr()))
                torch.cuda.current_stream().synchronize()
                recorded = True
            simulated = True
        finally:
            nat.lib().ssrs_traj_recorder_destroy(C.c_void_p(rec))
            del pool
        if not recorded and is_ring:
            table = build_transition_table(upd, pot, ring=False)
            p = make_track_params((rows, cols), move_dirn, memory_parameter, scaling_parameter,
                                  steps_per_launch, profile, exact_only, schedule, binning, ring=False,
                                  scattered=scattered)
            if max_moves is not None:
                p.max_moves = int(max_moves)
    replay = None
    if want_tracks and not recorded:
        if not simulated:
            run(hist, None, None)
        offsets = torch.zeros(n + 1, dtype=torch.int64, device=dev)
        torch.cumsum(lengths, 0, out=offsets[1:])
        total = int(offsets[-1].item())
        if total * 4 <= int(traj_budget_bytes):
            traj = torch.empty((total, 2), dtype=torch.int16, device=dev)
            run(None, traj, offsets)
        else:
            offsets = None
            two_table, two_p = table, p

            def replay(t0, t1):
                sub = st[t0:t1].contiguous()
                m = t1 - t0
                sub_len = torch.empty(m, dtype=torch.int32, device=dev)
                sub_end = torch.empty((m, 2), dtype=torch.int16, device=dev)
                off = torch.zeros(m + 1, dtype=torch.int64, device=dev)
                torch.cumsum(lengths[t0:t1], 0, out=off[1:])
                out = torch.empty((int(off[-1].item()), 2), dtype=torch.int16, device=dev)
                wsb = nat.lib().ssrs_tracks_workspace_bytes(m)
                wss = torch.empty(wsb, dtype=torch.uint8, device=dev)
                st2 = nat.SsrsTrackStats()
                nat.check(nat.lib().ssrs_tracks_simulate(
                    C.byref(two_p), nat.ptr(upd), nat.ptr(pot), nat.ptr(two_table), nat.ptr(sub),
                    C.c_int64(m), C.c_uint64(int(seed) & 0xFFFFFFFFFFFFFFFF),
                    C.c_uint64(int(track_id_base) + t0), None, nat.ptr(sub_end), nat.ptr(sub_len),
                    nat.ptr(out), nat.ptr(off), nat.ptr(wss), C.c_size_t(wsb), C.byref(st2), stream_ptr()))
                if not torch.equal(sub_len, lengths[t0:t1]):
                    raise RuntimeError('trajectory replay: a track changed its length between the passes')
                return out, off
    elif hist64:
        nat.check(nat.lib().ssrs_tracks_simulate_h64(
            C.byref(p), nat.ptr(upd), nat.ptr(pot), nat.ptr(table), nat.ptr(st),
            C.c_int64(n), C.c_uint64(int(seed) & 0xFFFFFFFFFFFFFFFF),
            C.c_uint64(int(track_id_base)), nat.ptr(hist_scratch), nat.ptr(hist), nat.ptr(ends),
            nat.ptr(lengths), nat.ptr(ws), C.c_size_t(ws_bytes), C.byref(stats), stream_ptr()))
    elif not want_tracks:
        run(hist, None, None)
    return TrackBatch(lengths, ends, hist, traj, offsets, replay=replay, stats=
                      dict(total_steps=int(stats.total_steps), launches=int(stats.launches),
                           kernel_ms=float(stats.kernel_ms), wall_ms=float(stats.wall_ms),
                           hist_ms=float(stats.hist_ms), window_launches=int(stats.window_launches),
                           tile_launches=int(stats.tile_launches),
                           block_window_launches=int(stats.block_window_launches),
                           wander_sorts=int(stats.wander_sorts), timed_launches=int(stats.timed_launches),
                           first_move_ms=float(stats.first_move_ms), recorded=bool(recorded),
                           traj_chunk_bytes=int(traj_budget_bytes),
                           block_window_ms=float(stats.block_window_ms),
                           block_window_timed=int(stats.block_window_timed),
                           block_window_steps=int(stats.block_window_steps),
                           roam_launches=int(stats.roam_launches),
                           roam_fine_settled=int(stats.reserved0),
                           roam_wave_pairs=int(stats.roam_wave_pairs),
                           roam_slow_wave_pairs=int(stats.roam_slow_wave_pairs),
                           roam_shuffles=int(stats.roam_shuffles),
                           roam_wide_launches=int(stats.roam_wide_launches)))


def generate_simulated_tracks(move_dirn, start_location, grid_shape, memory_parameter=1,
                              scaling_parameter=1., updraft_field=None, potential_field=None,
                              *, seed=0, track_id=0):
    res = simulate_tracks(move_dirn, [list(start_location)], grid_shape, memory_parameter,
                          scaling_parameter, updraft_field, potential_field, seed=seed,
                          track_id_base=track_id, use_table=False, want_hist=False,
                          want_tracks=True)
    return res.tracks()[0]


def uniforms(seed, track, step):
    tr = to_dev(np.asarray(track, dtype=np.uint64).view(np.int64), torch.int64).reshape(-1)
    sp = to_dev(np.asarray(step, dtype=np.uint64).view(np.int64), torch.int64).reshape(-1)
    if tr.numel() != sp.numel():
        raise ValueError('track and step lengths differ')
    out = torch.empty(tr.numel(), dtype=torch.float64, device=tr.device)
    nat.check(nat.lib().ssrs_uniform_selftest(
        C.c_uint64(int(seed) & 0xFFFFFFFFFFFFFFFF), nat.ptr(tr), nat.ptr(sp), nat.ptr(out),
        C.c_size_t(tr.numel()), stream_ptr()))
    return out.cpu().numpy()


from .presence import (compute_presence_counts, compute_smooth_presence_counts)
from . import potential as _potential


class MovModel:

    def __init__(self, move_dirn, grid_shape):
        self.move_dirn = move_dirn
        self.grid_shape = grid_shape

    def get_boundary_nodes(self):
        return _potential.get_boundary_nodes(self.move_dirn, self.grid_shape)

    def assemble_sparse_linear_system(self):
        return None, None, None

    def solve_sparse_linear_system(self, conductivity, bnodes=None, benergy=None,
                                   row_inds=None, col_inds=None, facs=None, **kwargs):
        return _potential.solve_potential(conductivity, self.move_dirn, **kwargs)
```

Before: 74130.

## Add feeder waves that precompute Philox random words for roam kernel

Launches the narrow roam kernel with twice as many threads. The extra waves act as producers: they compute packed Philox random words ahead of time into an LDS ring buffer, and worker waves consume them with a tag handshake, falling back to computing the words themselves when a slot is not ready. Worker waves get raised scheduling priority. The aim is to take RNG arithmetic off the critical path of the stepping loop. The default shuffle setting also changes when feeding is enabled. The cost is doubled block size, extra LDS use, spin-waiting feeder waves, and recomputing the full Philox block on slow steps.

```diff
diff --git a/include/ssrs_hip.h b/include/ssrs_hip.h
--- a/include/ssrs_hip.h
+++ b/include/ssrs_hip.h
@@ -350,6 +350,12 @@
                           const uint64_t *step, double *out, size_t n,
                           void *stream);
 
+int ssrs_roam_pair_word_selftest(uint64_t seed, const uint64_t *track,
+                                 const uint64_t *block, uint32_t *packed,
+                                 uint32_t *words, size_t n, void *stream);
+
+void ssrs_tracks_roam_feed_counts(int64_t *fed, int64_t *own);
+
 #ifdef __cplusplus
 }
 #endif
diff --git a/ssrs_amd/_native.py b/ssrs_amd/_native.py
--- a/ssrs_amd/_native.py
+++ b/ssrs_amd/_native.py
@@ -49,6 +49,7 @@
     'ssrs_projection_init_albers', 'ssrs_warp_lonlat_raster',
     'ssrs_allen_workspace_bytes', 'ssrs_allen_thermal_field',
     'ssrs_track_occupancy_workspace_bytes', 'ssrs_track_occupancy',
+    'ssrs_roam_pair_word_selftest', 'ssrs_tracks_roam_feed_counts',
 )
 
 
@@ -198,6 +199,9 @@
         L.ssrs_track_occupancy_workspace_bytes.restype = C.c_size_t
         L.ssrs_track_occupancy_workspace_bytes.argtypes = [C.c_int, C.c_int, C.c_int]
         L.ssrs_track_occupancy.argtypes = OCCUPANCY_ARGTYPES
+        L.ssrs_roam_pair_word_selftest.argtypes = [C.c_uint64] + [C.c_void_p] * 4 + [C.c_size_t, C.c_void_p]
+        L.ssrs_tracks_roam_feed_counts.restype = None
+        L.ssrs_tracks_roam_feed_counts.argtypes = [C.POINTER(C.c_int64), C.POINTER(C.c_int64)]
         _lib = L
     return _lib
 
diff --git a/ssrs_amd/csrc/tracks.hip b/ssrs_amd/csrc/tracks.hip
--- a/ssrs_amd/csrc/tracks.hip
+++ b/ssrs_amd/csrc/tracks.hip
@@ -207,6 +207,22 @@
     const bool same = w.x == v.x && w.y == v.y && w.z == v.z && w.w == v.w;
     const double u = (step[i] & 1) ? words_to_uniform(w.z, w.w) : words_to_uniform(w.x, w.y);
     out[i] = same ? u : __longlong_as_double(0x7FF8000000000000ll);
+}
+
+__device__ __forceinline__ uint32_t roam_pair_word(uint64_t seed, uint64_t track, uint64_t blk)
+{
+    const uint4 w = philox_block_b3(seed, track, blk);
+    return (w.x & 0xFFFF0000u) | (w.z >> 16);
+}
+
+__global__ void k_roam_pair_word_selftest(uint64_t seed, const uint64_t *track, const uint64_t *blk,
+                                          uint32_t *packed, uint32_t *words, size_t n)
+{
+    const size_t i = blockIdx.x * static_cast<size_t>(blockDim.x) + threadIdx.x;
+    if (i >= n) return;
+    const uint4 w = philox_block(seed, track[i], blk[i]);
+    packed[i] = roam_pair_word(seed, track[i], blk[i]);
+    words[4 * i] = w.x; words[4 * i + 1] = w.y; words[4 * i + 2] = w.z; words[4 * i + 3] = w.w;
 }
 
 __host__ __device__ __forceinline__ double sum9(const double *x)
@@ -541,6 +557,7 @@
     unsigned long long dbg_tsum, dbg_tmax, dbg_waves, dbg_slowmax;
     uint32_t roam_stop;
     uint32_t deal_live;
+    unsigned long long roam_fed, roam_own;
 };
 
 static_assert(sizeof(TrackCtl) <= 128 * sizeof(uint32_t), "final read-back slot of pinned_counts()");
@@ -651,6 +668,7 @@
     int cheap_exact;
     unsigned long long *dbg_buf;
     int debug_roam;
+    int roam_feed;
     uint32_t vis_r, vis_c;
 };
 
@@ -901,6 +919,7 @@
         ctl->error = bad; ctl->par_min = 0xFFFFFFFFu; ctl->steps = 0; ctl->strays = 0; ctl->bin_done = 0; ctl->pad = 0; ctl->roam_slow = 0; ctl->roam_pairs = 0;
         ctl->dbg_tsum = ctl->dbg_tmax = ctl->dbg_waves = ctl->dbg_slowmax = 0;
         ctl->roam_stop = ctl->deal_live = 0;
+        ctl->roam_fed = ctl->roam_own = 0;
     }
     if (d < 9) ctl->prior[d] = pr.v[d];
     if (d >= 9) return;
@@ -1887,20 +1906,32 @@
     }
 }
 
-template <bool REV, int BT = kBlock>
-__global__ __launch_bounds__(BT) void k_step_roam(const StepArgs a, const ThrPrior pr)
-{
+constexpr int kFeedDepth = 3;
+constexpr uint32_t kFeedDone = 0xFFFFFFFFu, kFeedNoTag = 0xFFFFFFFFu;
+template <bool REV, int BT = kBlock, bool FEED = false>
+__global__ __launch_bounds__(FEED ? 2 * BT : BT) void k_step_roam(const StepArgs a, const ThrPrior pr)
+{
+    static_assert(!FEED || BT == kBlock, "feeder waves: narrow blocks only");
+    constexpr int NT = FEED ? 2 * BT : BT;
     __shared__ uint32_t s_win[kWinRows * kWinCols];
     __shared__ int s_box[4];
     __shared__ int s_wid[BT / 64];
-    for (int q = threadIdx.x; q < kWinRows * kWinCols; q += BT) s_win[q] = 0u;
+    __shared__ uint4 s_ring[FEED ? (BT / 64) * kFeedDepth * 64 : 1];
+    __shared__ uint32_t s_tag[FEED ? (BT / 64) * kFeedDepth : 1];
+    __shared__ uint32_t s_read[BT / 64];
+    const bool feeder = FEED && __builtin_amdgcn_readfirstlane(static_cast<int>(threadIdx.x)) >= BT;
+    const uint32_t tid = feeder ? threadIdx.x - BT : threadIdx.x;
+    const int lane = threadIdx.x & 63, wv = static_cast<int>(tid >> 6);
+    for (int q = threadIdx.x; q < kWinRows * kWinCols; q += NT) s_win[q] = 0u;
     if (threadIdx.x == 0) { s_box[0] = s_box[1] = 0x7fffffff; s_box[2] = s_box[3] = -1; }
+    if (FEED && threadIdx.x < (BT / 64) * kFeedDepth) s_tag[threadIdx.x] = kFeedNoTag;
+    if (FEED && threadIdx.x < BT / 64) s_read[threadIdx.x] = 0u;
     __syncthreads();
     TrackCtl *ctl = a.ctl;
     const int in_slot = a.launch & 3, out_slot = (a.launch + 1) & 3;
     const uint32_t xcd = blockIdx.x % kXcd;
     const uint32_t nlive = ctl->count[in_slot][xcd];
-    const uint32_t il = (blockIdx.x / kXcd) * BT + threadIdx.x;
+    const uint32_t il = (blockIdx.x / kXcd) * BT + tid;
     const uint32_t i = xcd * a.cap + il;
     if (blockIdx.x == 0 && threadIdx.x < kXcd) ctl->count[(a.launch + 2) & 3][threadIdx.x] = 0;
 
@@ -1913,6 +1944,25 @@
     live0 = live0 && s.k >= 0 && rc < 8u;
     rc &= 7u;
     int row = s.pos & 0xFFFF, col = (s.pos >> 16) & 0xFFFF;
+    int k = s.k;
+    const long long rel64 = (a.coherent ? static_cast<long long>(s.aux >> 9) : 0) + 1 - a.it_base;
+    const int rel = rel64 > 0x3fffffffLL ? 0x3fffffff : (rel64 < 0 ? 0 : static_cast<int>(rel64));
+    const long long left = a.max_k - k;
+    uint32_t span = !live0 ? 0u : (left > 0x3fffffffLL ? 0x3fffffffu : (left < 0 ? 0u : static_cast<uint32_t>(left)));
+    const int blk0 = (k - rel) >> 1;
+    const unsigned long long track = a.track_base + static_cast<unsigned long long>(t);
+    auto blk_of = [&](const int p) __attribute__((always_inline)) {
+        return static_cast<unsigned long long>(static_cast<uint32_t>(blk0 + p));
+    };
+    const uint32_t ntrips = static_cast<uint32_t>(a.steps) >> 3;
+    auto feed_trip = [&](const uint32_t n) __attribute__((always_inline)) {
+        const int p = 4 * static_cast<int>(n);
+        const uint4 r = make_uint4(roam_pair_word(a.seed, track, blk_of(p)), roam_pair_word(a.seed, track, blk_of(p + 1)),
+                                   roam_pair_word(a.seed, track, blk_of(p + 2)), roam_pair_word(a.seed, track, blk_of(p + 3)));
+        const uint32_t slot = static_cast<uint32_t>(wv * kFeedDepth) + n % static_cast<uint32_t>(kFeedDepth);
+        s_ring[slot * 64u + static_cast<uint32_t>(lane)] = r;
+        if (lane == 0) __hip_atomic_store(&s_tag[slot], n, __ATOMIC_RELEASE, __HIP_MEMORY_SCOPE_WORKGROUP);
+    };
     int win_r0 = 0, win_c0 = 0;
     {
         int r_lo = live0 ? row : 0x7fffffff, r_hi = live0 ? row : -1, c_lo = live0 ? col : 0x7fffffff, c_hi = live0 ? col : -1;
@@ -1936,7 +1986,7 @@
             const unsigned long long lm = __ballot(wid != 0x7fffffff);
             wid = lm ? __shfl(wid, __ffsll(static_cast<long long>(lm)) - 1) : 0x7fffffff;
         }
-        if ((threadIdx.x & 63) == 0) s_wid[threadIdx.x >> 6] = wid;
+        if (lane == 0) s_wid[wv] = wid;
         __syncthreads();
         wid = 0x7fffffff;
         for (int q = BT / 64 - 1; q >= 0; --q) wid = s_wid[q] != 0x7fffffff ? s_wid[q] : wid;
@@ -1947,6 +1997,11 @@
         const bool placed = wid != 0x7fffffff;
         __syncthreads();
         if (!placed && !fits && threadIdx.x == 0) { s_box[0] = r_lo; s_box[1] = c_lo; s_box[2] = r_hi; s_box[3] = c_hi; }
+        if (feeder && __any(live0 && span != 0u)) {
+#pragma unroll 1
+            for (uint32_t n = 0; n < static_cast<uint32_t>(kFeedDepth) && n < ntrips; ++n)
+                if (a.roam_feed != 2 || !(n & 1u)) feed_trip(n);
+        }
         __syncthreads();
         if (s_box[2] >= 0) {
             win_r0 = (s_box[0] + s_box[2] + 1 - kWinRows) / 2;
@@ -1956,13 +2011,27 @@
     const char *pair = reinterpret_cast<const char *>(a.roam);
     const uint32_t ucols = static_cast<uint32_t>(a.cols);
     const uint32_t last_cell = static_cast<uint32_t>(a.rows) * ucols - 1u;
-    int k = s.k;
-    const long long rel64 = (a.coherent ? static_cast<long long>(s.aux >> 9) : 0) + 1 - a.it_base;
-    const int rel = rel64 > 0x3fffffffLL ? 0x3fffffff : (rel64 < 0 ? 0 : static_cast<int>(rel64));
-    const long long left = a.max_k - k;
-    uint32_t span = !live0 ? 0u : (left > 0x3fffffffLL ? 0x3fffffffu : (left < 0 ? 0u : static_cast<uint32_t>(left)));
-    const int blk0 = (k - rel) >> 1;
-    const unsigned long long track = a.track_base + static_cast<unsigned long long>(t);
+    if (feeder) {
+        if (__any(live0 && span != 0u)) {
+            uint32_t n = ntrips < static_cast<uint32_t>(kFeedDepth) ? ntrips : static_cast<uint32_t>(kFeedDepth);
+            uint32_t naps = 1024u + 3u * static_cast<uint32_t>(a.steps);
+            while (n < ntrips) {
+                const uint32_t rd = static_cast<uint32_t>(__builtin_amdgcn_readfirstlane(static_cast<int>(
+                    __hip_atomic_load(&s_read[wv], __ATOMIC_ACQUIRE, __HIP_MEMORY_SCOPE_WORKGROUP))));
+                if (rd == kFeedDone) break;
+                if (n >= rd + static_cast<uint32_t>(kFeedDepth)) {
+                    if (naps-- == 0u) break;
+                    __builtin_amdgcn_s_sleep(16);
+                    continue;
+                }
+                if (n <= rd) { n = rd + 1u; continue; }
+                if (a.roam_feed != 2 || !(n & 1u)) feed_trip(n);
+                ++n;
+            }
+        }
+        live0 = false;
+        span = 0u;
+    }
     const char *tab = reinterpret_cast<const char *>(a.table);
     const uint32_t psh = static_cast<uint32_t>(a.plane_shift);
     const uint32_t rev_e = pr.rev_e;
@@ -2062,9 +2131,10 @@
     int it = 0;
     uint32_t n_pairs = 0, n_slow = 0;
     const unsigned long long t_begin = a.debug_roam ? __builtin_amdgcn_s_memtime() : 0ull;
-    auto one_pair = [&]() __attribute__((always_inline)) {
-        const uint4 w4 = philox_block_b3(a.seed, track, static_cast<unsigned long long>(static_cast<uint32_t>(blk0 + (it >> 1))));
-        const uint32_t ufa = w4.x >> 16, ufb = w4.z >> 16;
+    auto one_pair = [&](const uint32_t uf, const bool given) __attribute__((always_inline)) {
+        uint4 w4 = make_uint4(0u, 0u, 0u, 0u);
+        if (!given) w4 = philox_block_b3(a.seed, track, blk_of(it >> 1));
+        const uint32_t ufa = given ? uf >> 16 : w4.x >> 16, ufb = given ? uf & 0xFFFFu : w4.z >> 16;
         const bool st_a = static_cast<uint32_t>(it - rel) < span, st_b = static_cast<uint32_t>(it + 1 - rel) < span;
         const uint32_t q0 = E.x, qa = E.y, qb = E.z, qc = E.w;
         const uint32_t rc0 = rc;
@@ -2125,6 +2195,7 @@
                 ++n_slow;
                 if (slow) {
                     if (fast) { row = win_r0 + wr; col = win_c0 + wc; }
+                    if (given) w4 = philox_block_b3(a.seed, track, blk_of(it >> 1));
 #pragma unroll 1
                     for (int h = 0; h < 2; ++h)
                         if (static_cast<uint32_t>(it + h - rel) < span) slow_step(h ? w4.z : w4.x, h ? w4.w : w4.y);
@@ -2137,18 +2208,55 @@
     const uint32_t stop_stamp = static_cast<uint32_t>(a.launch) + 1u;
     uint32_t stop_seen = 0u;
     bool stopped = false;
+    uint32_t fd_tag = kFeedNoTag, trip = 0u, fd_slot = 0u, n_fed = 0u;
+    uint4 fd_rec = make_uint4(0u, 0u, 0u, 0u);
+    auto feed_read = [&]() __attribute__((always_inline)) {
+        const uint32_t slot = static_cast<uint32_t>(wv * kFeedDepth) + fd_slot;
+        asm volatile("" ::: "memory");
+        fd_tag = __hip_atomic_load(&s_tag[slot], __ATOMIC_RELAXED, __HIP_MEMORY_SCOPE_WORKGROUP);
+        asm volatile("" ::: "memory");
+        fd_rec = s_ring[slot * 64u + static_cast<uint32_t>(lane)];
+        asm volatile("" ::: "memory");
+    };
+    if (FEED && !feeder) {
+        feed_read();
+        __builtin_amdgcn_s_setprio(1);
+    }
     for (; it + 8 <= a.steps; ) {
         const unsigned long long stepping = __ballot(static_cast<uint32_t>(it - rel) < span), waiting = __ballot(it < rel && span != 0u);
         const bool stop_now = a.roam_stop && waiting == 0ull &&
                               static_cast<uint32_t>(__builtin_amdgcn_readfirstlane(static_cast<int>(stop_seen))) == stop_stamp;
         if (((stepping | waiting) == 0ull) | stop_now) { stopped = stop_now; break; }
         if (a.roam_stop) stop_seen = __hip_atomic_load(&ctl->roam_stop, __ATOMIC_RELAXED, __HIP_MEMORY_SCOPE_AGENT);
-#pragma unroll
-        for (int u = 0; u < 4; ++u) one_pair();
+        if (FEED) {
+            const bool fed = static_cast<uint32_t>(__builtin_amdgcn_readfirstlane(static_cast<int>(fd_tag))) == trip;
+            uint4 rec = fd_rec;
+            ++trip;
+            if (lane == 0) __hip_atomic_store(&s_read[wv], trip, __ATOMIC_RELAXED, __HIP_MEMORY_SCOPE_WORKGROUP);
+            fd_slot = fd_slot + 1u == static_cast<uint32_t>(kFeedDepth) ? 0u : fd_slot + 1u;
+            feed_read();
+            if (!fed) {
+                const int p = it >> 1;
+                rec = make_uint4(roam_pair_word(a.seed, track, blk_of(p)), roam_pair_word(a.seed, track, blk_of(p + 1)),
+                                 roam_pair_word(a.seed, track, blk_of(p + 2)), roam_pair_word(a.seed, track, blk_of(p + 3)));
+            }
+            n_fed += fed ? 4u : 0u;
+            one_pair(rec.x, true);
+            one_pair(rec.y, true);
+            one_pair(rec.z, true);
+            one_pair(rec.w, true);
+        } else {
+#pragma unroll
+            for (int u = 0; u < 4; ++u) one_pair(0u, false);
+        }
     }
     for (; it < a.steps && !stopped; ) {
         if (!__any(static_cast<uint32_t>(it - rel) < span || (it < rel && span != 0u))) break;
-        one_pair();
+        one_pair(0u, false);
+    }
+    if (FEED && !feeder) {
+        __builtin_amdgcn_s_setprio(0);
+        if (lane == 0) __hip_atomic_store(&s_read[wv], kFeedDone, __ATOMIC_RELAXED, __HIP_MEMORY_SCOPE_WORKGROUP);
     }
     if (a.roam_stop && !stopped && it >= a.steps && (threadIdx.x & 63) == 0) atomicMax(&ctl->roam_stop, stop_stamp);
     if (fast) { row = win_r0 + wr; col = win_c0 + wc; }
@@ -2160,6 +2268,8 @@
     }
     if ((threadIdx.x & 63) == 0 && n_pairs) {
         atomicAdd(&ctl->roam_pairs, static_cast<unsigned long long>(n_pairs));
+        atomicAdd(&ctl->roam_own, static_cast<unsigned long long>(n_pairs - n_fed));
+        if (n_fed) atomicAdd(&ctl->roam_fed, static_cast<unsigned long long>(n_fed));
         if (n_slow) atomicAdd(&ctl->roam_slow, static_cast<unsigned long long>(n_slow));
         if (a.debug_roam) {
             const unsigned long long dt = __builtin_amdgcn_s_memtime() - t_begin;
@@ -2170,7 +2280,7 @@
         }
     }
 #ifdef SSRS_DEBUG_WAVE_DUMP
-    if (a.debug_roam && a.launch == SSRS_DEBUG_WAVE_DUMP && a.dbg_buf) {
+    if (a.debug_roam && a.launch == SSRS_DEBUG_WAVE_DUMP && a.dbg_buf && !feeder) {
         const unsigned long long dt = __builtin_amdgcn_s_memtime() - t_begin;
         const int lanes = __popcll(__ballot(live0));
         uint32_t wst = win_stray;
@@ -2184,7 +2294,7 @@
     }
 #endif
     __syncthreads();
-    for (int q = threadIdx.x; q < kWinRows * kWinCols; q += BT) {
+    for (int q = threadIdx.x; q < kWinRows * kWinCols; q += NT) {
         const uint32_t n = s_win[q];
         if (n) atomicAdd(&a.hist[static_cast<uint32_t>(win_r0 + q / kWinCols) * ucols + static_cast<uint32_t>(win_c0 + q % kWinCols)], n);
     }
@@ -2200,9 +2310,8 @@
         if (a.end_rc) reinterpret_cast<uint32_t *>(a.end_rc)[t] = (static_cast<uint32_t>(row) & 0xFFFFu) | (static_cast<uint32_t>(col) << 16);
     }
     __shared__ uint32_t s_surv[BT / 64 + 1];
-    const int lane = threadIdx.x & 63, wv = threadIdx.x >> 6;
     const int nsurv = __popcll(__ballot(active));
-    if (lane == 0) s_surv[wv] = static_cast<uint32_t>(nsurv);
+    if (lane == 0 && !feeder) s_surv[wv] = static_cast<uint32_t>(nsurv);
     __syncthreads();
     if (threadIdx.x == 0) {
         uint32_t tot = 0;
@@ -2211,8 +2320,8 @@
     }
     __syncthreads();
     const uint32_t basei = s_surv[BT / 64];
-    if (basei != 0xFFFFFFFFu) {
-        a.list_out[xcd * a.cap + basei + threadIdx.x] = active ? t : -1;
+    if (basei != 0xFFFFFFFFu && !feeder) {
+        a.list_out[xcd * a.cap + basei + tid] = active ? t : -1;
         if (active) {
             TrackState o;
             o.pos = static_cast<int32_t>((static_cast<uint32_t>(row) & 0xFFFFu) | (static_cast<uint32_t>(col) << 16));
@@ -3161,6 +3270,25 @@
     return SSRS_OK;
 }
 
+extern "C" int ssrs_roam_pair_word_selftest(uint64_t seed, const uint64_t *track, const uint64_t *block,
+                                            uint32_t *packed, uint32_t *words, size_t n, void *stream)
+{
+    SSRS_REQUIRE(track && block && packed && words, "ssrs_roam_pair_word_selftest: NULL pointer");
+    if (n == 0) return SSRS_OK;
+    hipLaunchKernelGGL(k_roam_pair_word_selftest, dim3(static_cast<unsigned>((n + 255) / 256)), dim3(256),
+                       0, as_stream(stream), seed, track, block, packed, words, n);
+    SSRS_HIP_CHECK(hipGetLastError());
+    return SSRS_OK;
+}
+
+static thread_local int64_t g_roam_fed = 0, g_roam_own = 0;
+
+extern "C" void ssrs_tracks_roam_feed_counts(int64_t *fed, int64_t *own)
+{
+    if (fed) *fed = g_roam_fed;
+    if (own) *own = g_roam_own;
+}
+
 extern "C" int ssrs_uniform_selftest(uint64_t seed, const uint64_t *track, const uint64_t *step,
                                      double *out, size_t n, void *stream)
 {
@@ -3189,6 +3317,8 @@
     long long roam_wide_from;
     int roam_width;
     int roam_shuffle;
+    int roam_shuffle_fed;
+    int roam_feed;
 };
 
 static TrackSwitches read_track_switches()
@@ -3210,8 +3340,12 @@
     if (const char *e = std::getenv("SSRS_TRACKS_ROAM_WIDE")) sw.roam_wide_from = std::atoll(e);
     sw.roam_width = 0;
     if (const char *e = std::getenv("SSRS_TRACKS_ROAM_WIDTH")) { const int w = std::atoi(e); if (w == 1 || w == 2 || w == 4) sw.roam_width = w; }
+    sw.roam_feed = 1;
+    if (const char *e = std::getenv("SSRS_TRACKS_ROAM_FEED")) { const int f = std::atoi(e); if (f == 0 || f == 2) sw.roam_feed = f; }
+    if (sw.roam_width > 1) sw.roam_feed = 0;
     sw.roam_shuffle = 16;
-    if (const char *e = std::getenv("SSRS_TRACKS_ROAM_SHUFFLE")) sw.roam_shuffle = std::atoi(e);
+    sw.roam_shuffle_fed = sw.roam_feed ? 4 : 16;
+    if (const char *e = std::getenv("SSRS_TRACKS_ROAM_SHUFFLE")) sw.roam_shuffle = sw.roam_shuffle_fed = std::atoi(e);
     return sw;
 }
 
@@ -3403,6 +3537,7 @@
     a.thr = ws.thr;
     a.wander = ws.wander;
     a.debug_roam = sw.debug_roam ? 1 : 0;
+    a.roam_feed = sw.roam_feed;
     a.roam_stop = sw.roam_stop ? 1 : 0;
     a.dbg_buf = nullptr;
 #ifdef SSRS_DEBUG_WAVE_DUMP
@@ -3492,7 +3627,7 @@
     a.v16_offset = geom.offset;
 
     pol.thr = thr; pol.tiles_ok = tiles_ok; pol.cache_ok = cache_ok; pol.never_scattered = never_scattered;
-    pol.front = a.pf_dir != 0; pol.may_rebalance = sw.rebalance; pol.debug = sw.debug; pol.roam_shuffle = sw.roam_shuffle;
+    pol.front = a.pf_dir != 0; pol.may_rebalance = sw.rebalance; pol.debug = sw.debug; pol.roam_shuffle = sw.roam_shuffle_fed;
     pol.ntracks = ntracks; pol.crossing = p->rows + p->cols;
     pol.binning_on = binning_on; pol.tiles_on = tiles_on; pol.scattered = scattered;
     pol.cached = cache_ok && scattered;
@@ -3592,6 +3727,9 @@
                             if (rev) hipLaunchKernelGGL((k_step_roam<true, 4 * kBlock>), dim3(wblocks), dim3(bt), 0, st, a, thr_prior);
                             else hipLaunchKernelGGL((k_step_roam<false, 4 * kBlock>), dim3(wblocks), dim3(bt), 0, st, a, thr_prior);
                         }
+                    } else if (a.roam_feed) {
+                        if (rev) hipLaunchKernelGGL((k_step_roam<true, kBlock, true>), dim3(blocks), dim3(2 * kBlock), 0, st, a, thr_prior);
+                        else hipLaunchKernelGGL((k_step_roam<false, kBlock, true>), dim3(blocks), dim3(2 * kBlock), 0, st, a, thr_prior);
                     } else if (rev) hipLaunchKernelGGL(k_step_roam<true>, dim3(blocks), dim3(kBlock), 0, st, a, thr_prior);
                     else hipLaunchKernelGGL(k_step_roam<false>, dim3(blocks), dim3(kBlock), 0, st, a, thr_prior);
 #ifdef SSRS_DEBUG_WAVE_DUMP
@@ -3612,9 +3750,11 @@
                         (void)hipStreamSynchronize(st);
                         memcpy(&cb, &host_counts[kFinalSlot], sizeof(TrackCtl));
                         if (cb.dbg_waves)
-                            fprintf(stderr, "[roam] launch %d blocks %u Sl %d: %llu waves, mean %.0f clk, max %.0f clk (x%.2f); slowest-by-slow-pairs wave: %llu of %llu pairs slow\n",
+                            fprintf(stderr, "[roam] launch %d blocks %u Sl %d: %llu waves, mean %.0f clk, max %.0f clk (x%.2f); slowest-by-slow-pairs wave: %llu of %llu pairs slow; "
+                                    "wave-pairs so far %llu, fed %llu\n",
                                     launch, blocks, Sl, cb.dbg_waves, static_cast<double>(cb.dbg_tsum) / cb.dbg_waves, static_cast<double>(cb.dbg_tmax),
-                                    static_cast<double>(cb.dbg_tmax) * cb.dbg_waves / static_cast<double>(cb.dbg_tsum), cb.dbg_slowmax >> 32, cb.dbg_slowmax & 0xFFFFFFFFull);
+                                    static_cast<double>(cb.dbg_tmax) * cb.dbg_waves / static_cast<double>(cb.dbg_tsum), cb.dbg_slowmax >> 32, cb.dbg_slowmax & 0xFFFFFFFFull,
+                                    cb.roam_pairs, cb.roam_fed);
                         (void)hipMemsetAsync(&ws.ctl->dbg_tsum, 0, 4 * sizeof(unsigned long long), st);
                     }
                     return;
@@ -3721,6 +3861,7 @@
         }
         if (sw.roam_width) roam_width = sw.roam_width;
     }
+    pol.roam_shuffle = roam_width > 1 ? sw.roam_shuffle : sw.roam_shuffle_fed;
     hipLaunchKernelGGL(k_deal_sorted, dim3(64), dim3(1024), 0, st, k1, sorted, ws.list[(launch + 1) & 1], ws.ctl,
                        (launch + 1) & 3, (launch + 2) & 3, ws.cap, sw.deal_contiguous ? 1 : 0, roam_width);
     ++launch;
@@ -3891,6 +4032,8 @@
         hipStreamSynchronize(st) != hipSuccess)
         return set_error(SSRS_ERR_HIP, "final read-back failed");
     memcpy(&host_ctl, &host_counts[kFinalSlot], sizeof(TrackCtl));
+    g_roam_fed = static_cast<int64_t>(host_ctl.roam_fed);
+    g_roam_own = static_cast<int64_t>(host_ctl.roam_own);
     if (stats) {
         stats->total_steps = static_cast<int64_t>(host_ctl.steps);
         stats->launches = launch;
@@ -3941,6 +4084,7 @@
     int rc = check_track_args(c);
     if (rc != SSRS_OK) return rc;
     if (stats) *stats = SsrsTrackStats{};
+    g_roam_fed = g_roam_own = 0;
     if (SsrsTrajRecorder *rec = c.rec) {
         rec->used = 0;
         rec->chunks.clear();
diff --git a/ssrs_amd/movmodel.py b/ssrs_amd/movmodel.py
--- a/ssrs_amd/movmodel.py
+++ b/ssrs_amd/movmodel.py
@@ -365,6 +365,8 @@
             nat.ptr(lengths), nat.ptr(ws), C.c_size_t(ws_bytes), C.byref(stats), stream_ptr()))
     elif not want_tracks:
         run(hist, None, None)
+    roam_fed, roam_own = C.c_int64(0), C.c_int64(0)
+    nat.lib().ssrs_tracks_roam_feed_counts(C.byref(roam_fed), C.byref(roam_own))
     return TrackBatch(lengths, ends, hist, traj, offsets, replay=replay, stats=
                       dict(total_steps=int(stats.total_steps), launches=int(stats.launches),
                            kernel_ms=float(stats.kernel_ms), wall_ms=float(stats.wall_ms),
@@ -381,6 +383,7 @@
                            roam_fine_settled=int(stats.reserved0),
                            roam_wave_pairs=int(stats.roam_wave_pairs),
                            roam_slow_wave_pairs=int(stats.roam_slow_wave_pairs),
+                           roam_fed_wave_pairs=int(roam_fed.value), roam_own_wave_pairs=int(roam_own.value),
                            roam_shuffles=int(stats.roam_shuffles),
                            roam_wide_launches=int(stats.roam_wide_launches)))
 
@@ -407,6 +410,19 @@
     return out.cpu().numpy()
 
 
+def roam_pair_words(seed, track, block):
+    tr = to_dev(np.asarray(track, dtype=np.uint64).view(np.int64), torch.int64).reshape(-1)
+    bk = to_dev(np.asarray(block, dtype=np.uint64).view(np.int64), torch.int64).reshape(-1)
+    if tr.numel() != bk.numel():
+        raise ValueError('track and block lengths differ')
+    packed = torch.empty(tr.numel(), dtype=torch.int32, device=tr.device)
+    words = torch.empty((tr.numel(), 4), dtype=torch.int32, device=tr.device)
+    nat.check(nat.lib().ssrs_roam_pair_word_selftest(
+        C.c_uint64(int(seed) & 0xFFFFFFFFFFFFFFFF), nat.ptr(tr), nat.ptr(bk), nat.ptr(packed), nat.ptr(words),
+        C.c_size_t(tr.numel()), stream_ptr()))
+    return packed.cpu().numpy().view(np.uint32), words.cpu().numpy().view(np.uint32)
+
+
 from .presence import (compute_presence_counts, compute_smooth_presence_counts)
 from . import potential as _potential
 
```

Measured after the change: 81710 (median of 6 runs). +10.2%, better.
